# jfdev001/algebraic-multigrid

Hardware: AMD Instinct MI355X
Metric: V-cycles/sec, 2D Poisson N=4096^2 (fine-grid smoother HBM GB/s under roofline) (higher is better)
Workload: dtype f64; 1 GPU; 2D 5-point Poisson 4096x4096 (Grid::laplacian/rhs), true Jacobi smoother omega=0.6 2+2 sweeps, 16-level V-cycle, coarsest 511 dofs, fp64, 1xMI355X; smoother has no counterpart in the reference: pinned to the oracle twin; n=4096, dim=2, levels=16, smoother=jacobi, sweeps=2, graph=True, coarse_solve=band-chain (LDS-resident scalar recurrence, half-bandwidth <= 3, bit-exact), layout=dict

## Files before the change

### algebraic-multigrid_amd/amg_ctypes.py

```python
import contextlib
import ctypes as C
import os

import numpy as np

_HERE = os.path.dirname(os.path.abspath(__file__))
LIB_PATH = os.path.join(_HERE, "libamg_hip.so")

OK, EINVAL, EHIP, ENOMEM, EUNSUPPORTED, ECOMM = 0, 1, 2, 3, 4, 5
SM_SPGS, SM_REF_JACOBI, SM_SOR, SM_JACOBI, SM_MULTICOLOR_GS, SM_CHEBYSHEV, SM_LINE_JACOBI = 0, 1, 2, 3, 4, 5, 6
SM_LINE_ALT = 7
LAYOUT_AUTO, LAYOUT_CSR, LAYOUT_SELL, LAYOUT_DICT = 0, 1, 2, 3

_i32p = C.POINTER(C.c_int32)
_f64p = C.POINTER(C.c_double)
_i64p = C.POINTER(C.c_int64)


class AmgHipError(RuntimeError):
    def __init__(self, status, msg):
        super().__init__(f"amg_hip status {status}: {msg}")
        self.status = status
        self.message = msg

# ... 76 lines not shown
    "amg_hip_setup_on_device": (C.c_int, [C.c_void_p, _i32p]),
    "amg_hip_create_tensor": (C.c_int, [C.c_int64, _i32p, _i32p, _f64p, _f64p, C.c_int32, _i64p,
                                        C.c_int32, C.POINTER(Options), C.POINTER(C.c_void_p)]),
    "amg_hip_create_tensor_dev": (C.c_int, [C.c_int64, C.c_void_p, C.c_void_p, C.c_void_p, C.c_void_p,
                                            C.c_int32, _i64p, C.c_int32, C.POINTER(Options),
                                            C.POINTER(C.c_void_p)]),
    "amg_hip_get_level_dims": (C.c_int, [C.c_void_p, C.c_int32, _i64p]),
    "amg_hip_create_tensor_semi": (C.c_int, [C.c_int64, _i32p, _i32p, _f64p, _f64p, C.c_int32, _i64p,
                                             C.c_int32, _i32p, C.c_double, C.c_int64, C.POINTER(Options),
                                             C.POINTER(C.c_void_p)]),
    "amg_hip_create_tensor_semi_dev": (C.c_int, [C.c_int64, C.c_void_p, C.c_void_p, C.c_void_p, C.c_void_p,
                                                 C.c_int32, _i64p, C.c_int32, _i32p, C.c_double, C.c_int64,
                                                 C.POINTER(Options), C.POINTER(C.c_void_p)]),
    "amg_hip_get_level_axes": (C.c_int, [C.c_void_p, C.c_int32, _i32p]),
    "amg_hip_create_tensor_opdep": (C.c_int, [C.c_int64, _i32p, _i32p, _f64p, _f64p, C.c_int32, _i64p,
                                              C.c_int32, _i32p, C.c_int64, C.POINTER(Options),
                                              C.POINTER(C.c_void_p)]),
    "amg_hip_set_axis_stencil": (None, [C.c_int32]),
    "amg_hip_get_axis_weights": (C.c_int, [C.c_void_p, C.c_int32, _f64p]),
    "amg_hip_axis_restrict": (C.c_int, [C.c_int32, _i64p, C.c_int32, _f64p, _f64p, _f64p]),
    "amg_hip_axis_prolong_add": (C.c_int, [C.c_int32, _i64p, C.c_int32, _f64p, _f64p, _f64p]),
    "amg_hip_get_natural_sides": (C.c_int, [C.c_void_p, _i32p]),
    "amg_hip_create_tensor_periodic": (C.c_int, [C.c_int64, _i32p, _i32p, _f64p, _f64p, C.c_int32, _i64p,
                                                 C.c_int32, C.c_int32, _i32p, C.POINTER(Options),
                                                 C.POINTER(C.c_void_p)]),
    "amg_hip_create_tensor_periodic_dev": (C.c_int, [C.c_int64, C.c_void_p, C.c_void_p, C.c_void_p, C.c_void_p,
                                                     C.c_int32, _i64p, C.c_int32, C.c_int32, _i32p,
                                                     C.POINTER(Options), C.POINTER(C.c_void_p)]),
    "amg_hip_get_periodic_axes": (C.c_int, [C.c_void_p, _i32p]),
    "amg_hip_tensor_restrict_per": (C.c_int, [C.c_int32, _i64p, C.c_int32, C.c_int32, C.c_int32, _f64p, _f64p]),
    "amg_hip_tensor_prolong_add_per": (C.c_int, [C.c_int32, _i64p, C.c_int32, C.c_int32, C.c_int32, _f64p, _f64p]),
    "amg_hip_tensor_restrict_bc": (C.c_int, [C.c_int32, _i64p, C.c_int32, C.c_int32, _f64p, _f64p]),
    "amg_hip_tensor_prolong_add_bc": (C.c_int, [C.c_int32, _i64p, C.c_int32, C.c_int32, _f64p, _f64p]),
    "amg_hip_tensor_axis_strength": (C.c_int, [C.c_int64, _i32p, _i32p, _f64p, C.c_int32, _i64p, _f64p]),
    "amg_hip_tensor_restrict_axes": (C.c_int, [C.c_int32, _i64p, C.c_int32, _f64p, _f64p]),
    "amg_hip_tensor_prolong_add_axes": (C.c_int, [C.c_int32, _i64p, C.c_int32, _f64p, _f64p]),
    "amg_hip_level_transfer_kind": (C.c_int, [C.c_void_p, C.c_int32, _i32p]),
    "amg_hip_tensor_restrict": (C.c_int, [C.c_int32, _i64p, _f64p, _f64p]),
    "amg_hip_tensor_prolong_add": (C.c_int, [C.c_int32, _i64p, _f64p, _f64p]),
    "amg_hip_destroy": (None, [C.c_void_p]),
    "amg_hip_vcycle": (C.c_int, [C.c_void_p]),
    "amg_hip_vcycles": (C.c_int, [C.c_void_p, C.c_int32]),
    "amg_hip_sync": (C.c_int, [C.c_void_p]),
    "amg_hip_solve": (C.c_int, [C.c_void_p, C.c_double, C.c_int64, C.c_int64, _i64p, _f64p,
                                _i32p]),
    "amg_hip_rss": (C.c_int, [C.c_void_p, _f64p]),
    "amg_hip_apply": (C.c_int, [C.c_void_p, C.c_void_p, C.c_void_p]),
    "amg_hip_pcg": (C.c_int, [C.c_void_p, C.c_double, C.c_int64, _i64p, _f64p]),
    "amg_hip_set_mean_projection": (C.c_int, [C.c_void_p, C.c_int32]),
    "amg_hip_get_mean_projection": (C.c_int, [C.c_void_p, _i32p]),
    "amg_hip_center_vec": (C.c_int, [C.c_void_p, C.c_int32, C.c_int32]),
    "amg_hip_block_vcycles": (C.c_int, [C.c_void_p, C.c_int32, C.c_void_p, C.c_void_p, C.c_int32]),
    "amg_hip_block_rss": (C.c_int, [C.c_void_p, C.c_int32, C.c_void_p, C.c_void_p, _f64p]),
    "amg_hip_block_pcg": (C.c_int, [C.c_void_p, C.c_int32, C.c_void_p, C.c_void_p, C.c_double, C.c_int64,
                                    _i64p, _f64p]),
    "amg_hip_block_must_move": (C.c_int, [C.c_void_p, C.c_int32, _f64p]),
    "amg_hip_apply_f32": (C.c_int, [C.c_void_p, C.c_void_p, C.c_void_p]),
    "amg_hip_pcg_mixed": (C.c_int, [C.c_void_p, C.c_double, C.c_int64, _i64p, _f64p]),
    "amg_hip_f32_must_move": (C.c_int, [C.c_void_p, _f64p]),
    "amg_hip_f32_get_vec": (C.c_int, [C.c_void_p, C.c_int32, C.c_int32, C.POINTER(C.c_float)]),
    "amg_hip_f32_set_vec": (C.c_int, [C.c_void_p, C.c_int32, C.c_int32, C.POINTER(C.c_float)]),
    "amg_hip_f32_level_op": (C.c_int, [C.c_void_p, C.c_int32, C.c_int32]),
    "amg_hip_f32_line_subsweep": (C.c_int, [C.c_void_p, C.c_int32, C.c_int32, C.c_int32]),
    "amg_hip_f32_line_factors": (C.c_int, [C.c_void_p, C.c_int32] + [C.POINTER(C.c_float)] * 3),
    "amg_hip_set_f32_lines": (None, [C.c_int32]),
    "amg_hip_set_f32_dict": (None, [C.c_int32]),
    "amg_hip_set_block_lines": (None, [C.c_int32]),
    "amg_hip_n_levels": (C.c_int32, [C.c_void_p]),
    "amg_hip_get_n_dofs": (C.c_int64, [C.c_void_p, C.c_int32]),
    "amg_hip_get_level_nnz": (C.c_int64, [C.c_void_p, C.c_int32]),
    "amg_hip_get_level_matrix": (C.c_int, [C.c_void_p, C.c_int32, _i32p, _i32p, _f64p]),
    "amg_hip_get_transfer_nnz": (C.c_int64, [C.c_void_p, C.c_int32, C.c_int32]),
    "amg_hip_get_transfer": (C.c_int, [C.c_void_p, C.c_int32, C.c_int32, _i32p, _i32p, _f64p]),
    "amg_hip_get_vec": (C.c_int, [C.c_void_p, C.c_int32, C.c_int32, _f64p]),
    "amg_hip_set_vec": (C.c_int, [C.c_void_p, C.c_int32, C.c_int32, _f64p]),
    "amg_hip_copy_vec_dev": (C.c_int, [C.c_void_p, C.c_int32, C.c_int32, C.c_void_p, C.c_int32]),
    "amg_hip_zero_vec": (C.c_int, [C.c_void_p, C.c_int32, C.c_int32]),
    "amg_hip_coarse_halfbw": (C.c_int64, [C.c_void_p]),
    "amg_hip_coarse_solve_kind": (C.c_int32, [C.c_void_p]),
    "amg_hip_fine_sweep_info": (C.c_int, [C.c_void_p, C.c_char_p, C.c_int32, _i32p, _f64p]),
    "amg_hip_set_patch_min_rows": (None, [C.c_int64]),
    "amg_hip_set_band_chain": (None, [C.c_int32]),
    "amg_hip_set_tail_fusion": (None, [C.c_int32]),
    "amg_hip_set_periodic_device_setup": (None, [C.c_int32]),
    "amg_hip_set_patch_tile_flags": (None, [C.c_int32]),
    "amg_hip_set_patch_xf": (None, [C.c_int32]),
    "amg_hip_set_patch_tall": (None, [C.c_int32]),
    "amg_hip_set_patch_seam": (None, [C.c_int32]),
    "amg_hip_patch_leg_lines": (C.c_int32, [C.c_void_p, C.c_int32, C.c_int32]),
    "amg_hip_create_rs": (C.c_int, [C.c_int64, _i32p, _i32p, _f64p, _f64p, C.c_int32, C.c_double, C.c_int64,
                                    C.POINTER(Options), C.POINTER(C.c_void_p)]),
    "amg_hip_slab_plan": (C.c_int, [C.c_int64, C.c_int32, C.c_int32, C.c_int32, C.POINTER(SlabInfo)]),
    "amg_hip_slab_setup": (C.c_int, [C.c_void_p, C.c_int32, C.c_int32, C.c_int32, C.POINTER(SlabInfo)]),
    "amg_hip_slab_run": (C.c_int, [C.c_void_p, C.c_int32]),
    "amg_hip_create_poisson_window": (C.c_int, [C.c_int32, C.c_int64, C.c_int64, C.c_int64, C.c_int32,
                                                C.POINTER(Options), C.POINTER(C.c_void_p)]),
    "amg_hip_window_setup": (C.c_int, [C.c_void_p, _i64p, _i64p, _i64p, _i64p]),
    "amg_hip_window_run": (C.c_int, [C.c_void_p, C.c_int32]),
    "amg_hip_vec_dev_ptr": (C.c_int, [C.c_void_p, C.c_int32, C.c_int32, C.POINTER(C.c_void_p), _i64p]),
    "amg_hip_get_stream": (C.c_int, [C.c_void_p, C.POINTER(C.c_void_p)]),
    "amg_hip_comm_unique_id": (C.c_int, [C.c_char_p]),
    "amg_hip_comm_create": (C.c_int, [C.c_char_p, C.c_int32, C.c_int32, C.c_int32, C.POINTER(C.c_void_p)]),
    "amg_hip_comm_destroy": (None, [C.c_void_p]),
    "amg_hip_comm_rank": (C.c_int32, [C.c_void_p]),
    "amg_hip_comm_world": (C.c_int32, [C.c_void_p]),
    "amg_hip_comm_neighbor_exchange": (C.c_int, [C.c_void_p, C.c_void_p, C.c_int64, C.c_void_p, C.c_int64,
                                                 C.c_void_p, C.c_int64, C.c_void_p, C.c_int64, C.c_void_p]),
    "amg_hip_comm_all_gather": (C.c_int, [C.c_void_p, C.c_void_p, C.c_void_p, C.c_int64, C.c_void_p]),
    "amg_hip_slab_cycle": (C.c_int, [C.c_void_p, C.c_void_p, C.POINTER(SlabInfo)]),
    "amg_hip_window_cycle": (C.c_int, [C.c_void_p, C.c_void_p, C.c_void_p, C.POINTER(WindowPlanC)]),
    "amg_hip_level_layout": (C.c_int32, [C.c_void_p, C.c_int32, C.POINTER(C.c_int32), C.POINTER(C.c_int64)]),
    "amg_hip_get_colors": (C.c_int, [C.c_void_p, C.c_int32, _i32p, _i32p]),
    "amg_hip_level_op": (C.c_int, [C.c_void_p, C.c_int32, C.c_int32]),
    "amg_hip_cheb_bounds": (C.c_int, [C.c_void_p, C.c_int32, _f64p, _f64p]),
    "amg_hip_line_stride": (C.c_int, [C.c_void_p, C.c_int32, C.POINTER(C.c_int64)]),
    "amg_hip_smooth_line": (C.c_int, [C.c_int64, _i32p, _i32p, _f64p, C.c_int64, C.c_double, C.c_int64,
                                      _f64p, _f64p]),
    "amg_hip_line_directions": (C.c_int, [C.c_void_p, C.c_int32, C.POINTER(C.c_int32), C.POINTER(C.c_int64)]),
    "amg_hip_smooth_line_alt": (C.c_int, [C.c_int64, _i32p, _i32p, _f64p, C.c_int32, C.POINTER(C.c_int64),
                                          C.c_double, C.c_int64, C.c_int32, _f64p, _f64p]),
    "amg_hip_line_cyclic": (C.c_int, [C.c_void_p, C.c_int32, _i32p]),
    "amg_hip_smooth_line_alt_per": (C.c_int, [C.c_int64, _i32p, _i32p, _f64p, C.c_int32, C.POINTER(C.c_int64),
                                              C.c_int32, C.c_double, C.c_int64, C.c_int32, _f64p, _f64p]),
    "amg_hip_smooth_chebyshev": (C.c_int, [C.c_int64, _i32p, _i32p, _f64p, _f64p, _f64p, C.c_int32,
                                           C.c_double, C.c_double, C.c_int64]),
    "amg_hip_cycle_bytes": (C.c_int, [C.c_void_p, _f64p, _f64p]),
    "amg_hip_cycle_must_move": (C.c_int, [C.c_void_p, C.c_int32, _f64p]),
    "amg_hip_profile_fine_sweep": (C.c_int, [C.c_void_p, C.c_int32, _f64p, _f64p]),
    "amg_hip_smooth": (C.c_int, [C.c_int32, C.c_int64, _i32p, _i32p, _f64p, _f64p, _f64p,
                                 C.c_double, C.c_double, C.c_int64, C.c_int64, _i64p, _i32p]),
    "amg_hip_spgs_sweep": (C.c_int, [C.c_int32, C.c_int64, _i32p, _i32p, _f64p, _f64p, _f64p]),
    "amg_hip_residual": (C.c_int, [C.c_int64, _i32p, _i32p, _f64p, _f64p, _f64p, _f64p]),
    "amg_hip_spmv": (C.c_int, [C.c_int64, C.c_int64, _i32p, _i32p, _f64p, _f64p, _f64p]),
    "amg_hip_linear_restrict": (C.c_int, [C.c_int64, C.c_int64, _f64p, _f64p]),
    "amg_hip_linear_prolong_add": (C.c_int, [C.c_int64, C.c_int64, _f64p, _f64p]),
    "amg_hip_rss_host": (C.c_int, [C.c_int64, _i32p, _i32p, _f64p, _f64p, _f64p, _f64p]),
    "amg_hip_coarse_solve": (C.c_int, [C.c_int64, _i32p, _i32p, _f64p, _f64p, _f64p, _i64p]),
    "amg_hip_coarse_solve_fast": (C.c_int, [C.c_int64, _i32p, _i32p, _f64p, _f64p, _f64p, _i64p,
                                            _i32p]),
    "amg_hip_laplacian": (C.c_int64, [C.c_int32, C.c_int64, _i32p, _i32p, _f64p]),
    "amg_hip_rhs": (C.c_int, [C.c_int32, C.c_int64, _f64p]),
    "amg_hip_csr_shape": (C.c_int, [C.c_int64, _i32p, _i32p, _i32p]),
    "amg_hip_dev_residual": (C.c_int, [C.c_int64, C.c_int64, C.c_int32, C.c_int32, C.c_void_p,
                                       C.c_void_p, C.c_void_p, C.c_void_p, C.c_void_p,
                                       C.c_void_p, C.c_void_p]),
    "amg_hip_dev_jacobi": (C.c_int, [C.c_int64, C.c_int64, C.c_int32, C.c_int32, C.c_void_p,
                                     C.c_void_p, C.c_void_p, C.c_void_p, C.c_void_p, C.c_void_p,
                                     C.c_double, C.c_int64, C.c_void_p]),
    "amg_hip_dev_spmv": (C.c_int, [C.c_int64, C.c_int64, C.c_int32, C.c_int32, C.c_void_p,
                                   C.c_void_p, C.c_void_p, C.c_void_p, C.c_void_p, C.c_void_p]),
    "amg_hip_devmat_create": (C.c_int, [C.c_int64, C.c_int64, _i32p, _i32p, _f64p, C.c_int32,
                                        C.c_int64, C.c_int32, C.POINTER(C.c_void_p)]),
    "amg_hip_set_index16": (None, [C.c_int32]),
    "amg_hip_set_nontemporal": (None, [C.c_int32]),
    "amg_hip_set_dict_rows": (None, [C.c_int32]),
    "amg_hip_set_dict_stencil": (None, [C.c_int32]),
    "amg_hip_set_xcd_mapping": (None, [C.c_int32]),
    "amg_hip_set_row_types": (None, [C.c_int32]),
    "amg_hip_dict_probe": (C.c_int, [C.c_int64, C.c_int64, _i32p, _i32p, _f64p, C.c_int64,
                                     C.POINTER(C.c_int32), C.POINTER(C.c_int32), C.POINTER(C.c_int32)]),
    "amg_hip_devmat_destroy": (None, [C.c_void_p]),
    "amg_hip_devmat_layout": (C.c_int, [C.c_void_p, C.POINTER(C.c_int32), C.POINTER(C.c_int64)]),
    "amg_hip_devmat_apply": (C.c_int, [C.c_void_p, C.c_int32, C.c_void_p, C.c_void_p, C.c_void_p,
                                       C.c_double, C.c_int64, C.c_void_p]),
    "amg_hip_dev_jacobi_from_zero": (C.c_int, [C.c_int64, C.c_void_p, C.c_void_p, C.c_void_p,
                                               C.c_double, C.c_void_p]),
# ... 72 lines not shown


def set_nontemporal(on):
    lib().amg_hip_set_nontemporal(int(on))


def set_dict_rows(rows_per_lane):
    lib().amg_hip_set_dict_rows(int(rows_per_lane))


def set_dict_stencil(on):
    lib().amg_hip_set_dict_stencil(int(on))


def dict_probe(rowptr, col, val, ncols, diag_shift=0):
    rowptr, col, val = _a32(rowptr), _a32(col), _a64(val)
    a, b, c = C.c_int32(0), C.c_int32(0), C.c_int32(0)
    st = lib().amg_hip_dict_probe(rowptr.size - 1, ncols, _p32(rowptr), _p32(col), _p64(val),
                                  diag_shift, C.byref(a), C.byref(b), C.byref(c))
    if st == EUNSUPPORTED:
        return None
    _chk(st)
    return a.value, b.value, c.value


class Comm:

    def __init__(self, id_bytes, rank, world, device=-1):
        h = C.c_void_p()
        _chk(lib().amg_hip_comm_create(bytes(id_bytes), int(rank), int(world), int(device), C.byref(h)))
        self._h, self.rank, self.world = h, rank, world

    @staticmethod
    def unique_id():
        buf = C.create_string_buffer(128)
        _chk(lib().amg_hip_comm_unique_id(buf))
        return buf.raw

    def slab_cycle(self, mg, info):
        _chk(lib().amg_hip_slab_cycle(mg._h, self._h, C.byref(info)))

    def window_cycle(self, window_mg, tail_mg, plan_c):
        _chk(lib().amg_hip_window_cycle(window_mg._h, tail_mg._h, self._h, C.byref(plan_c)))

    def close(self):
        if getattr(self, "_h", None):
            lib().amg_hip_comm_destroy(self._h)
            self._h = None

    def __del__(self):
        self.close()


def slab_plan(lines, rank, world, levels):
    info = SlabInfo()
    _chk(lib().amg_hip_slab_plan(int(lines), int(rank), int(world), int(levels), C.byref(info)))
    return info


def set_patch_tile_flags(on):
    lib().amg_hip_set_patch_tile_flags(int(bool(on)))


def set_axis_stencil(on):
    lib().amg_hip_set_axis_stencil(int(bool(on)))


def set_patch_xf(on):
    lib().amg_hip_set_patch_xf(int(bool(on)))


def set_patch_tall(on):
    lib().amg_hip_set_patch_tall(int(bool(on)))


def set_patch_seam(on):
    lib().amg_hip_set_patch_seam(int(bool(on)))


def set_tail_fusion(on):
    lib().amg_hip_set_tail_fusion(int(bool(on)))


def set_periodic_device_setup(on):
    lib().amg_hip_set_periodic_device_setup(int(bool(on)))


def set_f32_lines(on):
    lib().amg_hip_set_f32_lines(int(bool(on)))


@contextlib.contextmanager
def f32_lines():
    set_f32_lines(1)
    try:
        yield
    finally:
        set_f32_lines(0)


def set_f32_dict(on):
    lib().amg_hip_set_f32_dict(int(bool(on)))


@contextlib.contextmanager
def f32_dict():
    set_f32_dict(1)
    try:
        yield
    finally:
        set_f32_dict(0)


def set_block_lines(on):
    lib().amg_hip_set_block_lines(int(bool(on)))


@contextlib.contextmanager
def block_lines():
    set_block_lines(1)
    try:
        yield
    finally:
        set_block_lines(0)


def set_band_chain(on):
    lib().amg_hip_set_band_chain(int(bool(on)))


PATCH_MIN_ROWS_DEFAULT = 1000000


def set_patch_min_rows(rows):
    lib().amg_hip_set_patch_min_rows(int(rows))


def set_row_types(on):
    lib().amg_hip_set_row_types(int(on))


def set_xcd_mapping(on):
    lib().amg_hip_set_xcd_mapping(int(on))


class DevMat:

    RESIDUAL, JACOBI, SPMV = 0, 1, 2

    def __init__(self, rowptr, col, val, ncols, layout=LAYOUT_AUTO, diag_shift=0, device=0):
        rowptr, col, val = _a32(rowptr), _a32(col), _a64(val)
        self.rows, self.cols = int(rowptr.size - 1), int(ncols)
        self.diag_shift, self.device = int(diag_shift), int(device)
        self._h = C.c_void_p()
        st = lib().amg_hip_devmat_create(self.rows, self.cols, _p32(rowptr), _p32(col), _p64(val), int(layout),
                                         self.diag_shift, self.device, C.byref(self._h))
        if st == EINVAL:
            raise ValueError(lib().amg_hip_last_error().decode())
        _chk(st)

    def layout(self):
        lay, nb = C.c_int32(0), C.c_int64(0)
        _chk(lib().amg_hip_devmat_layout(self._h, C.byref(lay), C.byref(nb)))
        return lay.value, int(nb.value)

    def apply(self, op, x, f=None, omega=1.0, diag_shift=None):
# ... 487 lines not shown

    @property
    def n_levels(self):
        return lib().amg_hip_n_levels(self._h)

    def get_n_dofs(self, level):
        return int(lib().amg_hip_get_n_dofs(self._h, level))

    def get_coefficient_matrix(self, level):
        n = self.get_n_dofs(level)
        nnz = lib().amg_hip_get_level_nnz(self._h, level)
        colptr = np.empty(n + 1, np.int32)
        rowind = np.empty(nnz, np.int32)
        val = np.empty(nnz, np.float64)
        _chk(lib().amg_hip_get_level_matrix(self._h, level, _p32(colptr), _p32(rowind), _p64(val)))
        return colptr, rowind, val

    def get_transfer(self, level, which):
        w = 1 if which == "R" else 0
        nnz = lib().amg_hip_get_transfer_nnz(self._h, level, w)
        if nnz < 0:
            raise ValueError("level out of range")
        n_h, n_H = self.get_n_dofs(level), self.get_n_dofs(level + 1)
        cols = n_h if w else n_H
        colptr = np.empty(cols + 1, np.int32)
        rowind = np.empty(nnz, np.int32)
        val = np.empty(nnz, np.float64)
        _chk(lib().amg_hip_get_transfer(self._h, level, w, _p32(colptr), _p32(rowind), _p64(val)))
        return colptr, rowind, val

    def _get(self, level, which):
        out = np.empty(self.get_n_dofs(level), np.float64)
        _chk(lib().amg_hip_get_vec(self._h, level, which, _p64(out)))
        return out

    def get_soln(self, level=0):
        return self._get(level, 0)

    def get_rhs(self, level=0):
        return self._get(level, 1)

    def get_residual(self, level=0):
        return self._get(level, 2)

    def set_vec(self, level, which, v):
        v = _a64(v)
        assert v.size == self.get_n_dofs(level)
        _chk(lib().amg_hip_set_vec(self._h, level, {"u": 0, "f": 1, "r": 2}[which], _p64(v)))

    def copy_vec_dev(self, level, which, dev_ptr, to_solver):
        _chk(lib().amg_hip_copy_vec_dev(self._h, level, {"u": 0, "f": 1, "r": 2}[which],
                                        C.c_void_p(dev_ptr), int(to_solver)))

    def zero_vec(self, level, which):
        _chk(lib().amg_hip_zero_vec(self._h, level, {"u": 0, "f": 1, "r": 2}[which]))

    def get_tolerance(self):
        return self.tolerance

    def level_layout(self, level):
        lay, nb = C.c_int32(0), C.c_int64(0)
        _chk(lib().amg_hip_level_layout(self._h, level, C.byref(lay), C.byref(nb)))
        return int(lay.value), int(nb.value)

    def coarse_halfbw(self):
        return int(lib().amg_hip_coarse_halfbw(self._h))

    def get_colors(self, level):
        color = np.empty(self.get_n_dofs(level), np.int32)
        nc = C.c_int32(0)
        _chk(lib().amg_hip_get_colors(self._h, level, _p32(color), C.byref(nc)))
        return color, nc.value

    def cycle_bytes(self):
        a, b = C.c_double(0), C.c_double(0)
        _chk(lib().amg_hip_cycle_bytes(self._h, C.byref(a), C.byref(b)))
        return a.value, b.value

    def cycle_must_move(self, part=0):
        b = C.c_double(0)
        _chk(lib().amg_hip_cycle_must_move(self._h, int(part), C.byref(b)))
        return b.value

    def patch_leg_lines(self, level, leg):
        return int(lib().amg_hip_patch_leg_lines(self._h, int(level), int(leg)))

    def profile_fine_sweep(self, n_launches):
        a, b = C.c_double(0), C.c_double(0)
        _chk(lib().amg_hip_profile_fine_sweep(self._h, n_launches, C.byref(a), C.byref(b)))
        name = C.create_string_buffer(256)
        k, nb = C.c_int32(0), C.c_double(0)
        _chk(lib().amg_hip_fine_sweep_info(self._h, name, 256, C.byref(k), C.byref(nb)))
        return a.value, b.value, k.value, name.value.decode(), nb.value

    def fine_sweep_info(self):
        name = C.create_string_buffer(256)
        k, nb = C.c_int32(0), C.c_double(0)
        _chk(lib().amg_hip_fine_sweep_info(self._h, name, 256, C.byref(k), C.byref(nb)))
        return name.value.decode(), k.value, nb.value

    def cheb_bounds(self, level):
        lo, hi = C.c_double(0), C.c_double(0)
        st = lib().amg_hip_cheb_bounds(self._h, int(level), C.byref(lo), C.byref(hi))
        if st == EINVAL:
            raise ValueError(lib().amg_hip_last_error().decode())
        _chk(st)
        return lo.value, hi.value

    def line_stride(self, level):
        s = C.c_int64(0)
        st = lib().amg_hip_line_stride(self._h, int(level), C.byref(s))
        if st == EINVAL:
            raise ValueError(lib().amg_hip_last_error().decode())
        _chk(st)
        return s.value

    def line_directions(self, level):
        nd = C.c_int32(0)
        st3 = (C.c_int64 * 3)()
        st = lib().amg_hip_line_directions(self._h, int(level), C.byref(nd), st3)
        if st == EINVAL:
            raise ValueError(lib().amg_hip_last_error().decode())
        _chk(st)
        return [int(st3[d]) for d in range(nd.value)]

    def line_cyclic(self, level):
        m = C.c_int32(0)
        st = lib().amg_hip_line_cyclic(self._h, int(level), C.byref(m))
        if st == EINVAL:
            raise ValueError(lib().amg_hip_last_error().decode())
        _chk(st)
        return m.value

    def coarse_solve_kind(self):
        return {0: "band (one wave, sequential, bit-exact)", 1: "spike (partitioned, parallel)",
                2: "band-wide (blocked sequential, any half-bandwidth, bit-exact)",
                3: "band-chain (LDS-resident scalar recurrence, half-bandwidth <= 3, bit-exact)"}[
                    int(lib().amg_hip_coarse_solve_kind(self._h))]

    def level_op(self, level, op):
        _chk(lib().amg_hip_level_op(self._h, level, op))

    def vcycle(self, n=1):
        _chk(lib().amg_hip_vcycles(self._h, n))

    def sync(self):
        _chk(lib().amg_hip_sync(self._h))

    def rss(self):
        out = C.c_double(0)
        _chk(lib().amg_hip_rss(self._h, C.byref(out)))
        return out.value

    def slab_setup(self, rank, world, max_levels=-1):
        info = SlabInfo()
        _chk(lib().amg_hip_slab_setup(self._h, int(rank), int(world), int(max_levels), C.byref(info)))
        return info

    def slab_run(self, part):
        _chk(lib().amg_hip_slab_run(self._h, int(part)))

    def apply_dev(self, v_dev, z_dev):
        _chk(lib().amg_hip_apply(self._h, C.c_void_p(v_dev), C.c_void_p(z_dev)))

    def pcg(self, rtol=1e-10, max_iters=100):
        it, rel = C.c_int64(0), C.c_double(0)
# ... 363 lines not shown
```

### algebraic-multigrid_amd/csrc/kernels.hip

```cpp
#include <hip/hip_runtime.h>
#include <cstdlib>
#include <stdint.h>

#include <cstdio>
#include <type_traits>
#include <utility>
#include <vector>
#include <algorithm>
#include <cmath>

#include "kernels.hpp"

namespace amg_hip {

__device__ __forceinline__ void lds_barrier() {
  asm volatile("s_waitcnt lgkmcnt(0)\n\ts_barrier" ::: "memory");
}

constexpr bool mode_cheb(int m) { return (m & ~3) == 16; }
constexpr bool mode_jac(int m) { return m == CSR_JACOBI || mode_cheb(m); }
constexpr bool cheb_first(int m) { return (m & 1) != 0; }
constexpr bool cheb_last(int m) { return (m & 2) != 0; }
template <int MODE>
__device__ __forceinline__ double cheb_update(double t, double xi, double di, double alpha, double beta,
// ... 745 lines not shown
    dict_rows<MODE, WORDS, UN, R>(s, row0, tab, x, omega, dshift, res);
  }
  if constexpr (mode_cheb(MODE)) {
    double dn[R];
#pragma unroll
    for (int r = 0; r < R; ++r) res[r] = cheb_update<MODE>(res[r], s.xi[r], s.di[r], alpha, omega, dn[r]);
    if (!cheb_last(MODE)) dict_store<WORDS, NT, R>(s, row0, dn, dvec);
  }
  dict_store<WORDS, NT, R>(s, row0, res, out);
}

template <int R>
__device__ __forceinline__ void dict_restrict_tail(int tile, int n, const double* rs, int nH,
                                                   double* __restrict__ fH,
                                                   const double* __restrict__ diagH,
                                                   double* __restrict__ uH1,
                                                   double* __restrict__ uH0, double omega) {
  for (int q = threadIdx.x; q < 128 * R - 1; q += 256) {
    const int j = tile * (128 * R - 1) + q;
    if (j >= nH) break;
    const int64_t i = 2 * (int64_t)j;
    double sum = 0.0;
    if (i < n) sum += 0.5 * rs[2 * q];
    if (i + 1 < n) sum += 1.0 * rs[2 * q + 1];
    if (i + 2 < n) sum += 0.5 * rs[2 * q + 2];
    fH[j] = sum;
    if (uH1) {
      const double xi = 0.0, acc = 0.0;
      const double d = diagH[j];
      uH1[j] = (d == 0.0) ? xi : xi + omega * ((sum - acc) / d - xi);
    } else {
      uH0[j] = 0.0;
    }
  }
}
template <int R>
__device__ __forceinline__ void dict_prolong_tail(int tile, int n, const double* rs, int n_h,
                                                  const double* uh_in, double* uh_out) {
  typedef double f64x2 __attribute__((ext_vector_type(2)));
  const int stride = 256 * R - 2;
#pragma unroll
  for (int r = 0; r < R; ++r) {
    const int q = (int)threadIdx.x * R + r;
    const int j = tile * stride + q;
    if ((q == 0 && tile != 0) || q > stride || j > n) continue;
    double t0 = 0.0, t1 = 0.0;
    const double b = (j < n) ? rs[q] : 0.0;
    if (j >= 1 && j - 1 < n) t0 += 0.5 * rs[q - 1];
    if (j < n) {
      t0 += 0.5 * b;
      t1 += 1.0 * b;
    }
    const int64_t i = 2 * (int64_t)j;
    if (i + 1 < n_h) {
      f64x2 u = *reinterpret_cast<const f64x2*>(uh_in + i);
      u.x = u.x + t0;
      u.y = u.y + t1;
      *reinterpret_cast<f64x2*>(uh_out + i) = u;
    } else if (i < n_h) {
      uh_out[i] = uh_in[i] + t0;
    }
  }
}
__device__ __forceinline__ double dict_restrict_pre(int tile, int nH, const double* __restrict__ diagH) {
  const int q = threadIdx.x, j = tile * 255 + q;
  return (q < 255 && j < nH) ? diagH[j] : 0.0;
}
__device__ __forceinline__ void dict_restrict_tail(int tile, int n, const double* rs, int nH,
                                                   double* __restrict__ fH, double dH,
                                                   double* __restrict__ uH1, double omega) {
  const int q = threadIdx.x, j = tile * 255 + q;
  if (q >= 255 || j >= nH) return;
  const int64_t i = 2 * (int64_t)j;
  double sum = 0.0;
  if (i < n) sum += 0.5 * rs[2 * q];
  if (i + 1 < n) sum += 1.0 * rs[2 * q + 1];
  if (i + 2 < n) sum += 0.5 * rs[2 * q + 2];
  fH[j] = sum;
  const double xi = 0.0, acc = 0.0;
  const double d = dH;
  uH1[j] = (d == 0.0) ? xi : xi + omega * ((sum - acc) / d - xi);
}
typedef double pair_f64x2 __attribute__((ext_vector_type(2)));
__device__ __forceinline__ void dict_prolong_pre(int tile, int n, int n_h, const double* uh_in,
                                                 pair_f64x2 (&pre)[2], double& lone) {
  bool two[2], one[2];
  int64_t i[2];
#pragma unroll
  for (int r = 0; r < 2; ++r) {
    const int q = (int)threadIdx.x * 2 + r;
    const int j = tile * 510 + q;
    const bool on = !((q == 0 && tile != 0) || q > 510 || j > n);
    i[r] = 2 * (int64_t)j;
    two[r] = on && i[r] + 1 < n_h;
    one[r] = on && i[r] + 1 == n_h;
    pre[r].x = pre[r].y = 0.0;
  }
  lone = 0.0;
#pragma unroll
  for (int r = 0; r < 2; ++r)
    if (two[r]) pre[r] = *reinterpret_cast<const pair_f64x2*>(uh_in + i[r]);
  if (one[0] || one[1]) lone = uh_in[n_h - 1];
}
__device__ __forceinline__ void dict_prolong_tail(int tile, int n, const double* rs, int n_h,
                                                  const pair_f64x2 (&pre)[2], double lone,
                                                  double* uh_out) {
#pragma unroll
  for (int r = 0; r < 2; ++r) {
    const int q = (int)threadIdx.x * 2 + r;
    const int j = tile * 510 + q;
    if ((q == 0 && tile != 0) || q > 510 || j > n) continue;
    double t0 = 0.0, t1 = 0.0;
    const double b = (j < n) ? rs[q] : 0.0;
    if (j >= 1 && j - 1 < n) t0 += 0.5 * rs[q - 1];
    if (j < n) {
      t0 += 0.5 * b;
      t1 += 1.0 * b;
    }
    const int64_t i = 2 * (int64_t)j;
    if (i + 1 < n_h) {
      pair_f64x2 u = pre[r];
      u.x = u.x + t0;
      u.y = u.y + t1;
      *reinterpret_cast<pair_f64x2*>(uh_out + i) = u;
    } else if (i < n_h) {
      uh_out[i] = lone + t0;
    }
  }
}
template <int WORDS, int UN, bool NT, int R>
__global__ __launch_bounds__(256) void dict_resid_restrict_kernel(
    int n, const uint64_t* __restrict__ codes, const uint8_t* __restrict__ rtype,
    const uint64_t* __restrict__ rwords, const int32_t* __restrict__ doff,
    const double* __restrict__ dval, int ntab, const double* x, const double* __restrict__ f,
    double* r_out, int nH, double* __restrict__ fH, const double* __restrict__ diagH,
    double* __restrict__ uH1, double* __restrict__ uH0, double omega, int xcd_map,
    const double* __restrict__ utd, const int32_t* __restrict__ uti) {
  __shared__ DictEntry tab[256];
  __shared__ uint64_t wtab[256 * WORDS];
  __shared__ double rs[256 * R];
  const int tile = xcd_tile(blockIdx.x, gridDim.x, xcd_map);
  const int row0 = tile * (256 * R - 2) + (int)threadIdx.x * R;
  DictStream<WORDS, R> s;
  dict_fetch<CSR_RESID, WORDS, NT, R>(s, row0, n, codes, rtype, f, x, 0);
  dict_stage_table<CSR_RESID>(tab, doff, dval, ntab);
  if (rtype) dict_stage_words<WORDS>(wtab, rwords);
  __syncthreads();
  double res[R];
  bool fast = false;
  if constexpr (R == 2 && (UN == 7 || UN == 16)) {
    if (utd) fast = dict_stencil_can<UN>(s.ty, s.live, uti);
    if (fast) dict_rows_stencil<CSR_RESID, UN>(s.ty, s.fi, s.xi, row0, utd, uti, x, omega, res);
  }
  if (!fast) {
    if (rtype) dict_expand<WORDS, R>(s, wtab);
    dict_rows<CSR_RESID, WORDS, UN, R>(s, row0, tab, x, omega, 0, res);
  }
  if (r_out) dict_store<WORDS, NT, R>(s, row0, res, r_out);
#pragma unroll
  for (int r = 0; r < R; ++r) rs[threadIdx.x * R + r] = s.live[r] ? res[r] : 0.0;
  __syncthreads();
  dict_restrict_tail<R>(tile, n, rs, nH, fH, diagH, uH1, uH0, omega);
}
template <int WORDS, int UN, bool NT, int R>
__global__ __launch_bounds__(256) void dict_jacobi_prolong_kernel(
    int n, const uint64_t* __restrict__ codes, const uint8_t* __restrict__ rtype,
    const uint64_t* __restrict__ rwords, const int32_t* __restrict__ doff,
    const double* __restrict__ dval, int ntab, const double* x, const double* __restrict__ f,
    double* out, double omega, int n_h, const double* uh_in, double* uh_out, int xcd_map,
    const double* __restrict__ utd, const int32_t* __restrict__ uti) {
  __shared__ DictEntry tab[256];
  __shared__ uint64_t wtab[256 * WORDS];
  __shared__ double rs[256 * R];
  const int tile = xcd_tile(blockIdx.x, gridDim.x, xcd_map);
  const int stride = 256 * R - 2;
  const int row0 = tile * stride + (int)threadIdx.x * R;
  DictStream<WORDS, R> s;
  dict_fetch<CSR_JACOBI, WORDS, NT, R>(s, row0, n, codes, rtype, f, x, 0);
  dict_stage_table<CSR_JACOBI>(tab, doff, dval, ntab);
  if (rtype) dict_stage_words<WORDS>(wtab, rwords);
  __syncthreads();
  double res[R];
  bool fast = false;
  if constexpr (R == 2 && (UN == 7 || UN == 16)) {
    if (utd) fast = dict_stencil_can<UN>(s.ty, s.live, uti);
    if (fast) dict_rows_stencil<CSR_JACOBI, UN>(s.ty, s.fi, s.xi, row0, utd, uti, x, omega, res);
  }
  if (!fast) {
    if (rtype) dict_expand<WORDS, R>(s, wtab);
    dict_rows<CSR_JACOBI, WORDS, UN, R>(s, row0, tab, x, omega, 0, res);
  }
  dict_store<WORDS, NT, R>(s, row0, res, out);
#pragma unroll
  for (int r = 0; r < R; ++r) rs[threadIdx.x * R + r] = s.live[r] ? res[r] : 0.0;
// ... 170 lines not shown
    const uint64_t* __restrict__ rwords, const int32_t* __restrict__ doff,
    const double* __restrict__ dval, int ntab, const double* a, const double* __restrict__ f,
    double* u_out, double* r_out, int nH, double* __restrict__ fH,
    const double* __restrict__ diagH, double* __restrict__ uH1, double omega, int hbw,
    int xcd_map) {
  __shared__ DictEntry tabJ[256];
  __shared__ DictEntry tabR[256];
  __shared__ __attribute__((aligned(16))) uint64_t wc[PAIR_W * WORDS];
  __shared__ uint16_t tw[PAIR_W / 2];
  __shared__ __attribute__((aligned(16))) double aw[PAIR_AW];
  __shared__ __attribute__((aligned(16))) double fw[PAIR_W];
  __shared__ double uw[PAIR_W];
  __shared__ double rs[512];
  const int tile = xcd_tile(blockIdx.x, gridDim.x, xcd_map);
  const int t0 = tile * 510, w0 = t0 - hbw, W = 512 + 2 * hbw;
  const bool types = rtype != nullptr;
  PairLoads<WORDS> g;
  if (types) dict_pair_issue<WORDS, true>(g, n, w0, hbw, codes, rtype, rwords, doff, dval, ntab, a, f);
  else dict_pair_issue<WORDS, false>(g, n, w0, hbw, codes, rtype, rwords, doff, dval, ntab, a, f);
  const double dH = dict_restrict_pre(tile, nH, diagH);
  dict_put_table<CSR_JACOBI>(tabJ, g.tv, g.to, ntab);
  dict_put_table<CSR_RESID>(tabR, g.tv, g.to, ntab);
  if (types) dict_pair_commit<WORDS, true>(g, n, w0, hbw, wc, tw, aw, fw);
  else dict_pair_commit<WORDS, false>(g, n, w0, hbw, wc, tw, aw, fw);
  __syncthreads();
  dict_pair_stage1<WORDS, UN>(n, w0, hbw, types, tabJ, wc, tw, aw, fw, omega, uw, u_out);
  __syncthreads();
  const int row0 = t0 + (int)threadIdx.x * 2;
  DictStream<WORDS, 2> s;
  dict_pair_stream<WORDS>(s, row0 - w0, W, row0, n, types, wc, tw, fw);
  if (types) dict_expand<WORDS, 2>(s, wc);
  double res[2];
  dict_rows<CSR_RESID, WORDS, UN, 2>(s, row0 - w0, tabR, uw, omega, 0, res);
  if (r_out) dict_store<WORDS, false, 2>(s, row0, res, r_out);
  rs[threadIdx.x * 2] = s.live[0] ? res[0] : 0.0;
  rs[threadIdx.x * 2 + 1] = s.live[1] ? res[1] : 0.0;
  __syncthreads();
  dict_restrict_tail(tile, n, rs, nH, fH, dH, uH1, omega);
}
template <int WORDS, int UN>
__global__ __launch_bounds__(256) void dict_pair_up_kernel(
    int n, const uint64_t* __restrict__ codes, const uint8_t* __restrict__ rtype,
    const uint64_t* __restrict__ rwords, const int32_t* __restrict__ doff,
    const double* __restrict__ dval, int ntab, const double* a, const double* __restrict__ f,
    double* u_out, double omega, int hbw, int n_h, const double* uh_in, double* uh_out,
    int xcd_map) {
  __shared__ DictEntry tabJ[256];
  __shared__ __attribute__((aligned(16))) uint64_t wc[PAIR_W * WORDS];
  __shared__ uint16_t tw[PAIR_W / 2];
  __shared__ __attribute__((aligned(16))) double aw[PAIR_AW];
  __shared__ __attribute__((aligned(16))) double fw[PAIR_W];
  __shared__ double uw[PAIR_W];
  __shared__ double rs[512];
  const int tile = xcd_tile(blockIdx.x, gridDim.x, xcd_map);
  const int t0 = tile * 510, w0 = t0 - hbw, W = 512 + 2 * hbw;
  const bool types = rtype != nullptr;
  PairLoads<WORDS> g;
  if (types) dict_pair_issue<WORDS, true>(g, n, w0, hbw, codes, rtype, rwords, doff, dval, ntab, a, f);
  else dict_pair_issue<WORDS, false>(g, n, w0, hbw, codes, rtype, rwords, doff, dval, ntab, a, f);
  pair_f64x2 pre[2];
  double pre1;
  dict_prolong_pre(tile, n, n_h, uh_in, pre, pre1);
  dict_put_table<CSR_JACOBI>(tabJ, g.tv, g.to, ntab);
  if (types) dict_pair_commit<WORDS, true>(g, n, w0, hbw, wc, tw, aw, fw);
  else dict_pair_commit<WORDS, false>(g, n, w0, hbw, wc, tw, aw, fw);
  __syncthreads();
  dict_pair_stage1<WORDS, UN>(n, w0, hbw, types, tabJ, wc, tw, aw, fw, omega, uw, nullptr);
  __syncthreads();
  const int row0 = t0 + (int)threadIdx.x * 2;
  DictStream<WORDS, 2> s;
  dict_pair_stream<WORDS>(s, row0 - w0, W, row0, n, types, wc, tw, fw);
  s.xi[0] = uw[row0 - w0];
  s.xi[1] = uw[row0 - w0 + 1];
  if (types) dict_expand<WORDS, 2>(s, wc);
  double res[2];
  dict_rows<CSR_JACOBI, WORDS, UN, 2>(s, row0 - w0, tabJ, uw, omega, 0, res);
  dict_store<WORDS, false, 2>(s, row0, res, u_out);
  rs[threadIdx.x * 2] = s.live[0] ? res[0] : 0.0;
  rs[threadIdx.x * 2 + 1] = s.live[1] ? res[1] : 0.0;
  __syncthreads();
  dict_prolong_tail(tile, n, rs, n_h, pre, pre1, uh_out);
}

constexpr int PATCH_TW = 64;
constexpr int PATCH_EH = 48;
constexpr int patch_th(int rings) { return PATCH_EH - 2 * rings; }
static bool patch_rings_ok(int rings) { return rings == 2 || rings == 3; }
constexpr int PATCH_EC = PATCH_TW + 8;
constexpr int PATCH_NT = 432;
constexpr int PATCH_K = PATCH_EH * PATCH_EC / PATCH_NT;
constexpr int PATCH_BUF = (PATCH_EH + 2) * PATCH_EC;
constexpr int PATCH_MAXTAB = 192;
static_assert(PATCH_EH * PATCH_EC == PATCH_K * PATCH_NT && PATCH_NT % PATCH_EC == 0, "patch geometry");
template <int EH_, int EC_>
struct PatchFrameT {
  static constexpr int EH = EH_, EC = EC_, CL = (EC_ - PATCH_TW) / 2;
  static constexpr int NT = EH_ / PATCH_K * EC_, BUF = (EH_ + 2) * EC_;
  static constexpr int th(int rings) { return EH_ - 2 * rings; }
  static_assert(EH_ % PATCH_K == 0 && (EC_ - PATCH_TW) % 2 == 0 && NT >= PATCH_MAXTAB && NT <= 1024, "patch frame");
};
using PatchFrame = PatchFrameT<PATCH_EH, PATCH_EC>;
static_assert(PatchFrame::NT == PATCH_NT && PatchFrame::BUF == PATCH_BUF && PatchFrame::CL == 4, "patch geometry");

struct PatchJ { double a, d; };
struct PatchR { double a; int32_t loff, ok; };

struct PatchCells {
  int cell0, row0, lj0, li;
  double f[PATCH_K];
  uint32_t ty[PATCH_K / 4];
  bool live[PATCH_K];
  bool uniform;
  uint32_t tu;
  bool flagged;
  __device__ __forceinline__ uint32_t type(int k) const {
    return flagged ? tu : (ty[k >> 2] >> (8 * (k & 3))) & 255u;
  }
};

struct PatchU {
  double wj[9], wr[9], diag;
#ifdef AMG_PATCH_FASTDIV
  double rdiag;
#endif
  uint32_t rmask, corners;
};
__device__ __forceinline__ void patch_load_u(PatchU& U, uint32_t tu, const double* __restrict__ utabd,
                                             const int32_t* __restrict__ utabi) {
  const double* d = utabd + (size_t)tu * 19;
  const int32_t* i = utabi + (size_t)tu * 2;
#pragma unroll
  for (int e = 0; e < 9; ++e) {
    U.wj[e] = d[e];
    U.wr[e] = d[9 + e];
  }
  U.diag = d[18];
#ifdef AMG_PATCH_FASTDIV
  U.rdiag = 1.0 / (U.diag == 0.0 ? 1.0 : U.diag);
#endif
  U.rmask = (uint32_t)i[0];
  U.corners = (uint32_t)i[1];
}
template <bool RESID, bool CORNERS, bool GS = false, int MASK = -1, class FR = PatchFrame>
__device__ __forceinline__ void patch_eval_u(const double* buf, int cell0, const PatchU& U,
                                             const double (&f)[PATCH_K], double omega,
                                             double (&res)[PATCH_K]) {
  const double* p = buf + cell0 - FR::EC;
  if (!CORNERS && !RESID && U.diag == 0.0) {
#pragma unroll
    for (int k = 0; k < PATCH_K; ++k) res[k] = p[(k + 1) * FR::EC];
    return;
  }
  double w[3][3];
#pragma unroll
  for (int r = 0; r < 2; ++r)
#pragma unroll
    for (int c = 0; c < 3; ++c) w[r][c] = (CORNERS || c == 1 || r == 1) ? p[r * FR::EC + c - 1] : 0.0;
#pragma unroll
  for (int k = 0; k < PATCH_K; ++k) {
#pragma unroll
    for (int c = 0; c < 3; ++c)
      w[2][c] = (CORNERS || c == 1) ? p[(k + 2) * FR::EC + c - 1] : 0.0;
    if (!CORNERS) {
      w[2][0] = p[(k + 2) * FR::EC - 1];
      w[2][2] = p[(k + 2) * FR::EC + 1];
    }
// ... 914 lines not shown
      if (nt) go(W, U, integral_constant<bool, true>{}, integral_constant<int, 1>{});
      else go(W, U, integral_constant<bool, false>{}, integral_constant<int, 1>{});
    }
    return hipGetLastError();
  };
  if (words == 1) {
    if (wmax <= 3) return with_nr(integral_constant<int, 1>{}, integral_constant<int, 3>{});
    if (wmax <= 5) return with_nr(integral_constant<int, 1>{}, integral_constant<int, 5>{});
    if (wmax <= 7) return with_nr(integral_constant<int, 1>{}, integral_constant<int, 7>{});
    return with_nr(integral_constant<int, 1>{}, integral_constant<int, 8>{});
  }
  if (wmax <= 9) return with_nr(integral_constant<int, 2>{}, integral_constant<int, 9>{});
  if (wmax <= 12) return with_nr(integral_constant<int, 2>{}, integral_constant<int, 12>{});
  return with_nr(integral_constant<int, 2>{}, integral_constant<int, 16>{});
}
static bool dict_args_ok(int64_t n, int words, int wmax, int ntab) {
  return n < ((int64_t)1 << 31) - 1024 && ntab <= 255 && (words == 1 || words == 2) &&
         wmax <= 8 * words;
}
static bool aligned16(const void* a, const void* b, const void* c) {
  return ((reinterpret_cast<uintptr_t>(a) | reinterpret_cast<uintptr_t>(b) |
           reinterpret_cast<uintptr_t>(c)) & 15) == 0;
}
static int g_xcd_slab = 1;
static int g_dict_stencil = [] {
  const char* e = std::getenv("AMG_HIP_DICT_STENCIL");
  return (e && *e == '0') ? 0 : 1;
}();
static const double* dict_stencil_tab(const DictRef& D, const double* x) {
  return (g_dict_stencil && D.utd && D.uti && D.rtype && (reinterpret_cast<uintptr_t>(x) & 15) == 0) ? D.utd : nullptr;
}
static int dict_xcd_map(const DictRef& D, int64_t tile_rows = 512) {
  if (!g_xcd_map) return 0;
  const int64_t tp = D.hb / tile_rows / 8 * 8;
  if (g_xcd_slab && tp >= 16 && tp <= (1 << 20)) return (int)tp;
  return D.nt ? 0 : 1;
}
static bool dict_two_rows(int64_t n, const DictRef& D, const void* f, const void* out) {
  return g_dict_rows_per_lane == 2 && n >= 4096 && aligned16(f, out, D.rtype ? nullptr : D.codes) &&
         (!D.rtype || (reinterpret_cast<uintptr_t>(D.rtype) & 1) == 0);
}
hipError_t launch_dict_resid_restrict(int64_t n, const DictRef& D, const double* x,
                                      const double* f, double* r_out, int64_t nH, double* fH,
                                      const double* diagH, double* uH1, double* uH0,
                                      double omega, hipStream_t st) {
  if (n <= 0) return hipSuccess;
  if (!dict_args_ok(n, D.words, D.wmax, D.ntab) || nH > n || !fH || (uH1 ? !diagH : !uH0))
    return hipErrorInvalidValue;
  const bool two = dict_two_rows(n, D, f, r_out);
  const int64_t stride = 256 * (two ? 2 : 1) - 2;
  const unsigned tiles = (unsigned)((n + stride - 1) / stride);
  return dict_dispatch(D.words, D.wmax, D.nt != 0, two, [&](auto W, auto U, auto NTF, auto RR) {
    hipLaunchKernelGGL((dict_resid_restrict_kernel<decltype(W)::value, decltype(U)::value,
                                                   decltype(NTF)::value, decltype(RR)::value>),
                       dim3(tiles), dim3(256), 0, st, (int)n, D.codes, D.rtype, D.rwords, D.doff,
                       D.dval, D.ntab, x, f, r_out, (int)nH, fH, diagH, uH1, uH0, omega, dict_xcd_map(D, stride),
                       dict_stencil_tab(D, x), D.uti);
  });
}
hipError_t launch_dict_jacobi_prolong(int64_t n, const DictRef& D, const double* x,
                                      const double* f, double* out, double omega, int64_t n_h,
                                      const double* uh_in, double* uh_out, hipStream_t st) {
  if (n <= 0) return hipSuccess;
  if (!dict_args_ok(n_h, D.words, D.wmax, D.ntab) || n > n_h || !uh_in || !uh_out ||
      ((reinterpret_cast<uintptr_t>(uh_in) | reinterpret_cast<uintptr_t>(uh_out)) & 15) != 0)
    return hipErrorInvalidValue;
  const bool two = dict_two_rows(n, D, f, out);
  const int64_t stride = 256 * (two ? 2 : 1) - 2;
  const unsigned tiles = (unsigned)((n + stride - 1) / stride);
  return dict_dispatch(D.words, D.wmax, D.nt != 0, two, [&](auto W, auto U, auto NTF, auto RR) {
    hipLaunchKernelGGL((dict_jacobi_prolong_kernel<decltype(W)::value, decltype(U)::value,
                                                   decltype(NTF)::value, decltype(RR)::value>),
                       dim3(tiles), dim3(256), 0, st, (int)n, D.codes, D.rtype, D.rwords, D.doff,
                       D.dval, D.ntab, x, f, out, omega, (int)n_h, uh_in, uh_out, dict_xcd_map(D, stride),
                       dict_stencil_tab(D, x), D.uti);
  });
}
bool dict_pair_ok(int64_t n, const DictRef& D, int hb, const void* a, const void* b, const void* c) {
  return hb >= 0 && hb <= PAIR_HB - 1 && n >= 256 && n <= 400000 && !D.nt &&
         dict_args_ok(n, D.words, D.wmax, D.ntab) && g_dict_rows_per_lane == 2 &&
         aligned16(a, b, c) && aligned16(D.rtype ? nullptr : D.codes, nullptr, nullptr) &&
         (!D.rtype || (reinterpret_cast<uintptr_t>(D.rtype) & 1) == 0);
}
template <class F>
static hipError_t dict_dispatch_wu(int words, int wmax, F&& go) {
  using std::integral_constant;
  if (words == 1) {
    if (wmax <= 3) go(integral_constant<int, 1>{}, integral_constant<int, 3>{});
    else if (wmax <= 5) go(integral_constant<int, 1>{}, integral_constant<int, 5>{});
    else if (wmax <= 7) go(integral_constant<int, 1>{}, integral_constant<int, 7>{});
    else go(integral_constant<int, 1>{}, integral_constant<int, 8>{});
  } else {
    if (wmax <= 9) go(integral_constant<int, 2>{}, integral_constant<int, 9>{});
    else if (wmax <= 12) go(integral_constant<int, 2>{}, integral_constant<int, 12>{});
    else go(integral_constant<int, 2>{}, integral_constant<int, 16>{});
  }
  return hipGetLastError();
}
hipError_t launch_dict_pair_down(int64_t n, const DictRef& D, int hb, const double* a,
                                 const double* f, double* u_out, double* r_out, int64_t nH,
                                 double* fH, const double* diagH, double* uH1, double omega,
                                 hipStream_t st) {
  if (!dict_pair_ok(n, D, hb, a, f, u_out) || !fH || !diagH || !uH1 || nH > n ||
      (r_out && (reinterpret_cast<uintptr_t>(r_out) & 15)))
    return hipErrorInvalidValue;
  const int hbw = (hb + 1) & ~1;
  const unsigned tiles = (unsigned)((n + 509) / 510);
  return dict_dispatch_wu(D.words, D.wmax, [&](auto W, auto U) {
    hipLaunchKernelGGL((dict_pair_down_kernel<decltype(W)::value, decltype(U)::value>), dim3(tiles),
                       dim3(256), 0, st, (int)n, D.codes, D.rtype, D.rwords, D.doff, D.dval, D.ntab,
                       a, f, u_out, r_out, (int)nH, fH, diagH, uH1, omega, hbw, dict_xcd_map(D));
  });
}
hipError_t launch_dict_pair_up(int64_t n, const DictRef& D, int hb, const double* a,
                               const double* f, double* u_out, double omega, int64_t n_h,
                               const double* uh_in, double* uh_out, hipStream_t st) {
  if (!dict_pair_ok(n, D, hb, a, f, u_out) || n > n_h || !uh_in || !uh_out ||
      ((reinterpret_cast<uintptr_t>(uh_in) | reinterpret_cast<uintptr_t>(uh_out)) & 15) != 0)
    return hipErrorInvalidValue;
  const int hbw = (hb + 1) & ~1;
  const unsigned tiles = (unsigned)((n + 509) / 510);
  return dict_dispatch_wu(D.words, D.wmax, [&](auto W, auto U) {
    hipLaunchKernelGGL((dict_pair_up_kernel<decltype(W)::value, decltype(U)::value>), dim3(tiles),
                       dim3(256), 0, st, (int)n, D.codes, D.rtype, D.rwords, D.doff, D.dval, D.ntab,
                       a, f, u_out, omega, hbw, (int)n_h, uh_in, uh_out, dict_xcd_map(D));
  });
}
constexpr int MARCH_TL = 16, MARCH_TC = 64, MARCH_NT = 512;
constexpr int MARCH_XL = MARCH_TL + 4, MARCH_XC = MARCH_TC + 4;
constexpr int MARCH_SL = MARCH_TL + 2, MARCH_SC = MARCH_TC + 2;
constexpr int MARCH_XN = MARCH_XL * MARCH_XC, MARCH_SN = MARCH_SL * MARCH_SC;
constexpr int MARCH_XS = (MARCH_XN + MARCH_NT - 1) / MARCH_NT;
constexpr int MARCH_SS = (MARCH_SN + MARCH_NT - 1) / MARCH_NT;
constexpr int MARCH_OS = MARCH_TL * MARCH_TC / MARCH_NT;
constexpr int MARCH_TYPES = 64;
typedef MarchRef MarchArgs;
__device__ __forceinline__ double march_update(const double (&w)[6], double diag, const double (&nb)[6],
                                               double xi, double fi, double omega) {
  double acc = 0.0;
#pragma unroll
  for (int u = 0; u < 6; ++u) acc += w[u] * nb[u];
  const bool nod = diag == 0.0;
  const double q = (fi - acc) / (nod ? 1.0 : diag);
  return nod ? xi : xi + omega * (q - xi);
}
__global__ __launch_bounds__(MARCH_NT) void march_kernel(MarchArgs A) {
  __shared__ double X[3][MARCH_XN];
  __shared__ double S[3][MARCH_SN];
  __shared__ double wt[MARCH_TYPES * 8];
  const int tid = (int)threadIdx.x;
  const int tiles_c = A.m / MARCH_TC, tiles_l = A.lines / MARCH_TL;
  const int tile = (int)blockIdx.x % (tiles_c * tiles_l), chunk = (int)blockIdx.x / (tiles_c * tiles_l);
  const int l0 = (tile / tiles_c) * MARCH_TL, c0 = (tile % tiles_c) * MARCH_TC;
  const int pa = chunk * A.chunk_planes, pb = min(pa + A.chunk_planes, A.planes);
  for (int q = tid; q < A.ntypes * 8; q += MARCH_NT) wt[q] = A.wtab[q];
  int xoff[MARCH_XS];
#pragma unroll
  for (int k = 0; k < MARCH_XS; ++k) {
    const int q = k * MARCH_NT + tid;
    const int line = l0 - 2 + q / MARCH_XC, col = c0 - 2 + q % MARCH_XC;
    xoff[k] = (q < MARCH_XN && line >= 0 && line < A.lines && col >= 0 && col < A.m) ? line * A.m + col : -1;
  }
  static_assert(MARCH_SS == MARCH_OS + 1 && 2 * MARCH_SC + 2 * MARCH_TL <= MARCH_NT, "first-sweep cell map");
  int soff[MARCH_SS], si[MARCH_SS], sx[MARCH_SS];
  int ooff[MARCH_OS];
#pragma unroll
  for (int k = 0; k < MARCH_OS; ++k) {
    const int q = k * MARCH_NT + tid;
    const int ol = q / MARCH_TC, oc = q % MARCH_TC;
    ooff[k] = (l0 + ol) * A.m + c0 + oc;
    soff[k] = ooff[k];
    si[k] = (ol + 1) * MARCH_SC + oc + 1;
    sx[k] = (ol + 2) * MARCH_XC + oc + 2;
  }
  {
    const int r = tid;
    int sl, sc;
    if (r < MARCH_SC) { sl = 0; sc = r; }
    else if (r < 2 * MARCH_SC) { sl = MARCH_SL - 1; sc = r - MARCH_SC; }
    else if (r < 2 * MARCH_SC + MARCH_TL) { sl = r - 2 * MARCH_SC + 1; sc = 0; }
    else { sl = r - 2 * MARCH_SC - MARCH_TL + 1; sc = MARCH_SC - 1; }
    const bool ring = r < 2 * MARCH_SC + 2 * MARCH_TL;
    if (!ring) { sl = 1; sc = 1; }
    const int line = l0 - 1 + sl, col = c0 - 1 + sc;
    soff[MARCH_OS] = (ring && line >= 0 && line < A.lines && col >= 0 && col < A.m) ? line * A.m + col : -1;
    si[MARCH_OS] = ring ? sl * MARCH_SC + sc : -1;
    sx[MARCH_OS] = (sl + 1) * MARCH_XC + sc + 1;
  }
  const int64_t M = (int64_t)A.m * A.lines;
  double xr[MARCH_XS];
  auto fetch_x = [&](int plane) {
#pragma unroll
    for (int k = 0; k < MARCH_XS; ++k)
      xr[k] = (plane >= 0 && plane < A.planes && xoff[k] >= 0) ? A.x[(int64_t)plane * M + xoff[k]] : 0.0;
  };
  double wi[6];
#pragma unroll
  for (int u = 0; u < 6; ++u) wi[u] = A.wint[u];
  const double di = A.dint;
  const uint32_t ti = (uint32_t)A.tint;
  double nf1[MARCH_SS];
  uint32_t nt1[MARCH_SS];
  auto fetch_ops = [&](int q) {
    const int p1 = q - 1;
    const bool live1 = p1 >= pa - 1 && p1 <= pb && p1 >= 0 && p1 < A.planes;
#pragma unroll
    for (int k = 0; k < MARCH_SS; ++k) {
      const bool live = live1 && soff[k] >= 0;
      const int64_t r = live ? (int64_t)p1 * M + soff[k] : 0;
// ... 5130 lines not shown
```

### algebraic-multigrid_amd/csrc/kernels.hpp

```cpp
#pragma once
#include <hip/hip_runtime_api.h>
#include <stddef.h>
#include <stdint.h>

namespace amg_hip {

enum CsrMode {
  CSR_RESID = 0,
  CSR_JACOBI = 1,
  CSR_SPMV = 2,
  CSR_RSSQ = 3,
  CSR_GS = 4,
  CSR_JACOBI_P = 5,
  CSR_SPMV_ADD = 6,
  CSR_CHEB = 7
};
constexpr int cheb_kernel_mode(bool first, bool last) { return 16 + (first ? 1 : 0) + (last ? 2 : 0); }
struct ChebStep {
  double* d = nullptr;
  double alpha = 0.0, beta = 0.0;
  bool first = true, last = true;
};

hipError_t launch_dict_gs_sweep(int nc, const int32_t* starts_dev, int64_t n_storage, int words, int wmax,
// ... 26 lines not shown
hipError_t launch_line_setup(const LineRef& L, const int32_t* rowptr, const int32_t* col, const double* val,
                             uint64_t* bad, hipStream_t st);
int64_t line_setup_host(int64_t n, int64_t s, const int32_t* rowptr, const int32_t* col, const double* val,
                        int64_t m = 0, int cyc = 0);
hipError_t launch_line_solve(const LineRef& L, const double* r, double* y, double* u, double omega,
                             hipStream_t st);
bool line_few_chains(int64_t s);
hipError_t launch_line_solve_f32(const LineRefT<float>& L, const float* r, float* y, float* u, float omega,
                                 hipStream_t st);
constexpr int LINEX_COLS = 64, LINEX_RUNS = 8;
template <typename T>
struct LineXRefT {
  int64_t n = 0, nx = 1;
  T *dl = nullptr, *ip = nullptr, *cp = nullptr;
  int32_t cyc = 0;
};
using LineXRef = LineXRefT<double>;
int64_t linex_run(int64_t nx);
hipError_t launch_linex_setup(const LineXRef& L, const int32_t* rowptr, const int32_t* col, const double* val,
                              uint64_t* bad, hipStream_t st);
int64_t linex_setup_host(int64_t n, int64_t nx, const int32_t* rowptr, const int32_t* col, const double* val,
                         int cyc = 0);
hipError_t launch_linex_solve(const LineXRef& L, double* r, double* u, double omega, hipStream_t st);
hipError_t launch_linex_solve_f32(const LineXRefT<float>& L, float* r, float* u, float omega, hipStream_t st);
template <typename T>
struct SeamRefT {
  int64_t n = 0, s = 1, m = 0;
  const T* p = nullptr;
  const T* coef = nullptr;
};
using SeamRef = SeamRefT<double>;
hipError_t launch_seam_rhs(int64_t n, int64_t s, int64_t m, const int32_t* rowptr, const int32_t* col,
                           const double* val, double* u, double* v, hipStream_t st);
hipError_t launch_seam_coef(int64_t n, int64_t s, int64_t m, const int32_t* rowptr, const int32_t* col,
                            const double* val, const double* q, double* coef, uint64_t* bad, hipStream_t st);
int64_t seam_setup_host(int64_t n, int64_t s, int64_t m, const int32_t* rowptr, const int32_t* col,
                        const double* val);
hipError_t launch_line_seam(const SeamRef& S, double* r, hipStream_t st);
hipError_t launch_line_seam_f32(const SeamRefT<float>& S, float* r, hipStream_t st);
hipError_t launch_sell(int mode, int64_t n, int idx16, const int64_t* soff,
                       const void* scol, const double* sval, const double* x,
                       const double* f, double* out, double omega, int64_t diag_shift,
                       hipStream_t st);
struct DictRef {
  int words = 1, wmax = 0, nt = 0, ntab = 0;
  const uint64_t* codes = nullptr;
  const uint8_t* rtype = nullptr;
  const uint64_t* rwords = nullptr;
  const int32_t* doff = nullptr;
  const double* dval = nullptr;
  int scan_new = 99;
  int hb = 0;
  const double* utd = nullptr;
  const int32_t* uti = nullptr;
};
void set_xcd_mapping(int on);
void set_dict_rows_per_lane(int r);
void set_dict_stencil(int on);
hipError_t launch_dict(int mode, int64_t n, const DictRef& D, const double* x, const double* f,
                       double* out, double omega, int64_t diag_shift, hipStream_t st);
hipError_t launch_dict_cheb(int64_t n, const DictRef& D, const double* x, const double* f, double* out,
                            const ChebStep& c, hipStream_t st);
void dict_kernel_name(int mode, int64_t n, const DictRef& D, const void* f, const void* out,
                      char* buf, size_t cap);
hipError_t launch_dict_gs_color(int64_t p0, int64_t count, int words, int wmax,
                                const uint64_t* codes, const int32_t* rowid, const int32_t* doff,
                                const double* dval, int ntab, const double* f, double* u,
                                hipStream_t st);
hipError_t launch_dict_resid_restrict(int64_t n, const DictRef& D, const double* x,
                                      const double* f, double* r_out, int64_t nH, double* fH,
                                      const double* diagH, double* uH1, double* uH0,
                                      double omega, hipStream_t st);
hipError_t launch_dict_jacobi_prolong(int64_t n, const DictRef& D, const double* x,
                                      const double* f, double* out, double omega, int64_t n_h,
                                      const double* uh_in, double* uh_out, hipStream_t st);
bool dict_pair_ok(int64_t n, const DictRef& D, int hb, const void* a, const void* b, const void* c);
hipError_t launch_dict_pair_down(int64_t n, const DictRef& D, int hb, const double* a,
                                 const double* f, double* u_out, double* r_out, int64_t nH,
                                 double* fH, const double* diagH, double* uH1, double omega,
                                 hipStream_t st);
hipError_t launch_dict_pair_up(int64_t n, const DictRef& D, int hb, const double* a,
                               const double* f, double* u_out, double omega, int64_t n_h,
                               const double* uh_in, double* uh_out, hipStream_t st);
constexpr int TAIL_LEVELS_MAX = 6;
struct TailLevelRef {
  int n, hbw, words, ntab;
  const uint8_t* rtype;
  const uint64_t* rwords;
  const int32_t* doff;
  const double* dval;
  const double* f;
  double* u;
  double* tmp;
  const double* diag;
};
struct TailRef {
  int nlev;
  TailLevelRef L[TAIL_LEVELS_MAX];
  int nc, wc;
  const double *cf, *cb, *dg;
  double *fc, *uc, *tmpc;
  const double* diagc;
  int n_fine;
  const double* uf_in;
  double* uf_out;
  double omega;
};
bool tail_level_ok(int64_t n, const DictRef& D, int hb);
int tail_max_coarse();
size_t tail_lds_bytes(const TailRef& A);
size_t tail_lds_capacity();
hipError_t launch_tail(const TailRef& A, hipStream_t st);

struct PatchRef {
  const uint8_t* rtype = nullptr;
  const double* ptab = nullptr;
  const double* utabd = nullptr;
  const int32_t* utabi = nullptr;
  int rings = 3;
  const uint8_t* tflag = nullptr;
  int nent = 0, ntypes = 0, un = 0, nt = 0;
  int umask = 0;
  const uint8_t* cflag = nullptr;
  double dHu = 0.0;
};
hipError_t launch_patch_coarse_flags(int64_t n, int64_t m, int rings, int64_t nH, const double* diagH,
                                     double dref, uint8_t* cflag, hipStream_t st);
hipError_t launch_patch_tile_flags(int64_t n, int64_t m, int rings, const uint8_t* rtype, int ntypes,
                                   uint8_t* flag, int64_t* n_tiles, hipStream_t st);
bool patch_geometry_ok(int64_t n, int64_t m);
int patch_un(int longest_row);
int patch_default_umask(int un);
int patch_kind_umask(int un, int umask);
int patch_lds_pitch();
int patch_max_entries();
hipError_t launch_patch_down(bool first, int64_t n, int64_t m, const PatchRef& P, const double* x,
                             const double* f, double* u_out, double* r_out, int64_t nH, double* fH,
                             const double* diagH, double* uH1, double omega, hipStream_t st,
                             int64_t line_lo = 0, int64_t line_hi = -1, bool xf = false);
int patch_tile_lines(int rings);
int patch_leg_rings(bool first);
hipError_t launch_patch_up(int64_t n, int64_t m, const PatchRef& P, const double* x, const double* f,
                           const double* uH, int64_t nH, double* u_out, double omega,
                           hipStream_t st, int64_t line_lo = 0, int64_t line_hi = -1);
int patch_seam_lines();
hipError_t launch_patch_seam_flags(int64_t n, int64_t m, const uint8_t* rtype, int ntypes, uint8_t* flag,
                                   int64_t* n_tiles, hipStream_t st);
hipError_t launch_patch_seam(int64_t n, int64_t m, const PatchRef& P, const double* x, const double* f,
                             const double* uH, int64_t nH, double* u_out, double* fH, double omega,
                             hipStream_t st);
int patch_rb_max_stages(bool tail);
uint32_t patch_rb_stages(const int* colors, int count);
hipError_t launch_patch_rb(bool prolong, bool tail, int64_t n, int64_t m, const PatchRef& P, const double* x,
                           const double* f, const double* uH, int64_t nH, double* u_out, double* r_out,
                           double* fH, double* uH_zero, uint32_t stages, uint32_t ctab, hipStream_t st,
                           int64_t line_lo = 0, int64_t line_hi = -1);
struct MarchRef {
  int m = 0, lines = 0, planes = 0, ntypes = 0, tint = -1, chunk_planes = 0;
  double omega = 1.0, dint = 0.0;
  double wint[6] = {0, 0, 0, 0, 0, 0};
  const double* wtab = nullptr;
  const uint8_t* rtype = nullptr;
  const double* x = nullptr;
  const double* f = nullptr;
  double* out = nullptr;
};
// ... 230 lines not shown
```

### algebraic-multigrid_amd/csrc/solver.cpp

```cpp
#include <cstddef>
#include <hip/hip_runtime.h>

#include <algorithm>
#include <cmath>
#include <chrono>
#include <cstdio>
#include <cstdlib>
#include <cstring>
#include <functional>
#include <map>
#include <memory>
#include <string>
#include <thread>
#include <vector>

#include <dlfcn.h>

#include "../../include/amg_hip.h"
#include "capture_once.hpp"
#include "host_setup.hpp"
#include "kernels.hpp"

using namespace amg_hip;
#ifdef AMG_PATCH_STAMPS
// ... 1340 lines not shown
  DevMem val;
};
struct F32Line {
  DevMem dl, ip, cp, v, w, y;
  LineRefT<float> ref(const LineOnDev& D) const {
    LineRefT<float> R;
    R.n = D.n;
    R.s = D.s;
    R.dl = dl.as<float>();
    R.ip = ip.as<float>();
    R.cp = cp.as<float>();
    R.v = v.as<float>();
    R.w = w.as<float>();
    return R;
  }
};
struct F32Level {
  F32Mat rows, cols_own;
  const F32Mat* cols = nullptr;
  DevMem u, f, r, tmp, d;
  DevMem pval, rval;
  F32Line line;
  DevMem xdl, xip, xcp;
  F32Line yz[2];
  DevMem seam_p[3], seam_coef[3];
  LineXRefT<float> xref(const AltOnDev& D) const {
    LineXRefT<float> R;
    R.n = D.n;
    R.nx = D.len[0];
    R.dl = xdl.as<float>();
    R.ip = xip.as<float>();
    R.cp = xcp.as<float>();
    return R;
  }
  SeamRefT<float> seam(const AltOnDev& D, int d) const {
    SeamRefT<float> S;
    S.n = D.n;
    S.s = D.stride[d];
    S.m = D.len[d];
    S.p = seam_p[d].as<float>();
    S.coef = seam_coef[d].as<float>();
    return S;
  }
};
struct F32 {
  bool ready = false;
  std::vector<F32Level> lv;
  DevMem cf, cy, cx;
  DevMem pr, pz;
  hipGraph_t graph = nullptr;
  hipGraphExec_t exec = nullptr;
  void reset_graph() {
    if (exec) (void)hipGraphExecDestroy(exec);
    if (graph) (void)hipGraphDestroy(graph);
    exec = nullptr;
    graph = nullptr;
  }
};

int g_march = [] {
  const char* e = std::getenv("AMG_HIP_MARCH");
  return (e && *e == '0') ? 0 : 1;
}();
int g_tail_fusion = [] {
  const char* e = std::getenv("AMG_HIP_TAIL_FUSION");
  return (e && *e == '1') ? 1 : 0;
}();
int g_periodic_device_setup = [] {
  const char* e = std::getenv("AMG_HIP_PERIODIC_DEVICE_SETUP");
  return (e && *e == '1') ? 1 : 0;
}();
int g_f32_lines = [] {
  const char* e = std::getenv("AMG_HIP_F32_LINES");
  return (e && *e == '1') ? 1 : 0;
}();
int g_f32_dict = [] {
  const char* e = std::getenv("AMG_HIP_F32_DICT");
  return (e && *e == '1') ? 1 : 0;
}();
int g_block_lines = [] {
  const char* e = std::getenv("AMG_HIP_BLOCK_LINES");
  return (e && *e == '1') ? 1 : 0;
}();
int64_t g_patch_min_rows = 1000000;

struct amg_hip_solver {
  amg_hip_options opt;
  int64_t patch_min_rows = g_patch_min_rows;
  int patch_xf = g_patch_xf;
  int patch_tall = g_patch_tall;
  int patch_seam = g_patch_seam;
  int device = 0;
  hipStream_t stream = nullptr;
  bool own_stream = true;
  std::vector<Level> lv;
  bool device_setup = false;
  CoarseOnDev coarse;
  DevMem scratch;
  DevMem pcg_x, pcg_p, pcg_q, pcg_b;
  bool project_mean = false;
  hipGraph_t graph = nullptr;
  hipGraphExec_t graph_exec = nullptr;
  bool graph_ready = false;
  double cycle_bytes = 0, fine_sweep_bytes = 0;
  double must_move[6] = {0, 0, 0, 0, 0, 0};
  int acct_part = -1;
  void acct(double bytes) { if (acct_part >= 0) must_move[acct_part] += bytes; }
  int seam_piece = 0, seam_src = 0;
  hipGraph_t seam_graph[5] = {nullptr, nullptr, nullptr, nullptr, nullptr};
  hipGraphExec_t seam_exec[5] = {nullptr, nullptr, nullptr, nullptr, nullptr};
  void reset_seam_graphs() {
    for (int i = 0; i < 5; ++i) {
      if (seam_exec[i]) (void)hipGraphExecDestroy(seam_exec[i]);
      if (seam_graph[i]) (void)hipGraphDestroy(seam_graph[i]);
      seam_exec[i] = nullptr;
      seam_graph[i] = nullptr;
    }
  }
  Slab slab;
  Block blk;
  bool block_acct = false;
  double block_mm[2] = {0, 0};
  void bacct(double mat, double per_col) {
    if (!block_acct) return;
    block_mm[0] += mat;
    block_mm[1] += per_col;
  }
  F32 f32;
  bool f32_acct = false;
  double f32_mm = 0;
  void facct(double bytes) { if (f32_acct) f32_mm += bytes; }

  ~amg_hip_solver() {
    f32.reset_graph();
    blk.reset_graphs();
    slab.reset_graphs();
    reset_seam_graphs();
    if (graph_exec) (void)hipGraphExecDestroy(graph_exec);
    if (graph) (void)hipGraphDestroy(graph);
    if (stream && own_stream) (void)hipStreamDestroy(stream);
  }
};

namespace {

void layout_of(const DevMat& A, int32_t* layout, int64_t* matrix_stream_bytes);
double mat_bytes(const DevMat& A) {
  int64_t b = 0;
  layout_of(A, nullptr, &b);
  return (double)b;
}

amg_hip_status enqueue_multicolor(amg_hip_solver* s, Level& L, hipStream_t st, bool again);

std::string tensor_level_error(int l, const int64_t d[3]) {
  return "level " + std::to_string(l + 1) + " is not possible: level " + std::to_string(l) + " is a " +
         std::to_string(d[0]) + " x " + std::to_string(d[1]) + " x " + std::to_string(d[2]) +
         " grid and an axis of fewer than 2 points cannot be coarsened; reduce `n_levels`";
}

bool jacobi_fuses_zero(const amg_hip_solver* s) {
  return s->opt.smoother == AMG_HIP_SM_JACOBI && !s->opt.no_fusion && s->opt.smoother_iters >= 1;
}
bool jacobi_fuses_prolong(const amg_hip_solver* s, int l) {
  const Level& L = s->lv[l];
  return s->opt.fuse_prolong && jacobi_fuses_zero(s) && L.linear && s->opt.stencil_transfers &&
         L.A_cols().sell;
}

bool fuses_resid_restrict(const amg_hip_solver* s, int l) {
  if (l + 1 >= (int)s->lv.size()) return false;
  const Level& L = s->lv[l];
  if (s->opt.no_fusion || !L.linear || !s->opt.stencil_transfers || !L.A_rows.dict ||
      L.A_rows.dict_shift != 0)
// ... 58 lines not shown
  Level& L = s->lv[l];
  const std::vector<int> q = mc_sequence(L.n_colors, s->opt.smoother_iters);
  const int n = (int)q.size();
  std::vector<McLaunch> P;
  auto chunks = [&](int from, int count, int cap, bool prolong_first) {
    if (count <= 0) return;
    const int k = (count + cap - 1) / cap;
    int at = from;
    for (int c = 0; c < k; ++c) {
      const int len = count / k + (c < count % k ? 1 : 0);
      McLaunch M;
      M.stages = patch_rb_stages(q.data() + at, len);
      M.prolong = prolong_first && c == 0;
      P.push_back(M);
      at += len;
    }
  };
  const int tail_cnt = std::min(n, patch_rb_max_stages(true));
  chunks(0, n - tail_cnt, patch_rb_max_stages(false), false);
  {
    McLaunch M;
    M.stages = patch_rb_stages(q.data() + (n - tail_cnt), tail_cnt);
    M.tail = true;
    P.push_back(M);
  }
  *n_down = (int)P.size();
  chunks(0, n, patch_rb_max_stages(false), true);
  double* third = s->opt.keep_residual ? L.mc_aux.as<double>() : L.r.as<double>();
  double* cur = L.u.as<double>();
  for (size_t i = 0; i < P.size(); ++i) {
    P[i].in = cur;
    P[i].out = i + 1 == P.size() ? L.u.as<double>() : ((i & 1) ? third : L.tmp.as<double>());
    cur = P[i].out;
  }
  return P;
}

bool fuses_jacobi_prolong(const amg_hip_solver* s, int l) {
  if (l + 2 >= (int)s->lv.size()) return false;
  if (patch_level_ok(s, l)) return false;
  const Level& L = s->lv[l];
  const DevMat& AC = s->lv[l + 1].A_cols();
  return jacobi_fuses_zero(s) && !jacobi_fuses_prolong(s, l) && L.linear &&
         s->opt.stencil_transfers && AC.dict && AC.dict_shift == 0;
}

bool pair_level_ok(const amg_hip_solver* s, int l) {
  if (l < 1 || l + 1 >= (int)s->lv.size()) return false;
  const Level& L = s->lv[l];
  const DevMat& A = L.A_rows;
  return jacobi_fuses_zero(s) && s->opt.smoother_iters == 2 && L.symmetric && A.dict &&
         A.dict_shift == 0 && fuses_resid_restrict(s, l) &&
         dict_pair_ok(L.n, A.dict_ref(), A.dict_hb, L.u.p, L.f.p, L.tmp.p);
}
bool pair_up_ok(const amg_hip_solver* s, int l) {
  return pair_level_ok(s, l) && fuses_jacobi_prolong(s, l - 1);
}

int tail_from(const amg_hip_solver* s) {
  const int nl = (int)s->lv.size();
  if (!g_tail_fusion || s->opt.keep_residual || s->opt.window || nl < 3 || s->coarse.kind != COARSE_CHAIN || s->coarse.pin ||
      s->coarse.n > tail_max_coarse())
    return -1;
  int lt = nl - 1;
  while (lt - 1 >= 1 && nl - 1 - (lt - 1) <= TAIL_LEVELS_MAX) {
    const int l = lt - 1;
    const Level& L = s->lv[l];
    if (!(pair_level_ok(s, l) && pair_up_ok(s, l) && tail_level_ok(L.n, L.A_rows.dict_ref(), L.A_rows.dict_hb) &&
          L.diag.p && s->lv[l + 1].diag.p))
      break;
    lt = l;
  }
  for (; lt <= nl - 2; ++lt) {
    TailRef T;
    std::memset(&T, 0, sizeof(T));
    T.nlev = nl - 1 - lt;
    for (int q = 0; q < T.nlev; ++q) T.L[q].n = (int)s->lv[lt + q].n;
    T.nc = (int)s->coarse.n;
    T.wc = (int)s->coarse.w;
    if (tail_lds_bytes(T) <= tail_lds_capacity()) return lt;
  }
  return -1;
}

static bool march_fill(const amg_hip_solver* s, int l, MarchRef* R) {
  const Level& L = s->lv[l];
  const DevMat& A = L.A_cols();
  if (!(s->opt.smoother == AMG_HIP_SM_JACOBI && s->opt.smoother_iters == 2 && !s->opt.no_fusion && !s->opt.window &&
        s->slab.levels == 0 && A.dict && A.dict_typed && A.march_ntypes > 0 && A.dmarch.p && A.march_m > 0 &&
        L.n % A.march_M == 0 && A.march_M % A.march_m == 0 && g_march))
    return false;
  R->m = A.march_m;
  R->lines = A.march_M / A.march_m;
  R->planes = (int)(L.n / A.march_M);
  R->ntypes = A.march_ntypes;
  R->tint = A.march_tint;
  R->omega = s->opt.omega;
  R->dint = A.march_dint;
  for (int u = 0; u < 6; ++u) R->wint[u] = A.march_wint[u];
  R->wtab = A.dmarch.as<double>();
  R->rtype = A.drtype.as<uint8_t>();
  R->f = L.f.as<double>();
  R->x = L.u.as<double>();
  R->out = L.tmp.as<double>();
  R->chunk_planes = 1;
  return march_ok(*R);
}
amg_hip_status enqueue_smooth(amg_hip_solver* s, int l, int phase = 0, int prolong_into = -1,
                              double* prolong_out = nullptr, bool reverse = false) {
  Level& L = s->lv[l];
  hipStream_t st = s->stream;
  const int iters = s->opt.smoother_iters;
  switch (s->opt.smoother) {
    case AMG_HIP_SM_SPGS:
      s->acct(iters * 2.0 * (mat_bytes(L.A_rows) + 24.0 * L.n + (L.scan_C > 0 ? 16.0 * L.n : 0.0)));
      for (int it = 0; it < iters; ++it) {
        if (L.scan_C > 0) {
          const DictRef D = L.A_rows.dict_ref();
          HIP_TRY(launch_gs_scan(L.n, D, L.f.as<double>(), L.u.as<double>(), L.tmp.as<double>(), false, 0,
                                 1.0, L.scan_C, L.scan_ring, st));
          HIP_TRY(launch_gs_scan(L.n, D, L.f.as<double>(), L.u.as<double>(), L.tmp.as<double>(), true, 0,
                                 1.0, L.scan_C, L.scan_ring, st));
          continue;
        }
        HIP_TRY(launch_gs_lex(L.lex_fwd->d, L.f.as<double>(), L.u.as<double>(), 0, 1.0, st));
        HIP_TRY(launch_gs_lex(L.lex_bwd->d, L.f.as<double>(), L.u.as<double>(), 0, 1.0, st));
      }
      return AMG_HIP_OK;
    case AMG_HIP_SM_REF_JACOBI:
    case AMG_HIP_SM_SOR: {
      const int mode = s->opt.smoother == AMG_HIP_SM_SOR ? 2 : 1;
      s->acct(iters * (mat_bytes(L.A_rows) + 24.0 * L.n + (L.scan_C > 0 ? 16.0 * L.n : 0.0)));
      for (int it = 0; it < iters; ++it) {
        if (L.scan_C > 0) {
          HIP_TRY(launch_gs_scan(L.n, L.A_rows.dict_ref(), L.f.as<double>(), L.u.as<double>(),
                                 L.tmp.as<double>(), false, mode, s->opt.omega, L.scan_C, L.scan_ring, st));
          continue;
        }
        HIP_TRY(launch_gs_lex(L.lex_fwd->d, L.f.as<double>(), L.u.as<double>(), mode,
                              s->opt.omega, st));
      }
      return AMG_HIP_OK;
    }
    case AMG_HIP_SM_JACOBI: {
      const DevMat& A = L.A_cols();
      double* a = L.u.as<double>();
      double* b = L.tmp.as<double>();
      int it = 0;
      if (phase == 3) {
        std::swap(a, b);
        it = 1;
      } else if (phase == 1 && jacobi_fuses_zero(s)) {
        HIP_TRY(launch_jacobi_from_zero(L.n, L.diag.as<double>(), L.f.as<double>(), b,
                                        s->opt.omega, st));
        s->acct(24.0 * L.n);
        std::swap(a, b);
        it = 1;
      } else if (phase == 2 && jacobi_fuses_prolong(s, l)) {
        Level& C = s->lv[l + 1];
        HIP_TRY(launch_sell_jacobi_prolong(A.n_rows, A.idx16, A.soff.as<int64_t>(),
                                           A.scol.p, A.sval.as<double>(), a,
                                           C.u.as<double>(), C.n, L.f.as<double>(), b,
                                           s->opt.omega, st));
        s->acct(mat_bytes(A) + 24.0 * L.n + 8.0 * C.n);
        std::swap(a, b);
        it = 1;
// ... 133 lines not shown
                                  L.mc_wmax, L.mc_codes.as<uint64_t>(), L.mc_rowid.as<int32_t>(),
                                  L.mc_doff.as<int32_t>(), L.mc_dval.as<double>(), L.mc_ntab,
                                  L.f.as<double>(), L.u.as<double>(), st);
    return launch_sell_gs_color(A.n_rows, A.max_width, A.soff.as<int64_t>(), A.scol.as<int32_t>(),
                                A.sval.as<double>(), L.mc_rowid.as<int32_t>(), L.mc_start[c],
                                L.mc_start[c + 1] - L.mc_start[c], L.f.as<double>(),
                                L.u.as<double>(), st);
  };
  const bool dedupe = !s->opt.no_fusion;
  for (int c = (again && dedupe) ? 1 : 0; c < L.n_colors; ++c) HIP_TRY(one(c));
  for (int c = L.n_colors - (dedupe ? 2 : 1); c >= 0; --c) HIP_TRY(one(c));
  return AMG_HIP_OK;
}

amg_hip_status enqueue_residual(amg_hip_solver* s, int l) {
  Level& L = s->lv[l];
  HIP_TRY(launch_mat(CSR_RESID, L.A_rows, L.u.as<double>(), L.f.as<double>(), L.r.as<double>(),
                     1.0, s->stream));
  s->acct(mat_bytes(L.A_rows) + 24.0 * L.n);
  return AMG_HIP_OK;
}

enum { CYCLE_ALL = 0, CYCLE_SLAB_DOWN = 1, CYCLE_SLAB_TAIL = 2, CYCLE_SLAB_UP = 3 };
struct Roctx {
  int (*push)(const char*) = nullptr;
  int (*pop)() = nullptr;
  Roctx() {
    if (!std::getenv("AMG_HIP_ROCTX")) return;
    void* h = dlopen("librocprofiler-sdk-roctx.so", RTLD_NOW | RTLD_LOCAL);
    if (!h) h = dlopen("libroctx64.so", RTLD_NOW | RTLD_LOCAL);
    if (!h) return;
    push = (int (*)(const char*))dlsym(h, "roctxRangePushA");
    pop = (int (*)())dlsym(h, "roctxRangePop");
    if (!push || !pop) push = nullptr;
  }
};
struct RoctxRange {
  static Roctx& api() {
    static Roctx r;
    return r;
  }
  bool on = false;
  RoctxRange(const char* what, int level) {
    if (!api().push) return;
    char name[48];
    if (level >= 0) std::snprintf(name, sizeof(name), "L%d %s", level, what);
    else std::snprintf(name, sizeof(name), "%s", what);
    api().push(name);
    on = true;
  }
  ~RoctxRange() {
    if (on) api().pop();
  }
};

amg_hip_status enqueue_vcycle_body(amg_hip_solver* s, int part);
amg_hip_status enqueue_vcycle(amg_hip_solver* s, int part = CYCLE_ALL) {
  const int slot = s->seam_piece == SEAM_CYCLE ? 4 : (s->seam_piece != SEAM_OFF ? 5 : part);
  s->must_move[slot] = 0;
  s->acct_part = slot;
  amg_hip_status r = enqueue_vcycle_body(s, part);
  for (Level& L : s->lv) {
    if (!L.march_odd) continue;
    L.march_odd = false;
    const hipError_t e =
        hipMemcpyAsync(L.tmp.p, L.u.p, sizeof(double) * L.n, hipMemcpyDeviceToDevice, s->stream);
    if (e != hipSuccess && r == AMG_HIP_OK) r = fail(AMG_HIP_EHIP, std::string("K-March copy: ") + hipGetErrorString(e));
    s->acct(16.0 * L.n);
    std::swap(L.u, L.tmp);
  }
  s->acct_part = -1;
  return r;
}
amg_hip_status enqueue_vcycle_body(amg_hip_solver* s, int part) {
  const int nl = (int)s->lv.size();
  hipStream_t st = s->stream;
  const Slab& sb = s->slab;
  const int k = sb.levels;
  const bool ranged = part == CYCLE_SLAB_DOWN || part == CYCLE_SLAB_UP;
  const bool zero_known = jacobi_fuses_zero(s);
  bool first_sweep_done = false;
  const int tail_lt = (part == CYCLE_ALL || part == CYCLE_SLAB_TAIL) ? tail_from(s) : -1;
  bool tail_done = false;
  if (part == CYCLE_SLAB_TAIL) {
    Level& L = s->lv[k];
    if (!patch_xf_pair(s, k - 1)) {
      HIP_TRY(launch_jacobi_from_zero(L.n, L.diag.as<double>(), L.f.as<double>(), L.tmp.as<double>(),
                                      s->opt.omega, st));
      s->acct(24.0 * L.n);
    }
    first_sweep_done = true;
  }
  const int piece = s->seam_piece;
  const int down_from = part == CYCLE_SLAB_TAIL ? k : 0;
  const int down_to = part == CYCLE_SLAB_DOWN ? k : ((part == CYCLE_SLAB_UP || piece == SEAM_FINISH) ? 0 : nl);
  for (int l = down_from; l < down_to; ++l) {
    RoctxRange range("down", l);
    if (l == nl - 1 && nl > 1 && !s->opt.keep_residual) break;
    if (mc_patch_ok(s, l)) {
      Level& L = s->lv[l];
      Level& C = s->lv[l + 1];
      const DevMat& A = L.A_rows;
      int nd = 0;
      const std::vector<McLaunch> plan = mc_plan(s, l, &nd);
      for (int q = 0; q < nd; ++q) {
        const McLaunch& M = plan[(size_t)q];
        HIP_TRY(launch_patch_rb(false, M.tail, L.n, A.patch_m, A.patch_ref(), M.in, L.f.as<double>(), nullptr, C.n,
                                M.out, (M.tail && s->opt.keep_residual) ? L.r.as<double>() : nullptr,
                                M.tail ? C.f.as<double>() : nullptr, M.tail ? C.u.as<double>() : nullptr, M.stages,
                                (uint32_t)L.mc_ctab, st));
      }
      s->acct(nd * 25.0 * L.n + 16.0 * C.n + (s->opt.keep_residual ? 8.0 * L.n : 0.0));
      first_sweep_done = false;
      continue;
    }
    if (mc_strip_ok(s, l)) {
      Level& L = s->lv[l];
      Level& C = s->lv[l + 1];
      StripRef R = mc_strip_ref(s, l);
      R.x = L.u.as<double>();
      R.u_out = L.tmp.as<double>();
      R.r_out = s->opt.keep_residual ? L.r.as<double>() : nullptr;
      R.fH = C.f.as<double>();
      R.uH_zero = C.u.as<double>();
      HIP_TRY(launch_mc_strip(false, true, R, L.A_rows.dict_ref(), st));
      s->acct(26.0 * L.n + 16.0 * C.n + (s->opt.keep_residual ? 8.0 * L.n : 0.0));
      first_sweep_done = false;
      continue;
    }
    if (patch_level_ok(s, l)) {
      Level& L = s->lv[l];
      Level& C = s->lv[l + 1];
      const DevMat& A = L.A_rows;
      if (l == 0 && piece == SEAM_CYCLE) {
        HIP_TRY(launch_patch_seam(L.n, A.patch_m, A.patch_ref(5), seam_buf(s, s->seam_src), L.f.as<double>(),
                                  C.tmp.as<double>(), C.n, seam_buf(s, 1 - s->seam_src), C.f.as<double>(),
                                  s->opt.omega, st));
        s->acct(25.0 * L.n + 16.0 * C.n);
        first_sweep_done = true;
        continue;
      }
      const bool first = l == 0;
      const bool xf_in = l >= 1 && patch_xf_pair(s, l - 1);
      const bool xf_out = patch_xf_pair(s, l);
      HIP_TRY(launch_patch_down(first, L.n, A.patch_m, A.patch_ref(patch_rings(s, first)),
                                first ? L.u.as<double>() : (xf_in ? nullptr : L.tmp.as<double>()),
                                L.f.as<double>(),
                                first ? (piece == SEAM_HEAD ? seam_buf(s, s->seam_src) : L.tmp.as<double>())
                                      : L.u.as<double>(),
                                s->opt.keep_residual ? L.r.as<double>() : nullptr, C.n,
                                C.f.as<double>(), C.diag.as<double>(), xf_out ? nullptr : C.tmp.as<double>(),
                                s->opt.omega, st, ranged ? sb.down_lo[l] : 0,
                                ranged ? sb.down_hi[l] : -1, xf_in));
      {
        double frac = 1.0;
        if (ranged && sb.down_hi[l] >= 0) {
          const double lines = (double)((L.n + A.patch_m - 1) / A.patch_m);
          frac = std::min(1.0, (double)(sb.down_hi[l] - sb.down_lo[l]) / lines);
        }
        s->acct(frac * ((xf_in ? 17.0 : 25.0) * L.n + (xf_out ? 8.0 : 24.0 - 8.0 * A.patch_cfrac) * C.n +
                        (s->opt.keep_residual ? 8.0 * L.n : 0.0)));
      }
      first_sweep_done = true;
      continue;
    }
    if (first_sweep_done && l == tail_lt) {
      TailRef T;
      std::memset(&T, 0, sizeof(T));
      T.nlev = nl - 1 - l;
      for (int q = 0; q < T.nlev; ++q) {
        Level& Q = s->lv[l + q];
        const DictRef D = Q.A_rows.dict_ref();
        TailLevelRef& R = T.L[q];
        R.n = (int)Q.n;
        R.hbw = (Q.A_rows.dict_hb + 1) & ~1;
        R.words = D.words;
        R.ntab = D.ntab;
        R.rtype = D.rtype;
        R.rwords = D.rwords;
        R.doff = D.doff;
        R.dval = D.dval;
        R.f = Q.f.as<double>();
        R.u = Q.u.as<double>();
        R.tmp = Q.tmp.as<double>();
        R.diag = Q.diag.as<double>();
      }
      Level& C = s->lv[nl - 1];
      T.nc = (int)C.n;
      T.wc = (int)s->coarse.w;
      T.cf = s->coarse.sf.as<double>();
      T.cb = s->coarse.sb.as<double>();
      T.dg = s->coarse.d.as<double>();
      T.fc = C.f.as<double>();
      T.uc = C.u.as<double>();
      T.tmpc = C.tmp.as<double>();
      T.diagc = C.diag.as<double>();
      Level& F = s->lv[l - 1];
      T.n_fine = (int)F.n;
      T.uf_in = F.u.as<double>();
      T.uf_out = pair_up_ok(s, l - 1) ? F.tmp.as<double>() : F.u.as<double>();
      T.omega = s->opt.omega;
      HIP_TRY(launch_tail(T, st));
      for (int q = 0; q < T.nlev; ++q) {
        const Level& Q = s->lv[l + q];
        const double nH = (double)s->lv[l + q + 1].n, nF = (double)s->lv[l + q - 1].n;
        s->acct(2.0 * (mat_bytes(Q.A_rows) + 24.0 * Q.n) + 24.0 * nH + 16.0 * nF);
      }
      s->acct(16.0 * (double)C.n * (double)std::max<int64_t>(s->coarse.w, 1) + 24.0 * C.n);
      tail_done = true;
      break;
    }
    if (first_sweep_done && pair_level_ok(s, l)) {
      Level& L = s->lv[l];
      Level& C = s->lv[l + 1];
      const DevMat& A = L.A_rows;
      HIP_TRY(launch_dict_pair_down(A.n_rows, A.dict_ref(), A.dict_hb, L.tmp.as<double>(),
                                    L.f.as<double>(), L.u.as<double>(),
                                    s->opt.keep_residual ? L.r.as<double>() : nullptr, C.n,
                                    C.f.as<double>(), C.diag.as<double>(), C.tmp.as<double>(),
                                    s->opt.omega, st));
      s->acct(mat_bytes(A) + 24.0 * L.n + 24.0 * C.n + (s->opt.keep_residual ? 8.0 * L.n : 0.0));
      continue;
    }
    amg_hip_status r =
        enqueue_smooth(s, l, first_sweep_done ? 3 : (l >= 1 && zero_known) ? 1 : 0);
    if (r != AMG_HIP_OK) return r;
    first_sweep_done = false;
    if (fuses_resid_restrict(s, l)) {
      Level& L = s->lv[l];
      Level& C = s->lv[l + 1];
      const DevMat& A = L.A_rows;
      HIP_TRY(launch_dict_resid_restrict(A.n_rows, A.dict_ref(), L.u.as<double>(),
                                         L.f.as<double>(),
                                         s->opt.keep_residual ? L.r.as<double>() : nullptr, C.n,
                                         C.f.as<double>(),
                                         zero_known ? C.diag.as<double>() : nullptr,
                                         zero_known ? C.tmp.as<double>() : nullptr,
                                         C.u.as<double>(), s->opt.omega, st));
      s->acct(mat_bytes(A) + 16.0 * L.n + (s->opt.keep_residual ? 8.0 * L.n : 0.0) +
              (zero_known ? 24.0 : 16.0) * C.n);
      first_sweep_done = zero_known;
      continue;
    }
    if ((r = enqueue_residual(s, l)) != AMG_HIP_OK) return r;
    if (l + 1 != nl) {
      Level& L = s->lv[l];
      Level& C = s->lv[l + 1];
      if (L.linear && s->opt.stencil_transfers) {
        HIP_TRY(launch_linear_restrict(L.n, C.n, L.r.as<double>(), C.f.as<double>(),
                                       zero_known ? nullptr : C.u.as<double>(), st));
        s->acct(8.0 * L.n + (zero_known ? 8.0 : 16.0) * C.n);
      } else if (L.tensor_stencil) {
        HIP_TRY(launch_tensor_restrict(L.tdim, L.dims, L.tmask, L.tsides, L.tper, L.r.as<double>(), C.f.as<double>(),
                                       zero_known ? nullptr : C.u.as<double>(), st));
        s->acct(8.0 * L.n + (zero_known ? 8.0 : 16.0) * C.n);
      } else if (L.axis_stencil) {
        HIP_TRY(launch_axis_restrict(L.tdim, L.dims, L.axis, L.axis_W_dev.as<double>(), L.r.as<double>(),
                                     C.f.as<double>(), zero_known ? nullptr : C.u.as<double>(), st));
        s->acct(8.0 * L.n + 16.0 * (L.n - C.n) + (zero_known ? 8.0 : 16.0) * C.n);
      } else {
        if (!zero_known) HIP_TRY(hipMemsetAsync(C.u.p, 0, sizeof(double) * C.n, st));
        const DevCsr& R = L.R_rows;
        HIP_TRY(launch_csr(CSR_SPMV, R.n_rows, R.nnz, R.max_block_nnz, R.max_row_nnz,
                           R.rowptr(), R.col(), R.v(), L.r.as<double>(), nullptr,
                           C.f.as<double>(), 1.0, 0, st));
        s->acct(12.0 * R.nnz + 4.0 * C.n + 8.0 * L.n + (zero_known ? 8.0 : 16.0) * C.n);
      }
    }
  }
  auto up_target = [&](int l) -> double* {
    return pair_up_ok(s, l) ? s->lv[l].tmp.as<double>() : s->lv[l].u.as<double>();
  };
  int prolonged_by_solve = -1;
  if (!ranged && !tail_done && piece != SEAM_FINISH) {
    RoctxRange range("coarse solve", -1);
    if (s->opt.window)
      return fail(AMG_HIP_EINVAL, "a window solver (opt.window) runs by parts: amg_hip_window_run");
    Level& C = s->lv[nl - 1];
    const int lp = nl - 2;
    const bool fuse_p = lp >= 0 && s->coarse.kind == COARSE_CHAIN && !s->opt.no_fusion && s->lv[lp].linear &&
                        s->opt.stencil_transfers && !mc_patch_ok(s, lp) && !mc_strip_ok(s, lp) &&
                        !patch_level_ok(s, lp) && !jacobi_fuses_prolong(s, lp) && !fuses_jacobi_prolong(s, lp) &&
                        (part == CYCLE_ALL || (part == CYCLE_SLAB_TAIL && lp >= k));
    if (fuse_p) {
      Level& Lp = s->lv[lp];
      HIP_TRY(launch_coarse(s->coarse, C.f.as<double>(), C.tmp.as<double>(), C.u.as<double>(), st, Lp.n,
                            Lp.u.as<double>(), up_target(lp)));
      s->acct(16.0 * Lp.n);
      prolonged_by_solve = lp;
    } else {
      HIP_TRY(launch_coarse(s->coarse, C.f.as<double>(), C.tmp.as<double>(), C.u.as<double>(), st));
    }
    s->acct(16.0 * (double)C.n * (double)std::max<int64_t>(s->coarse.w, 1) + 24.0 * C.n);
  }
  const int up_from = piece == SEAM_FINISH ? 0 : (part == CYCLE_SLAB_UP ? k - 1 : (part == CYCLE_SLAB_DOWN ? -1 : (tail_done ? tail_lt - 1 : nl - 2)));
  const int up_to = part == CYCLE_SLAB_TAIL ? k : ((piece == SEAM_HEAD || piece == SEAM_CYCLE) ? 1 : 0);
  for (int l = up_from; l >= up_to; --l) {
    RoctxRange range("up", l);
    Level& L = s->lv[l];
    Level& C = s->lv[l + 1];
    if (mc_patch_ok(s, l)) {
      const DevMat& A = L.A_rows;
      int nd = 0;
      const std::vector<McLaunch> plan = mc_plan(s, l, &nd);
      for (size_t q = (size_t)nd; q < plan.size(); ++q) {
        const McLaunch& M = plan[q];
        HIP_TRY(launch_patch_rb(M.prolong, false, L.n, A.patch_m, A.patch_ref(), M.in, L.f.as<double>(),
                                M.prolong ? C.u.as<double>() : nullptr, C.n, M.out, nullptr, nullptr, nullptr,
                                M.stages, (uint32_t)L.mc_ctab, st));
      }
      s->acct((double)(plan.size() - (size_t)nd) * 25.0 * L.n + 8.0 * C.n);
      continue;
    }
    if (mc_strip_ok(s, l)) {
      StripRef R = mc_strip_ref(s, l);
      R.x = L.tmp.as<double>();
      R.u_out = L.u.as<double>();
      R.uH = C.u.as<double>();
      HIP_TRY(launch_mc_strip(true, false, R, L.A_rows.dict_ref(), st));
      s->acct(26.0 * L.n + 8.0 * C.n);
      continue;
    }
    if (patch_level_ok(s, l)) {
      const DevMat& A = L.A_rows;
      const bool top = l == 0;
      const double* uH = patch_level_ok(s, l + 1) ? C.tmp.as<double>() : C.u.as<double>();
      HIP_TRY(launch_patch_up(L.n, A.patch_m, A.patch_ref(patch_rings(s, false)),
                              top ? L.tmp.as<double>() : L.u.as<double>(), L.f.as<double>(), uH, C.n,
                              top ? L.u.as<double>() : L.tmp.as<double>(), s->opt.omega, st,
                              ranged ? sb.up_lo[l] : 0, ranged ? sb.up_hi[l] : -1));
      {
        double frac = 1.0;
        if (ranged && sb.up_hi[l] >= 0) {
          const double lines = (double)((L.n + A.patch_m - 1) / A.patch_m);
          frac = std::min(1.0, (double)(sb.up_hi[l] - sb.up_lo[l]) / lines);
        }
        s->acct(frac * (25.0 * L.n + 8.0 * C.n));
      }
      continue;
    }
    const int into = (l >= 1 && fuses_jacobi_prolong(s, l - 1)) ? l - 1 : -1;
    if (jacobi_fuses_prolong(s, l)) {
      amg_hip_status r = enqueue_smooth(s, l, 2, into, into >= 0 ? up_target(into) : nullptr);
      if (r != AMG_HIP_OK) return r;
      continue;
    }
    if (fuses_jacobi_prolong(s, l)) {
    } else if (l == prolonged_by_solve) {
    } else if (L.linear && s->opt.stencil_transfers) {
      if (up_target(l) != L.u.as<double>())
        HIP_TRY(launch_linear_prolong_to(L.n, C.n, C.u.as<double>(), L.u.as<double>(), up_target(l), st));
      else
        HIP_TRY(launch_linear_prolong_add(L.n, C.n, C.u.as<double>(), L.u.as<double>(), st));
      s->acct(8.0 * C.n + 16.0 * L.n);
    } else if (L.tensor_stencil) {
      HIP_TRY(launch_tensor_prolong_add(L.tdim, L.dims, L.tmask, L.tsides, L.tper, C.u.as<double>(), L.u.as<double>(), st));
      s->acct(8.0 * C.n + 16.0 * L.n);
    } else if (L.axis_stencil) {
      HIP_TRY(launch_axis_prolong_add(L.tdim, L.dims, L.axis, L.axis_W_dev.as<double>(), C.u.as<double>(),
                                      L.u.as<double>(), st));
      s->acct(16.0 * L.n + 16.0 * (L.n - C.n) + 8.0 * C.n);
    } else {
      const DevCsr& P = L.P_rows;
      HIP_TRY(launch_csr(CSR_SPMV_ADD, P.n_rows, P.nnz, P.max_block_nnz, P.max_row_nnz,
                         P.rowptr(), P.col(), P.v(), C.u.as<double>(), L.u.as<double>(),
                         L.u.as<double>(), 1.0, 0, st));
      s->acct(12.0 * P.nnz + 4.0 * L.n + 8.0 * C.n + 16.0 * L.n);
    }
    if (pair_up_ok(s, l)) {
      Level& F = s->lv[l - 1];
      const DevMat& A = L.A_cols();
      HIP_TRY(launch_dict_pair_up(A.n_rows, A.dict_ref(), A.dict_hb, L.tmp.as<double>(),
                                  L.f.as<double>(), L.u.as<double>(), s->opt.omega, F.n,
                                  F.u.as<double>(), up_target(l - 1), st));
      s->acct(mat_bytes(A) + 24.0 * L.n + 16.0 * F.n);
      continue;
    }
    amg_hip_status r = enqueue_smooth(s, l, 0, into, into >= 0 ? up_target(into) : nullptr, true);
    if (r != AMG_HIP_OK) return r;
  }
  return AMG_HIP_OK;
}

amg_hip_status ensure_graph(amg_hip_solver* s) {
  if (s->graph_ready) return AMG_HIP_OK;
  AMG_TRY(capture_once(s->stream, [s] { return enqueue_vcycle(s); }, &s->graph, &s->graph_exec));
  s->graph_ready = true;
  return AMG_HIP_OK;
}

amg_hip_status run_seam_piece(amg_hip_solver* s, int piece, int src) {
  auto enqueue = [s, piece, src] {
    s->seam_piece = piece;
    s->seam_src = src;
    const amg_hip_status r = enqueue_vcycle(s);
    s->seam_piece = SEAM_OFF;
    s->seam_src = 0;
    return r;
  };
  if (!s->opt.use_graph) return enqueue();
  const int gi = piece == SEAM_FINISH ? 4 : (piece == SEAM_HEAD ? 0 : 2) + src;
  if (!s->seam_exec[gi]) AMG_TRY(capture_once(s->stream, enqueue, &s->seam_graph[gi], &s->seam_exec[gi]));
  HIP_TRY(hipGraphLaunch(s->seam_exec[gi], s->stream));
  return AMG_HIP_OK;
}

amg_hip_status set_device(const amg_hip_solver* s) {
  if (s->opt.host_only)
    return fail(AMG_HIP_EINVAL, "solver was created with host_only = 1: no device state");
  HIP_TRY(hipSetDevice(s->device));
  return AMG_HIP_OK;
}

amg_hip_status set_patch_coarse_flags(amg_hip_solver* s) {
  for (size_t l = 0; l + 1 < s->lv.size(); ++l) {
    Level& L = s->lv[l];
    Level& C = s->lv[l + 1];
    DevMat& A = L.A_rows;
    if (!A.patch || !C.diag.p || C.n < 1) continue;
    const int rings = s->opt.smoother == AMG_HIP_SM_MULTICOLOR_GS ? 3 : patch_rings(s, l == 0);
    const int64_t lines = (L.n + A.patch_m - 1) / A.patch_m;
    const int64_t cref = std::min<int64_t>(C.n - 1, ((lines / 2) * A.patch_m + A.patch_m / 2) >> 1);
    double dref = 0.0;
    HIP_TRY(hipMemcpy(&dref, C.diag.as<double>() + cref, sizeof(double), hipMemcpyDeviceToHost));
    for (int rg = 3; rg >= rings; --rg) {
      int64_t tiles = 0;
      HIP_TRY(launch_patch_tile_flags(L.n, A.patch_m, rg, nullptr, A.patch_ntypes, nullptr, &tiles, nullptr));
      HIP_TRY(A.patch_cflags.alloc(((size_t)tiles + 3) & ~(size_t)3));
      HIP_TRY(hipMemset(A.patch_cflags.p, 0, A.patch_cflags.bytes));
      HIP_TRY(launch_patch_coarse_flags(L.n, A.patch_m, rg, C.n, C.diag.as<double>(), dref,
                                        A.patch_cflags.as<uint8_t>(), nullptr));
      if (rg != 3) continue;
      std::vector<uint8_t> fl((size_t)tiles);
      HIP_TRY(hipMemcpy(fl.data(), A.patch_cflags.p, fl.size(), hipMemcpyDeviceToHost));
      int64_t on = 0;
      for (uint8_t f : fl) on += f != 0;
      A.patch_cfrac = g_patch_tile_flags && tiles > 0 ? (double)on / (double)tiles : 0.0;
    }
    A.patch_crings = rings;
    A.patch_dH = dref;
  }
  HIP_TRY(hipDeviceSynchronize());
  return AMG_HIP_OK;
}

void compute_bytes(amg_hip_solver* s) {
  const int nl = (int)s->lv.size();
  double total = 0;
  const int iters = s->opt.smoother_iters;
  int sweeps_per_smooth = iters;
// ... 1726 lines not shown
}

amg_hip_status enqueue_f32_vcycle(amg_hip_solver* s, bool dry) {
  const int nl = (int)s->lv.size();
  amg_hip_status r;
  F32_DO(launch_zero_f32(s->lv[0].n, s->f32.lv[0].u.as<float>(), s->stream));
  s->facct(4.0 * (double)s->lv[0].n);
  for (int l = 0; l + 1 < nl; ++l) {
    if ((r = enqueue_f32_smooth(s, l, dry)) != AMG_HIP_OK) return r;
    if ((r = enqueue_f32_residual(s, l, dry)) != AMG_HIP_OK) return r;
    if ((r = enqueue_f32_restrict(s, l, dry)) != AMG_HIP_OK) return r;
  }
  if ((r = enqueue_f32_coarse(s, dry)) != AMG_HIP_OK) return r;
  for (int l = nl - 2; l >= 0; --l) {
    if ((r = enqueue_f32_prolong(s, l, dry)) != AMG_HIP_OK) return r;
    if ((r = enqueue_f32_smooth(s, l, dry, true)) != AMG_HIP_OK) return r;
  }
  return AMG_HIP_OK;
}
#undef F32_DO

amg_hip_status f32_apply(amg_hip_solver* s, const double* v, double* z) {
  F32& F = s->f32;
  const int64_t n = s->lv[0].n;
  HIP_TRY(launch_to_f32(n, v, F.lv[0].f.as<float>(), s->stream));
  if (!s->opt.use_graph) {
    amg_hip_status r = enqueue_f32_vcycle(s, false);
    if (r != AMG_HIP_OK) return r;
  } else {
    if (!F.exec) AMG_TRY(capture_once(s->stream, [s] { return enqueue_f32_vcycle(s, false); }, &F.graph, &F.exec));
    HIP_TRY(hipGraphLaunch(F.exec, s->stream));
  }
  HIP_TRY(launch_to_f64(n, F.lv[0].u.as<float>(), z, s->stream));
  return AMG_HIP_OK;
}

}

namespace amg_hip {
amg_hip_status fail_status(amg_hip_status st, const std::string& msg) { return fail(st, msg); }
}

extern "C" {

const char* amg_hip_last_error(void) { return g_err.c_str(); }

static_assert(offsetof(amg_hip_options, cyclic_lines) == 68 && offsetof(amg_hip_options, stream) == 72 &&
                  offsetof(amg_hip_options, singular) == 108 && sizeof(amg_hip_options) == 112,
              "amg_hip_options: the layout of the earlier releases must not move");
void amg_hip_default_options(amg_hip_options* o) {
  if (!o) return;
  std::memset(o, 0, sizeof(*o));
  o->smoother = AMG_HIP_SM_SPGS;
  o->smoother_iters = 1;
  o->omega = 1.0;
  o->device = -1;
  o->use_graph = 1;
  o->stencil_transfers = 1;
  o->layout = g_default_layout;
  o->keep_structural_zeros = 0;
  o->no_fusion = 0;
  o->fuse_prolong = 0;
  o->fast_coarse_solve = 0;
  o->stream = nullptr;
  o->window = 0;
  o->cheb_degree = 2;
  o->cheb_lower = 0.3;
  o->cheb_upper = 1.0;
}

void amg_hip_set_index16(int32_t on) { g_index16 = on ? 1 : 0; }
void amg_hip_set_nontemporal(int32_t on) { g_nontemporal = on ? 1 : 0; }
void amg_hip_set_xcd_mapping(int32_t on) { set_xcd_mapping(on); }
void amg_hip_set_row_types(int32_t on) { g_row_types = on ? 1 : 0; }
void amg_hip_set_dict_rows(int32_t rows_per_lane) { set_dict_rows_per_lane(rows_per_lane); }
void amg_hip_set_dict_stencil(int32_t on) { set_dict_stencil(on); }
void amg_hip_set_patch_tile_flags(int32_t on) { g_patch_tile_flags = on ? 1 : 0; }
void amg_hip_set_axis_stencil(int32_t on) { g_axis_stencil = on ? 1 : 0; }
void amg_hip_set_patch_xf(int32_t on) { g_patch_xf = on ? 1 : 0; }
void amg_hip_set_patch_tall(int32_t on) { g_patch_tall = on ? 1 : 0; }
void amg_hip_set_patch_seam(int32_t on) { g_patch_seam = on ? 1 : 0; }
void amg_hip_set_band_chain(int32_t on) { g_no_band_chain = on ? 0 : 1; }
void amg_hip_set_tail_fusion(int32_t on) { g_tail_fusion = on ? 1 : 0; }
void amg_hip_set_periodic_device_setup(int32_t on) { g_periodic_device_setup = on ? 1 : 0; }
void amg_hip_set_f32_lines(int32_t on) { g_f32_lines = on ? 1 : 0; }
void amg_hip_set_f32_dict(int32_t on) { g_f32_dict = on ? 1 : 0; }
void amg_hip_set_block_lines(int32_t on) { g_block_lines = on ? 1 : 0; }
void amg_hip_set_patch_min_rows(int64_t rows) { g_patch_min_rows = rows < 0 ? INT64_MAX : rows; }

void amg_hip_set_default_layout(int32_t layout) {
  if (layout >= AMG_HIP_LAYOUT_AUTO && layout <= AMG_HIP_LAYOUT_DICT) g_default_layout = layout;
}

int amg_hip_device_count(void) {
  int n = 0;
  if (hipGetDeviceCount(&n) != hipSuccess) return 0;
  return n;
}

amg_hip_status amg_hip_create(int64_t n, const int32_t* colptr, const int32_t* rowind,
                              const double* val, const double* b, int32_t n_levels,
                              const amg_hip_options* opts, amg_hip_solver** out) {
  return build_solver(n, colptr, rowind, val, b, n_levels, opts, out);
}

amg_hip_status amg_hip_create_custom(int64_t n, const int32_t* colptr, const int32_t* rowind,
                                     const double* val, const double* b, int32_t n_levels,
                                     const int32_t* const* P_colptr,
                                     const int32_t* const* P_rowind, const double* const* P_val,
                                     const int32_t* const* R_colptr,
                                     const int32_t* const* R_rowind, const double* const* R_val,
                                     const amg_hip_options* opts, amg_hip_solver** out) {
  if (n_levels > 1 && (!P_colptr || !P_rowind || !P_val || !R_colptr || !R_rowind || !R_val))
    return fail(AMG_HIP_EINVAL, "custom transfer operator arrays are null");
  HierarchySpec h;
  h.Pc = P_colptr, h.Pr = P_rowind, h.Pv = P_val;
  h.Rc = R_colptr, h.Rr = R_rowind, h.Rv = R_val;
  return build_solver(n, colptr, rowind, val, b, n_levels, opts, out, h);
}

amg_hip_status amg_hip_create_rs(int64_t n, const int32_t* colptr, const int32_t* rowind,
                                 const double* val, const double* b, int32_t max_levels,
                                 double theta, int64_t min_coarse, const amg_hip_options* opts,
                                 amg_hip_solver** out) {
  if (!(theta >= 0.0 && theta <= 1.0)) return fail(AMG_HIP_EINVAL, "`theta` must be in [0, 1]");
  if (min_coarse < 1) return fail(AMG_HIP_EINVAL, "`min_coarse` must be at least 1");
  HierarchySpec h;
  h.rs_theta = theta;
  h.rs_min_coarse = min_coarse;
  return build_solver(n, colptr, rowind, val, b, max_levels, opts, out, h);
}

static std::string tensor_dims_error(int32_t dim, const int64_t* dims) {
  if (dim != 2 && dim != 3) return "`dim` must be 2 or 3";
  if (!dims) return "`dims` is null";
  if (dims[0] < 1 || dims[1] < 1 || dims[2] < 1) return "every entry of `dims` must be at least 1";
  if (dim == 2 && dims[2] != 1) return "`dims[2]` must be 1 when `dim` is 2";
  if (dims[0] >= ((int64_t)1 << 31) / dims[1] / dims[2]) return "the grid has 2^31 points or more";
  return "";
}

static std::string window_error(const std::string& who, const char* kind) {
  return who + "window solvers (opt.window) coarsen the flat index; a " + kind + "-coarsening hierarchy is not sharded";
}
static std::string grid_size_error(int64_t n, const int64_t* dims, bool figures) {
  if (n == dims[0] * dims[1] * dims[2]) return "";
  const std::string grid = std::to_string(dims[0]) + " x " + std::to_string(dims[1]) + " x " +
                           std::to_string(dims[2]) + " grid";
  return "`n`" + (figures ? " = " + std::to_string(n) : "") + " is not the " + (figures ? grid : "number of points") +
         " of `dims`";
}
static amg_hip_status tensor_grid_args(const std::string& who, int64_t n, int32_t dim, const int64_t* dims,
                                       int32_t window, const char* kind) {
  std::string e = tensor_dims_error(dim, dims);
  if (e.empty()) e = grid_size_error(n, dims, kind != nullptr);
  if (!e.empty()) return fail(AMG_HIP_EINVAL, who + e);
  if (kind && window) return fail(AMG_HIP_EUNSUPPORTED, window_error(who, kind));
  return AMG_HIP_OK;
}
static HierarchySpec tensor_spec(int32_t dim, const int64_t* dims, const SemiRule* semi = nullptr,
                                 int32_t periodic_axes = 0, bool periodic_ctor = false) {
  HierarchySpec h;
  h.dim = dim;
  h.dims = dims;
  h.semi = semi;
  h.periodic = (uint32_t)periodic_axes;
// ... 503 lines not shown
    s->graph = nullptr;
    s->graph_ready = false;
  }
  *info = pl;
  info->pitch0 = m0;
  info->gather_pitch = mk;
  info->gather_rows = G.n;
  info->u0 = s->lv[0].u.as<double>();
  info->f_gather = G.f.as<double>();
  return AMG_HIP_OK;
}

amg_hip_status amg_hip_slab_run(amg_hip_solver* s, int32_t part) {
  if (!s || part < CYCLE_SLAB_DOWN || part > CYCLE_SLAB_UP)
    return fail(AMG_HIP_EINVAL, "amg_hip_slab_run: part is 1 (down-legs), 2 (replicated rest) or 3 (up-legs)");
  Slab& sb = s->slab;
  if (sb.levels < 1) return fail(AMG_HIP_EINVAL, "amg_hip_slab_run: amg_hip_slab_setup has not succeeded");
  amg_hip_status r = set_device(s);
  if (r != AMG_HIP_OK) return r;
  if (!s->opt.use_graph) return enqueue_vcycle(s, part);
  const int gi = part - 1;
  if (!sb.exec[gi])
    AMG_TRY(capture_once(s->stream, [s, part] { return enqueue_vcycle(s, part); }, &sb.graph[gi], &sb.exec[gi]));
  HIP_TRY(hipGraphLaunch(sb.exec[gi], s->stream));
  return AMG_HIP_OK;
}

amg_hip_status amg_hip_window_setup(amg_hip_solver* s, const int64_t* down_lo, const int64_t* down_hi,
                                    const int64_t* up_lo, const int64_t* up_hi) {
  if (!s) return fail(AMG_HIP_EINVAL, "null solver");
  if (!s->opt.window) return fail(AMG_HIP_EINVAL, "amg_hip_window_setup: not a window solver (opt.window)");
  if ((down_lo || down_hi || up_lo || up_hi) && !(down_lo && down_hi && up_lo && up_hi))
    return fail(AMG_HIP_EINVAL, "amg_hip_window_setup: give all four range arrays or none");
  amg_hip_status r = set_device(s);
  if (r != AMG_HIP_OK) return r;
  HIP_TRY(hipStreamSynchronize(s->stream));
  const int k = (int)s->lv.size() - 1;
  Slab& sb = s->slab;
  sb.reset_graphs();
  sb.levels = k;
  sb.rank = 0;
  sb.world = 1;
  sb.down_lo.assign(k, 0);
  sb.down_hi.assign(k, -1);
  sb.up_lo.assign(k, 0);
  sb.up_hi.assign(k, -1);
  if (down_lo)
    for (int l = 0; l < k; ++l) {
      if (down_lo[l] < 0 || up_lo[l] < 0 || down_hi[l] < down_lo[l] || up_hi[l] < up_lo[l])
        return fail(AMG_HIP_EINVAL, "amg_hip_window_setup: bad line range");
      sb.down_lo[l] = down_lo[l];
      sb.down_hi[l] = down_hi[l];
      sb.up_lo[l] = up_lo[l];
      sb.up_hi[l] = up_hi[l];
    }
  return AMG_HIP_OK;
}

amg_hip_status amg_hip_window_run(amg_hip_solver* s, int32_t part) {
  if (!s || (part != CYCLE_SLAB_DOWN && part != CYCLE_SLAB_UP))
    return fail(AMG_HIP_EINVAL, "amg_hip_window_run: part is 1 (down-legs) or 3 (up-legs)");
  if (!s->opt.window) return fail(AMG_HIP_EINVAL, "amg_hip_window_run: not a window solver (opt.window)");
  if (s->slab.levels < 1) {
    amg_hip_status r = amg_hip_window_setup(s, nullptr, nullptr, nullptr, nullptr);
    if (r != AMG_HIP_OK) return r;
  }
  return amg_hip_slab_run(s, part);
}

#ifdef AMG_PATCH_STAMPS
amg_hip_status amg_hip_debug_patch_stamps(void* dev_ptr) {
  HIP_TRY(debug_set_patch_stamps((unsigned long long*)dev_ptr));
  return AMG_HIP_OK;
}
#endif

amg_hip_status amg_hip_get_stream(amg_hip_solver* s, void** stream) {
  if (!s || !stream) return fail(AMG_HIP_EINVAL, "bad argument");
  if (s->opt.host_only) return fail(AMG_HIP_EINVAL, "solver was created with host_only = 1: no device state");
  *stream = (void*)s->stream;
  return AMG_HIP_OK;
}

amg_hip_status amg_hip_vec_dev_ptr(amg_hip_solver* s, int32_t level, int32_t which, void** ptr, int64_t* n) {
  if (!s || !ptr || level < 0 || level >= (int32_t)s->lv.size() || which < 0 || which > 2)
    return fail(AMG_HIP_EINVAL, "bad argument");
  if (s->opt.host_only) return fail(AMG_HIP_EINVAL, "solver was created with host_only = 1: no device state");
  Level& L = s->lv[level];
  *ptr = which == 0 ? L.u.p : (which == 1 ? L.f.p : L.r.p);
  if (n) *n = L.n;
  return AMG_HIP_OK;
}

amg_hip_status amg_hip_sync(amg_hip_solver* s) {
  if (!s) return fail(AMG_HIP_EINVAL, "null solver");
  amg_hip_status r = set_device(s);
  if (r != AMG_HIP_OK) return r;
  HIP_TRY(hipStreamSynchronize(s->stream));
  return AMG_HIP_OK;
}

amg_hip_status amg_hip_copy_vec_dev(amg_hip_solver* s, int32_t level, int32_t which,
                                    void* dev_ptr, int32_t to_solver) {
  if (!s || !dev_ptr || level < 0 || level >= (int32_t)s->lv.size() || which < 0 || which > 2)
    return fail(AMG_HIP_EINVAL, "bad argument");
  amg_hip_status r = set_device(s);
  if (r != AMG_HIP_OK) return r;
  Level& L = s->lv[level];
  void* v = which == 0 ? L.u.p : (which == 1 ? L.f.p : L.r.p);
  if (to_solver)
    HIP_TRY(hipMemcpyAsync(v, dev_ptr, sizeof(double) * L.n, hipMemcpyDeviceToDevice, s->stream));
  else
    HIP_TRY(hipMemcpyAsync(dev_ptr, v, sizeof(double) * L.n, hipMemcpyDeviceToDevice, s->stream));
  return AMG_HIP_OK;
}

amg_hip_status amg_hip_zero_vec(amg_hip_solver* s, int32_t level, int32_t which) {
  if (!s || level < 0 || level >= (int32_t)s->lv.size() || which < 0 || which > 2)
    return fail(AMG_HIP_EINVAL, "bad argument");
  amg_hip_status r = set_device(s);
  if (r != AMG_HIP_OK) return r;
  Level& L = s->lv[level];
  void* v = which == 0 ? L.u.p : (which == 1 ? L.f.p : L.r.p);
  HIP_TRY(hipMemsetAsync(v, 0, sizeof(double) * L.n, s->stream));
  return AMG_HIP_OK;
}

amg_hip_status amg_hip_level_op(amg_hip_solver* s, int32_t level, int32_t op) {
  if (!s) return fail(AMG_HIP_EINVAL, "null solver");
  const int nl = (int)s->lv.size();
  if (level < 0 || level >= nl) return fail(AMG_HIP_EINVAL, "level out of range");
  amg_hip_status r = set_device(s);
  if (r != AMG_HIP_OK) return r;
  hipStream_t st = s->stream;
  Level& L = s->lv[level];
  switch (op) {
    case 0: return enqueue_smooth(s, level, 0);
    case 1: return enqueue_residual(s, level);
    case 2: {
      if (level + 1 >= nl) return fail(AMG_HIP_EINVAL, "no coarser level");
      Level& C = s->lv[level + 1];
      if (L.linear && s->opt.stencil_transfers) {
        HIP_TRY(launch_linear_restrict(L.n, C.n, L.r.as<double>(), C.f.as<double>(), C.u.as<double>(), st));
      } else if (L.tensor_stencil) {
        HIP_TRY(launch_tensor_restrict(L.tdim, L.dims, L.tmask, L.tsides, L.tper, L.r.as<double>(), C.f.as<double>(), C.u.as<double>(), st));
      } else if (L.axis_stencil) {
        HIP_TRY(launch_axis_restrict(L.tdim, L.dims, L.axis, L.axis_W_dev.as<double>(), L.r.as<double>(),
                                     C.f.as<double>(), C.u.as<double>(), st));
      } else {
        HIP_TRY(hipMemsetAsync(C.u.p, 0, sizeof(double) * C.n, st));
        const DevCsr& R = L.R_rows;
        HIP_TRY(launch_csr(CSR_SPMV, R.n_rows, R.nnz, R.max_block_nnz, R.max_row_nnz, R.rowptr(),
                           R.col(), R.v(), L.r.as<double>(), nullptr, C.f.as<double>(), 1.0, 0, st));
      }
      return AMG_HIP_OK;
    }
    case 3: {
      if (level + 1 >= nl) return fail(AMG_HIP_EINVAL, "no coarser level");
      Level& C = s->lv[level + 1];
      if (L.linear && s->opt.stencil_transfers) {
        HIP_TRY(launch_linear_prolong_add(L.n, C.n, C.u.as<double>(), L.u.as<double>(), st));
      } else if (L.tensor_stencil) {
        HIP_TRY(launch_tensor_prolong_add(L.tdim, L.dims, L.tmask, L.tsides, L.tper, C.u.as<double>(), L.u.as<double>(), st));
      } else if (L.axis_stencil) {
        HIP_TRY(launch_axis_prolong_add(L.tdim, L.dims, L.axis, L.axis_W_dev.as<double>(), C.u.as<double>(),
                                        L.u.as<double>(), st));
      } else {
        const DevCsr& P = L.P_rows;
        HIP_TRY(launch_csr(CSR_SPMV_ADD, P.n_rows, P.nnz, P.max_block_nnz, P.max_row_nnz, P.rowptr(),
                           P.col(), P.v(), C.u.as<double>(), L.u.as<double>(), L.u.as<double>(), 1.0, 0, st));
      }
      return AMG_HIP_OK;
    }
    case 4:
      if (level != nl - 1) return fail(AMG_HIP_EINVAL, "the direct solve belongs to the coarsest level");
      HIP_TRY(launch_coarse(s->coarse, L.f.as<double>(), L.tmp.as<double>(), L.u.as<double>(), st));
      return AMG_HIP_OK;
  }
  return fail(AMG_HIP_EINVAL, "unknown level operation");
}

amg_hip_status amg_hip_cheb_bounds(const amg_hip_solver* s, int32_t level, double* lo, double* hi) {
  if (!s || !lo || !hi) return fail(AMG_HIP_EINVAL, "null argument");
  if (s->opt.smoother != AMG_HIP_SM_CHEBYSHEV)
    return fail(AMG_HIP_EINVAL, "amg_hip_cheb_bounds: the solver's smoother is not AMG_HIP_SM_CHEBYSHEV");
  if (level < 0 || level >= (int)s->lv.size()) return fail(AMG_HIP_EINVAL, "level out of range");
  *lo = s->lv[level].cheb_lo;
  *hi = s->lv[level].cheb_hi;
  return AMG_HIP_OK;
}

amg_hip_status amg_hip_line_stride(const amg_hip_solver* s, int32_t level, int64_t* stride) {
  if (!s || !stride) return fail(AMG_HIP_EINVAL, "null argument");
  if (s->opt.smoother != AMG_HIP_SM_LINE_JACOBI)
    return fail(AMG_HIP_EINVAL, "amg_hip_line_stride: the solver's smoother is not AMG_HIP_SM_LINE_JACOBI");
  if (level < 0 || level >= (int)s->lv.size()) return fail(AMG_HIP_EINVAL, "level out of range");
  *stride = s->lv[level].line.s;
  return AMG_HIP_OK;
}

amg_hip_status amg_hip_line_directions(const amg_hip_solver* s, int32_t level, int32_t* n_dir, int64_t strides[3]) {
  if (!s || !n_dir || !strides) return fail(AMG_HIP_EINVAL, "null argument");
  if (s->opt.smoother != AMG_HIP_SM_LINE_ALT)
    return fail(AMG_HIP_EINVAL, "amg_hip_line_directions: the solver's smoother is not AMG_HIP_SM_LINE_ALT");
  if (level < 0 || level >= (int)s->lv.size()) return fail(AMG_HIP_EINVAL, "level out of range");
  const AltOnDev& D = s->lv[level].alt;
  *n_dir = D.n_dir;
  for (int d = 0; d < 3; ++d) strides[d] = d < D.n_dir ? D.stride[d] : 0;
  return AMG_HIP_OK;
}

amg_hip_status amg_hip_line_cyclic(const amg_hip_solver* s, int32_t level, int32_t* axis_mask) {
  if (!s || !axis_mask) return fail(AMG_HIP_EINVAL, "null argument");
  if (s->opt.smoother != AMG_HIP_SM_LINE_ALT)
    return fail(AMG_HIP_EINVAL, "amg_hip_line_cyclic: the solver's smoother is not AMG_HIP_SM_LINE_ALT");
  if (level < 0 || level >= (int)s->lv.size()) return fail(AMG_HIP_EINVAL, "level out of range");
  *axis_mask = s->lv[level].alt.cyclic_mask();
  return AMG_HIP_OK;
// ... 291 lines not shown
  return enqueue_f32_line_subsweep(s, level, d, false);
}

amg_hip_status amg_hip_f32_line_factors(amg_hip_solver* s, int32_t level, float* dl, float* ip, float* cp) {
  amg_hip_status r = f32_line_hook_ready(s, level, !dl || !ip || !cp ? "null argument" : nullptr);
  if (r != AMG_HIP_OK) return r;
  const AltOnDev& D = s->lv[level].alt;
  if (s->opt.smoother != AMG_HIP_SM_LINE_ALT || D.n_dir == 0 || D.axis[0] != 0)
    return fail(AMG_HIP_EINVAL, "level " + std::to_string(level) + " has no x direction (K-LineX factors)");
  F32Level& Q = s->f32.lv[(size_t)level];
  const size_t bytes = sizeof(float) * (size_t)D.n;
  HIP_TRY(hipStreamSynchronize(s->stream));
  HIP_TRY(hipMemcpy(dl, Q.xdl.p, bytes, hipMemcpyDeviceToHost));
  HIP_TRY(hipMemcpy(ip, Q.xip.p, bytes, hipMemcpyDeviceToHost));
  HIP_TRY(hipMemcpy(cp, Q.xcp.p, bytes, hipMemcpyDeviceToHost));
  return AMG_HIP_OK;
}

amg_hip_status amg_hip_solve(amg_hip_solver* s, double tol, int64_t every, int64_t n_iters,
                             int64_t* iters, double* last_rss, int32_t* converged) {
  if (!s) return fail(AMG_HIP_EINVAL, "null solver");
  if (every > n_iters)
    return fail(AMG_HIP_EINVAL, "`compute_error_every_n_iters` must be leq to `n_iters`, got " +
                                    std::to_string(every) + " and " + std::to_string(n_iters));
  if (every <= 0) return fail(AMG_HIP_EINVAL, "`compute_error_every_n_iters` must be positive");
  int64_t iter = 0;
  double error = 100;
  while (iter < n_iters && error > tol) {
    const int64_t k = std::min<int64_t>(std::min(every - iter % every, n_iters - iter), 1 << 20);
    amg_hip_status r = amg_hip_vcycles(s, (int32_t)k);
    if (r != AMG_HIP_OK) return r;
    iter += k;
    if ((iter % every) == 0) {
      if ((r = amg_hip_rss(s, &error)) != AMG_HIP_OK) return r;
    }
  }
  HIP_TRY(hipStreamSynchronize(s->stream));
  if (iters) *iters = iter;
  if (last_rss) *last_rss = error;
  if (converged) *converged = error <= tol;
  return AMG_HIP_OK;
}

int32_t amg_hip_n_levels(const amg_hip_solver* s) { return s ? (int32_t)s->lv.size() : 0; }
int64_t amg_hip_get_n_dofs(const amg_hip_solver* s, int32_t level) {
  if (!s || level < 0 || level >= (int32_t)s->lv.size()) return -1;
  return s->lv[level].n;
}
int64_t amg_hip_get_level_nnz(const amg_hip_solver* s, int32_t level) {
  if (!s || level < 0 || level >= (int32_t)s->lv.size()) return -1;
  return s->lv[level].nnz_struct;
}
amg_hip_status amg_hip_get_level_matrix(const amg_hip_solver* s, int32_t level,
                                        int32_t* colptr, int32_t* rowind, double* val) {
  if (!s || level < 0 || level >= (int32_t)s->lv.size())
    return fail(AMG_HIP_EINVAL, "level out of range");
  if (!s->opt.host_only) HIP_TRY(hipSetDevice(s->device));
  HIP_TRY(s->lv[level].ensure_host_matrix());
  const Sparse& A = s->lv[level].A_csc;
  if (colptr) std::memcpy(colptr, A.ptr.data(), sizeof(int32_t) * A.ptr.size());
  if (rowind) std::memcpy(rowind, A.idx.data(), sizeof(int32_t) * A.idx.size());
  if (val) std::memcpy(val, A.val.data(), sizeof(double) * A.val.size());
  return AMG_HIP_OK;
}
int64_t amg_hip_get_transfer_nnz(const amg_hip_solver* s, int32_t level, int32_t which) {
  if (!s || level < 0 || level + 1 >= (int32_t)s->lv.size()) return -1;
  return (which ? s->lv[level].R() : s->lv[level].P()).nnz();
}
amg_hip_status amg_hip_get_transfer(const amg_hip_solver* s, int32_t level, int32_t which,
                                    int32_t* colptr, int32_t* rowind, double* val) {
  if (!s || level < 0 || level + 1 >= (int32_t)s->lv.size())
    return fail(AMG_HIP_EINVAL, "level out of range");
  const Sparse& M = which ? s->lv[level].R() : s->lv[level].P();
  if (colptr) std::memcpy(colptr, M.ptr.data(), sizeof(int32_t) * M.ptr.size());
  if (rowind) std::memcpy(rowind, M.idx.data(), sizeof(int32_t) * M.idx.size());
  if (val) std::memcpy(val, M.val.data(), sizeof(double) * M.val.size());
  return AMG_HIP_OK;
}

static DevMem* pick_vec(amg_hip_solver* s, int32_t level, int32_t which) {
  if (!s || level < 0 || level >= (int32_t)s->lv.size()) return nullptr;
  Level& L = s->lv[level];
  if (which == 0 && level >= 1 && !s->opt.host_only && patch_level_ok(s, level)) return &L.tmp;
  return which == 0 ? &L.u : (which == 1 ? &L.f : (which == 2 ? &L.r : nullptr));
}
amg_hip_status amg_hip_get_vec(amg_hip_solver* s, int32_t level, int32_t which, double* out) {
  DevMem* m = pick_vec(s, level, which);
  if (!m || !out) return fail(AMG_HIP_EINVAL, "bad level / vector selector");
  if (s->opt.host_only) return fail(AMG_HIP_EINVAL, "host_only solver has no vectors");
  if (which == 2 && !s->opt.keep_residual &&
      (fuses_resid_restrict(s, level) || patch_level_ok(s, level) || mc_patch_ok(s, level) || mc_strip_ok(s, level) ||
       (level == (int32_t)s->lv.size() - 1 && level > 0)))
    return fail(AMG_HIP_EINVAL, "the residual of this level is not kept (create the solver with "
                                "opt.keep_residual = 1)");
  HIP_TRY(hipSetDevice(s->device));
  HIP_TRY(hipStreamSynchronize(s->stream));
  HIP_TRY(hipMemcpy(out, m->p, sizeof(double) * s->lv[level].n, hipMemcpyDeviceToHost));
  return AMG_HIP_OK;
}
amg_hip_status amg_hip_set_vec(amg_hip_solver* s, int32_t level, int32_t which,
                               const double* in) {
  DevMem* m = pick_vec(s, level, which);
  if (!m || !in) return fail(AMG_HIP_EINVAL, "bad level / vector selector");
  if (s->opt.host_only) return fail(AMG_HIP_EINVAL, "host_only solver has no vectors");
  HIP_TRY(hipSetDevice(s->device));
  HIP_TRY(hipStreamSynchronize(s->stream));
  HIP_TRY(hipMemcpy(m->p, in, sizeof(double) * s->lv[level].n, hipMemcpyHostToDevice));
  return AMG_HIP_OK;
}
int64_t amg_hip_coarse_halfbw(const amg_hip_solver* s) { return s ? s->coarse.w : -1; }
int32_t amg_hip_coarse_solve_kind(const amg_hip_solver* s) { return s ? s->coarse.kind : -1; }

namespace {
void layout_of(const DevMat& A, int32_t* layout, int64_t* matrix_stream_bytes) {
  int32_t lay;
  int64_t bytes;
  if (A.dict) {
    lay = AMG_HIP_LAYOUT_DICT;
    bytes = (A.dict_typed ? A.n_rows + 256 * 8 * A.dict_words : A.n_rows * 8 * A.dict_words) +
            (int64_t)A.dict_ntab * 12;
  } else if (A.sell) {
    lay = AMG_HIP_LAYOUT_SELL;
    bytes = A.slots * ((A.idx16 & 1) ? 10 : 12) + (A.n_rows + 63) / 64 * 8;
  } else {
    lay = AMG_HIP_LAYOUT_CSR;
    bytes = A.csr.nnz * 12 + (A.csr.n_rows + 1) * 4;
  }
  if (layout) *layout = lay;
  if (matrix_stream_bytes) *matrix_stream_bytes = bytes;
}
}
amg_hip_status amg_hip_level_layout(const amg_hip_solver* s, int32_t level, int32_t* layout,
                                    int64_t* matrix_stream_bytes) {
  if (!s || level < 0 || level >= (int32_t)s->lv.size())
    return fail(AMG_HIP_EINVAL, "level out of range");
  if (s->opt.host_only) return fail(AMG_HIP_EINVAL, "host_only solver has no device matrices");
  layout_of(s->lv[level].A_rows, layout, matrix_stream_bytes);
  return AMG_HIP_OK;
}

amg_hip_status amg_hip_get_colors(const amg_hip_solver* s, int32_t level, int32_t* color,
                                  int32_t* n_colors) {
  if (!s || level < 0 || level >= (int32_t)s->lv.size())
    return fail(AMG_HIP_EINVAL, "level out of range");
  const Level& L = s->lv[level];
  if (L.color.empty()) return fail(AMG_HIP_EINVAL, "solver was not built with the multicolour smoother");
  if (color) std::memcpy(color, L.color.data(), sizeof(int32_t) * L.color.size());
  if (n_colors) *n_colors = L.n_colors;
  return AMG_HIP_OK;
}

amg_hip_status amg_hip_cycle_bytes(const amg_hip_solver* s, double* cycle_bytes,
                                   double* fine_sweep_bytes) {
  if (!s) return fail(AMG_HIP_EINVAL, "null solver");
  if (cycle_bytes) *cycle_bytes = s->cycle_bytes;
  if (fine_sweep_bytes) *fine_sweep_bytes = s->fine_sweep_bytes;
  return AMG_HIP_OK;
}

namespace {
void cheb_profiled_step(const amg_hip_solver* s, ChebStep* out) {
  const Level& L = s->lv[0];
  const int k = s->opt.cheb_degree;
  std::vector<double> alpha, beta;
  cheb_coefs(L.cheb_lo, L.cheb_hi, k, &alpha, &beta);
  const int j = k >= 3 ? 1 : 0;
// ... 1255 lines not shown
```

### include/amg_hip.h

```cpp
#ifndef AMG_HIP_H
#define AMG_HIP_H

#include <stddef.h>
#include <stdint.h>

#ifdef __cplusplus
extern "C" {
#endif

typedef enum {
  AMG_HIP_OK = 0,
  AMG_HIP_EINVAL = 1,
  AMG_HIP_EHIP = 2,
  AMG_HIP_ENOMEM = 3,
  AMG_HIP_EUNSUPPORTED = 4,
  AMG_HIP_ECOMM = 5
} amg_hip_status;

typedef enum {
  AMG_HIP_SM_SPGS = 0,
  AMG_HIP_SM_REF_JACOBI = 1,
  AMG_HIP_SM_SOR = 2,
  AMG_HIP_SM_JACOBI = 3,
  AMG_HIP_SM_MULTICOLOR_GS = 4,
  AMG_HIP_SM_CHEBYSHEV = 5,
  AMG_HIP_SM_LINE_JACOBI = 6,
  AMG_HIP_SM_LINE_ALT = 7
} amg_hip_smoother;

typedef enum {
  AMG_HIP_LAYOUT_AUTO = 0,
  AMG_HIP_LAYOUT_CSR = 1,
  AMG_HIP_LAYOUT_SELL = 2,
  AMG_HIP_LAYOUT_DICT = 3
} amg_hip_layout;

typedef struct {
  int32_t smoother;
  int32_t smoother_iters;
  double omega;
  int32_t device;
  int32_t use_graph;
  int32_t stencil_transfers;
  int32_t layout;
  int32_t host_only;
  int32_t keep_structural_zeros;
  int32_t no_fusion;
  int32_t fuse_prolong;
  int32_t fast_coarse_solve;
  int32_t host_galerkin;
  int32_t keep_residual;
  int32_t exact_coarse_solve;
  int32_t exact_gs;
  int32_t cyclic_lines;
  void* stream;
  int32_t window;
  int32_t cheb_degree;
  double cheb_lower;
  double cheb_upper;
  int32_t natural_sides;
  int32_t singular;
} amg_hip_options;

typedef struct amg_hip_solver amg_hip_solver;

const char* amg_hip_last_error(void);
void amg_hip_default_options(amg_hip_options* o);

void amg_hip_set_default_layout(int32_t layout);

void amg_hip_set_index16(int32_t on);
void amg_hip_set_nontemporal(int32_t on);
void amg_hip_set_xcd_mapping(int32_t on);
void amg_hip_set_row_types(int32_t on);
void amg_hip_set_dict_rows(int32_t rows_per_lane);
void amg_hip_set_dict_stencil(int32_t on);
void amg_hip_set_patch_min_rows(int64_t rows);

void amg_hip_set_patch_tile_flags(int32_t on);
void amg_hip_set_patch_xf(int32_t on);
void amg_hip_set_patch_tall(int32_t on);
void amg_hip_set_patch_seam(int32_t on);
void amg_hip_set_band_chain(int32_t on);

void amg_hip_set_tail_fusion(int32_t on);

void amg_hip_set_periodic_device_setup(int32_t on);

void amg_hip_set_f32_lines(int32_t on);

void amg_hip_set_f32_dict(int32_t on);

void amg_hip_set_block_lines(int32_t on);

int amg_hip_device_count(void);

amg_hip_status amg_hip_create(int64_t n, const int32_t* colptr,
                              const int32_t* rowind, const double* val,
                              const double* b, int32_t n_levels,
                              const amg_hip_options* opts,
                              amg_hip_solver** out);

amg_hip_status amg_hip_create_custom(int64_t n, const int32_t* colptr,
                                     const int32_t* rowind, const double* val,
                                     const double* b, int32_t n_levels,
                                     const int32_t* const* P_colptr,
                                     const int32_t* const* P_rowind,
                                     const double* const* P_val,
                                     const int32_t* const* R_colptr,
                                     const int32_t* const* R_rowind,
                                     const double* const* R_val,
                                     const amg_hip_options* opts,
                                     amg_hip_solver** out);

amg_hip_status amg_hip_create_rs(int64_t n, const int32_t* colptr, const int32_t* rowind,
                                 const double* val, const double* b, int32_t max_levels,
                                 double theta, int64_t min_coarse, const amg_hip_options* opts,
                                 amg_hip_solver** out);

amg_hip_status amg_hip_create_tensor(int64_t n, const int32_t* colptr, const int32_t* rowind,
                                     const double* val, const double* b, int32_t dim,
                                     const int64_t* dims , int32_t n_levels,
                                     const amg_hip_options* opts, amg_hip_solver** out);
amg_hip_status amg_hip_create_tensor_semi(int64_t n, const int32_t* colptr, const int32_t* rowind,
                                          const double* val, const double* b, int32_t dim,
                                          const int64_t* dims , int32_t n_levels,
                                          const int32_t* axis_masks ,
                                          double theta, int64_t min_coarse,
                                          const amg_hip_options* opts, amg_hip_solver** out);
amg_hip_status amg_hip_create_tensor_opdep(int64_t n, const int32_t* colptr, const int32_t* rowind,
                                           const double* val, const double* b, int32_t dim,
                                           const int64_t* dims , int32_t n_levels,
                                           const int32_t* axis_masks ,
                                           int64_t min_coarse, const amg_hip_options* opts, amg_hip_solver** out);
void amg_hip_set_axis_stencil(int32_t on);
amg_hip_status amg_hip_get_axis_weights(const amg_hip_solver* s, int32_t level, double* W);
amg_hip_status amg_hip_get_natural_sides(const amg_hip_solver* s, int32_t* mask);
amg_hip_status amg_hip_create_tensor_periodic(int64_t n, const int32_t* colptr, const int32_t* rowind,
                                              const double* val, const double* b, int32_t dim,
                                              const int64_t* dims , int32_t periodic_axes,
                                              int32_t n_levels,
                                              const int32_t* axis_masks ,
                                              const amg_hip_options* opts, amg_hip_solver** out);
amg_hip_status amg_hip_get_periodic_axes(const amg_hip_solver* s, int32_t* mask);
amg_hip_status amg_hip_get_level_axes(const amg_hip_solver* s, int32_t level, int32_t* axis_mask);
amg_hip_status amg_hip_tensor_axis_strength(int64_t n, const int32_t* colptr, const int32_t* rowind,
                                            const double* val, int32_t dim, const int64_t* dims ,
                                            double* w );
amg_hip_status amg_hip_get_level_dims(const amg_hip_solver* s, int32_t level, int64_t* dims );
amg_hip_status amg_hip_level_transfer_kind(const amg_hip_solver* s, int32_t level, int32_t* kind);

amg_hip_status amg_hip_create_poisson(int32_t dim, int64_t n, int32_t n_levels,
                                      const amg_hip_options* opts, amg_hip_solver** out);

amg_hip_status amg_hip_create_poisson_tensor(int32_t dim, int64_t n, int32_t n_levels,
                                             const amg_hip_options* opts, amg_hip_solver** out);
amg_hip_status amg_hip_create_tensor_dev(int64_t n, const int32_t* rowptr_dev, const int32_t* col_dev,
                                         const double* val_dev, const double* b_dev, int32_t dim,
                                         const int64_t* dims , int32_t n_levels,
                                         const amg_hip_options* opts, amg_hip_solver** out);
amg_hip_status amg_hip_create_tensor_semi_dev(int64_t n, const int32_t* rowptr_dev, const int32_t* col_dev,
                                              const double* val_dev, const double* b_dev, int32_t dim,
                                              const int64_t* dims , int32_t n_levels,
                                              const int32_t* axis_masks ,
                                              double theta, int64_t min_coarse,
                                              const amg_hip_options* opts, amg_hip_solver** out);
amg_hip_status amg_hip_create_tensor_periodic_dev(int64_t n, const int32_t* rowptr_dev, const int32_t* col_dev,
                                                  const double* val_dev, const double* b_dev, int32_t dim,
// ... 317 lines not shown
```

Before: 1541 V-cycles/s.

## Fuse two consecutive coarse levels' smooth/residual/restrict into single duo kernels

Adds dict_duo_down and dict_duo_up kernels. Each one processes two adjacent intermediate levels (smooth, residual, restrict, and the next level's smooth and restrict) within one LDS-resident tile, using halo windows sized from the two half-bandwidths. The goal is to halve kernel launches and the global round trips of intermediate vectors on the mid-hierarchy levels. In exchange it recomputes overlapping halo rows and uses more LDS per block, which may lower occupancy. A tmp/u swap view keeps the external vector API consistent.

```diff
diff --git a/algebraic-multigrid_amd/amg_ctypes.py b/algebraic-multigrid_amd/amg_ctypes.py
--- a/algebraic-multigrid_amd/amg_ctypes.py
+++ b/algebraic-multigrid_amd/amg_ctypes.py
@@ -182,6 +182,11 @@
     "amg_hip_set_patch_min_rows": (None, [C.c_int64]),
     "amg_hip_set_band_chain": (None, [C.c_int32]),
     "amg_hip_set_tail_fusion": (None, [C.c_int32]),
+    "amg_hip_set_pair_duo": (None, [C.c_int32]),
+    "amg_hip_pair_duo_partner": (C.c_int32, [C.c_void_p, C.c_int32]),
+    "amg_hip_duo_windows": (C.c_int32, [C.c_int32, C.c_int32, C.c_int32, _i32p]),
+    "amg_hip_duo_owned": (C.c_int32, [C.c_int32, C.c_int32, _i32p]),
+    "amg_hip_duo_tile_rows": (C.c_int32, [C.c_int32]),
     "amg_hip_set_periodic_device_setup": (None, [C.c_int32]),
     "amg_hip_set_patch_tile_flags": (None, [C.c_int32]),
     "amg_hip_set_patch_xf": (None, [C.c_int32]),
@@ -420,6 +425,30 @@
     lib().amg_hip_set_tail_fusion(int(bool(on)))
 
 
+def set_pair_duo(on):
+    lib().amg_hip_set_pair_duo(int(bool(on)))
+
+
+DUO_WINDOWS_LEN = 31
+
+
+def duo_windows(hb_l, hb_l1, tile_rows=510):
+    out = np.zeros(DUO_WINDOWS_LEN, np.int32)
+    rc = lib().amg_hip_duo_windows(int(hb_l), int(hb_l1), int(tile_rows), out.ctypes.data_as(_i32p))
+    return rc == 0, out
+
+
+def duo_owned(tile, tile_rows=510):
+    out = np.zeros(6, np.int32)
+    if lib().amg_hip_duo_owned(int(tile), int(tile_rows), out.ctypes.data_as(_i32p)) != 0:
+        raise ValueError("amg_hip_duo_owned: bad argument")
+    return [(int(out[0]), int(out[1])), (int(out[2]), int(out[3])), (int(out[4]), int(out[5]))]
+
+
+def duo_tile_rows(hb_l):
+    return int(lib().amg_hip_duo_tile_rows(int(hb_l)))
+
+
 def set_periodic_device_setup(on):
     lib().amg_hip_set_periodic_device_setup(int(bool(on)))
 
@@ -1073,6 +1102,9 @@
         _chk(lib().amg_hip_cycle_must_move(self._h, int(part), C.byref(b)))
         return b.value
 
+    def pair_duo_partner(self, level):
+        return int(lib().amg_hip_pair_duo_partner(self._h, int(level)))
+
     def patch_leg_lines(self, level, leg):
         return int(lib().amg_hip_patch_leg_lines(self._h, int(level), int(leg)))
 
diff --git a/algebraic-multigrid_amd/csrc/kernels.hip b/algebraic-multigrid_amd/csrc/kernels.hip
--- a/algebraic-multigrid_amd/csrc/kernels.hip
+++ b/algebraic-multigrid_amd/csrc/kernels.hip
@@ -851,6 +851,7 @@
   uH1[j] = (d == 0.0) ? xi : xi + omega * ((sum - acc) / d - xi);
 }
 typedef double pair_f64x2 __attribute__((ext_vector_type(2)));
+template <int STRIDE = 510>
 __device__ __forceinline__ void dict_prolong_pre(int tile, int n, int n_h, const double* uh_in,
                                                  pair_f64x2 (&pre)[2], double& lone) {
   bool two[2], one[2];
@@ -858,8 +859,8 @@
 #pragma unroll
   for (int r = 0; r < 2; ++r) {
     const int q = (int)threadIdx.x * 2 + r;
-    const int j = tile * 510 + q;
-    const bool on = !((q == 0 && tile != 0) || q > 510 || j > n);
+    const int j = tile * STRIDE + q;
+    const bool on = !((q == 0 && tile != 0) || q > STRIDE || j > n);
     i[r] = 2 * (int64_t)j;
     two[r] = on && i[r] + 1 < n_h;
     one[r] = on && i[r] + 1 == n_h;
@@ -871,14 +872,15 @@
     if (two[r]) pre[r] = *reinterpret_cast<const pair_f64x2*>(uh_in + i[r]);
   if (one[0] || one[1]) lone = uh_in[n_h - 1];
 }
+template <int STRIDE = 510>
 __device__ __forceinline__ void dict_prolong_tail(int tile, int n, const double* rs, int n_h,
                                                   const pair_f64x2 (&pre)[2], double lone,
                                                   double* uh_out) {
 #pragma unroll
   for (int r = 0; r < 2; ++r) {
     const int q = (int)threadIdx.x * 2 + r;
-    const int j = tile * 510 + q;
-    if ((q == 0 && tile != 0) || q > 510 || j > n) continue;
+    const int j = tile * STRIDE + q;
+    if ((q == 0 && tile != 0) || q > STRIDE || j > n) continue;
     double t0 = 0.0, t1 = 0.0;
     const double b = (j < n) ? rs[q] : 0.0;
     if (j >= 1 && j - 1 < n) t0 += 0.5 * rs[q - 1];
@@ -1215,6 +1217,392 @@
   dict_prolong_tail(tile, n, rs, n_h, pre, pre1, uh_out);
 }
 
+enum {
+  DW_D_R1_LO, DW_D_R1,
+  DW_D_U1_LO, DW_D_U1,
+  DW_D_M1_LO, DW_D_M1,
+  DW_D_R0_LO, DW_D_R0,
+  DW_D_M0_LO, DW_D_M0,
+  DW_D_A0_LO, DW_D_A0,
+  DW_U_S1_LO, DW_U_S1,
+  DW_U_M1_LO, DW_U_M1,
+  DW_U_A1_LO, DW_U_A1,
+  DW_U_S0_LO, DW_U_S0,
+  DW_U_M0_LO, DW_U_M0,
+  DW_U_A0_LO, DW_U_A0,
+  DW_CAP_D_M1, DW_CAP_D_M0, DW_CAP_D_A0, DW_CAP_U_M1, DW_CAP_U_A1, DW_CAP_U_M0, DW_CAP_U_A0,
+  DW_COUNT
+};
+constexpr int DUO_T = 510;
+constexpr int DUO_T_SMALL = 254;
+constexpr int DUO_T_SMALL_HBW = 34;
+constexpr int DUO_D_M1 = 448;
+constexpr int DUO_D_M0 = 1024;
+constexpr int DUO_D_A0 = DUO_D_M0 + 2 * PAIR_HB;
+constexpr int DUO_U_M1 = 512;
+constexpr int DUO_U_A1 = DUO_U_M1 + 2 * PAIR_HB;
+constexpr int DUO_U_M0 = 512 + 2 * PAIR_HB;
+constexpr int DUO_U_A0 = DUO_U_M0 + 2 * PAIR_HB;
+static_assert(DW_COUNT == AMG_DUO_WINDOWS_LEN, "kernels.hpp");
+__host__ __device__ inline void duo_windows(int hbw0, int hbw1, int T, int* w) {
+  const int r1 = (T / 2 + 4) & ~1;
+  w[DW_D_R1_LO] = 0;                    w[DW_D_R1] = r1;
+  w[DW_D_U1_LO] = hbw1;                 w[DW_D_U1] = r1 + 2 * hbw1;
+  w[DW_D_M1_LO] = 2 * hbw1;             w[DW_D_M1] = r1 + 4 * hbw1;
+  w[DW_D_R0_LO] = 4 * hbw1;             w[DW_D_R0] = 2 * w[DW_D_M1] + 2;
+  w[DW_D_M0_LO] = 4 * hbw1 + hbw0;      w[DW_D_M0] = w[DW_D_R0] + 2 * hbw0;
+  w[DW_D_A0_LO] = 4 * hbw1 + 2 * hbw0;  w[DW_D_A0] = w[DW_D_R0] + 4 * hbw0;
+  const int s0 = T + 2;
+  w[DW_U_S0_LO] = 0;         w[DW_U_S0] = s0;
+  w[DW_U_M0_LO] = hbw0;      w[DW_U_M0] = s0 + 2 * hbw0;
+  w[DW_U_A0_LO] = 2 * hbw0;  w[DW_U_A0] = s0 + 4 * hbw0;
+  const int s1 = (s0 / 2 + 2 * hbw0 + 4) & ~1;
+  w[DW_U_S1_LO] = hbw0 + 2;             w[DW_U_S1] = s1;
+  w[DW_U_M1_LO] = hbw0 + 2 + hbw1;      w[DW_U_M1] = s1 + 2 * hbw1;
+  w[DW_U_A1_LO] = hbw0 + 2 + 2 * hbw1;  w[DW_U_A1] = s1 + 4 * hbw1;
+  w[DW_CAP_D_M1] = DUO_D_M1; w[DW_CAP_D_M0] = DUO_D_M0; w[DW_CAP_D_A0] = DUO_D_A0;
+  w[DW_CAP_U_M1] = DUO_U_M1; w[DW_CAP_U_A1] = DUO_U_A1; w[DW_CAP_U_M0] = DUO_U_M0; w[DW_CAP_U_A0] = DUO_U_A0;
+}
+
+__host__ __device__ inline void duo_owned(int t0, int T, int* o) {
+  o[0] = t0;             o[1] = t0 + T;
+  o[2] = t0 / 2;         o[3] = (t0 + T) / 2;
+  o[4] = (t0 + 3) >> 2;  o[5] = (t0 + T + 3) >> 2;
+}
+template <int WORDS, int AP, int FP>
+struct DuoLoads {
+  double tv;
+  int32_t to;
+  uint64_t rw[WORDS];
+  pair_f64x2 a[AP > 0 ? AP : 1];
+  pair_f64x2 f[FP];
+  double fl[FP];
+  uint32_t ty[FP], tl[FP];
+  pair_u64x2 c[FP][WORDS], cl[FP];
+};
+template <int WORDS, bool TYPES, int AP, int FP>
+__device__ __forceinline__ void duo_issue(DuoLoads<WORDS, AP, FP>& g, int n, int a_lo, int AW, int m_lo,
+                                          int W, const uint64_t* __restrict__ codes,
+                                          const uint8_t* __restrict__ rtype,
+                                          const uint64_t* __restrict__ rwords,
+                                          const int32_t* __restrict__ doff,
+                                          const double* __restrict__ dval, int ntab, const double* a,
+                                          const double* __restrict__ f) {
+  const int t = threadIdx.x;
+  g.tv = t < ntab ? dval[t] : 0.0;
+  g.to = t < ntab ? doff[t] : 0;
+#pragma unroll
+  for (int k = 0; k < WORDS; ++k) g.rw[k] = TYPES ? rwords[t * WORDS + k] : 0;
+#pragma unroll
+  for (int k = 0; k < AP; ++k) {
+    const int idx = (k * 256 + t) * 2;
+    const int row = a_lo + idx;
+    g.a[k].x = g.a[k].y = 0.0;
+    if (idx < AW && row >= 0) {
+      if (row + 1 < n) g.a[k] = *reinterpret_cast<const pair_f64x2*>(a + row);
+      else if (row < n) g.a[k].x = a[row];
+    }
+  }
+  bool both[FP], lone[FP];
+#pragma unroll
+  for (int k = 0; k < FP; ++k) {
+    const int lw = (k * 256 + t) * 2, row0 = m_lo + lw;
+    const bool inside = row0 >= 0 && lw < W;
+    both[k] = inside && row0 + 1 < n;
+    lone[k] = inside && row0 + 1 == n;
+    g.f[k].x = g.f[k].y = g.fl[k] = 0.0;
+    if (f) {
+      if (both[k]) g.f[k] = *reinterpret_cast<const pair_f64x2*>(f + row0);
+      if (lone[k]) g.fl[k] = f[row0];
+    }
+  }
+#pragma unroll
+  for (int k = 0; k < FP; ++k) {
+    const int row0 = m_lo + (k * 256 + t) * 2;
+    if (TYPES) {
+      g.ty[k] = 0xFFFFu;
+      g.tl[k] = 0xFFu;
+      if (both[k]) g.ty[k] = *reinterpret_cast<const uint16_t*>(rtype + row0);
+      if (lone[k]) g.tl[k] = rtype[row0];
+    } else {
+      g.cl[k].x = g.cl[k].y = ~(uint64_t)0;
+#pragma unroll
+      for (int j = 0; j < WORDS; ++j) g.c[k][j].x = g.c[k][j].y = ~(uint64_t)0;
+      const uint64_t* cp = codes + (int64_t)row0 * WORDS;
+      if (both[k]) {
+#pragma unroll
+        for (int j = 0; j < WORDS; ++j) g.c[k][j] = reinterpret_cast<const pair_u64x2*>(cp)[j];
+      }
+      if (lone[k]) {
+        if (WORDS == 2) g.cl[k] = *reinterpret_cast<const pair_u64x2*>(cp);
+        else g.cl[k].x = cp[0];
+      }
+    }
+  }
+}
+template <int WORDS, bool TYPES, int AP, int FP>
+__device__ __forceinline__ void duo_commit(const DuoLoads<WORDS, AP, FP>& g, int n, int AW, int m_lo, int W,
+                                           uint64_t* wc, uint16_t* tw, double* aw, double* fw) {
+  const int t = threadIdx.x;
+  if (TYPES) {
+#pragma unroll
+    for (int k = 0; k < WORDS; ++k) wc[t * WORDS + k] = g.rw[k];
+  }
+#pragma unroll
+  for (int k = 0; k < AP; ++k) {
+    const int idx = (k * 256 + t) * 2;
+    if (idx < AW) *reinterpret_cast<pair_f64x2*>(aw + idx) = g.a[k];
+  }
+#pragma unroll
+  for (int k = 0; k < FP; ++k) {
+    const int lw = (k * 256 + t) * 2;
+    if (lw >= W) continue;
+    const bool both = m_lo + lw >= 0 && m_lo + lw + 1 < n;
+    if (fw) {
+      pair_f64x2 fv = g.f[k];
+      fv.x = both ? fv.x : g.fl[k];
+      *reinterpret_cast<pair_f64x2*>(fw + lw) = fv;
+    }
+    if (TYPES) {
+      uint32_t tl = g.tl[k];
+      asm volatile("" : "+v"(tl));
+      tw[lw >> 1] = (uint16_t)(both ? g.ty[k] : (tl | 0xFF00u));
+    } else {
+      pair_u64x2* wp = reinterpret_cast<pair_u64x2*>(wc + lw * WORDS);
+      wp[0] = both ? g.c[k][0] : g.cl[k];
+      if (WORDS == 2) wp[1] = g.c[k][WORDS - 1];
+    }
+  }
+}
+template <int MODE, int WORDS, int UN>
+__device__ __forceinline__ void duo_stage(int n, int m_lo, int W, int lo, int cnt, bool types,
+                                          const DictEntry* tab, const uint64_t* wc, const uint16_t* tw,
+                                          const double* fw, const double* x, int xs, double omega,
+                                          double* out, double* gout, int own_lo, int own_hi) {
+  for (int base = 0; base < cnt; base += 512) {
+    const int k = base + (int)threadIdx.x * 2;
+    const bool in = k < cnt;
+    const int lw = in ? lo + k : W;
+    const int row0 = m_lo + lw;
+    DictStream<WORDS, 2> s;
+    dict_pair_stream<WORDS>(s, lw, W, row0, n, types, wc, tw, fw);
+    if (in && mode_jac(MODE)) {
+      s.xi[0] = x[xs + lw];
+      s.xi[1] = x[xs + lw + 1];
+    }
+    if (types) dict_expand<WORDS, 2>(s, wc);
+    double res[2];
+    dict_rows<MODE, WORDS, UN, 2>(s, in ? xs + lw : 0, tab, x, omega, 0, res);
+    if (in) {
+      out[k] = s.live[0] ? res[0] : 0.0;
+      out[k + 1] = s.live[1] ? res[1] : 0.0;
+      if (gout) {
+#pragma unroll
+        for (int r = 0; r < 2; ++r)
+          if (s.live[r] && row0 + r >= own_lo && row0 + r < own_hi) gout[row0 + r] = res[r];
+      }
+    }
+  }
+}
+__device__ __forceinline__ void duo_restrict_row(int c, int n, int nH, const double* rs, int q, double d,
+                                                 double omega, double& sum_out, double& v_out) {
+  double sum = 0.0, v = 0.0;
+  if (c >= 0 && c < nH) {
+    const int64_t i = 2 * (int64_t)c;
+    if (i < n) sum += 0.5 * rs[2 * q];
+    if (i + 1 < n) sum += 1.0 * rs[2 * q + 1];
+    if (i + 2 < n) sum += 0.5 * rs[2 * q + 2];
+    const double xi = 0.0, acc = 0.0;
+    v = (d == 0.0) ? xi : xi + omega * ((sum - acc) / d - xi);
+  }
+  sum_out = sum;
+  v_out = v;
+}
+
+template <int W0, int U0, int W1, int U1>
+__global__ __launch_bounds__(256) void dict_duo_down_kernel(
+    int n0, const uint64_t* __restrict__ codes0, const uint8_t* __restrict__ rtype0,
+    const uint64_t* __restrict__ rwords0, const int32_t* __restrict__ doff0,
+    const double* __restrict__ dval0, int ntab0, int hbw0,
+    int n1, const uint64_t* __restrict__ codes1, const uint8_t* __restrict__ rtype1,
+    const uint64_t* __restrict__ rwords1, const int32_t* __restrict__ doff1,
+    const double* __restrict__ dval1, int ntab1, int hbw1,
+    const double* a0, const double* __restrict__ f0, double* u0_out, double* r0_out,
+    double* __restrict__ f1_out, const double* __restrict__ diag1, double* u1_out, double* r1_out,
+    int n2, double* __restrict__ f2_out, const double* __restrict__ diag2, double* __restrict__ v2_out,
+    double omega, int T, int xcd_map) {
+  constexpr int WC0 = DUO_D_M0 * W0, WC1 = (DUO_D_M1 > 256 ? DUO_D_M1 : 256) * W1;
+  __shared__ DictEntry tab[256];
+  __shared__ __attribute__((aligned(16))) uint64_t wc0[WC0];
+  __shared__ __attribute__((aligned(16))) uint64_t wc1[WC1];
+  __shared__ uint16_t tw0[DUO_D_M0 / 2];
+  __shared__ uint16_t tw1[DUO_D_M1 / 2];
+  __shared__ __attribute__((aligned(16))) double aw0[DUO_D_A0];
+  __shared__ __attribute__((aligned(16))) double fw0[DUO_D_M0];
+  __shared__ __attribute__((aligned(16))) double uw0[DUO_D_M0];
+  static_assert(2 * DUO_D_M1 <= DUO_D_M0 && DUO_D_M1 + DUO_T / 2 + 8 <= DUO_D_M0, "the aliases fit");
+  double* rs0 = aw0;
+  double* fw1 = fw0;
+  double* vw1 = fw0 + DUO_D_M1;
+  double* uw1 = uw0;
+  double* rs1 = uw0 + DUO_D_M1;
+  int w[DW_COUNT];
+  duo_windows(hbw0, hbw1, T, w);
+  const int tile = xcd_tile(blockIdx.x, gridDim.x, xcd_map);
+  const int t0 = tile * T, ce = (t0 / 2) & ~1, b0 = 2 * ce;
+  const int m0 = b0 - w[DW_D_M0_LO], M0 = w[DW_D_M0], A0 = w[DW_D_A0];
+  const int m1 = ce - w[DW_D_M1_LO], M1 = w[DW_D_M1];
+  const bool types0 = rtype0 != nullptr, types1 = rtype1 != nullptr;
+  const int t = threadIdx.x;
+  DuoLoads<W0, (DUO_D_A0 / 2 + 255) / 256, DUO_D_M0 / 512> g0;
+  DuoLoads<W1, 0, 1> g1;
+  if (types0) duo_issue<W0, true>(g0, n0, m0 - hbw0, A0, m0, M0, codes0, rtype0, rwords0, doff0, dval0, ntab0, a0, f0);
+  else duo_issue<W0, false>(g0, n0, m0 - hbw0, A0, m0, M0, codes0, rtype0, rwords0, doff0, dval0, ntab0, a0, f0);
+  if (types1) duo_issue<W1, true>(g1, n1, 0, 0, m1, M1, codes1, rtype1, rwords1, doff1, dval1, ntab1, nullptr, nullptr);
+  else duo_issue<W1, false>(g1, n1, 0, 0, m1, M1, codes1, rtype1, rwords1, doff1, dval1, ntab1, nullptr, nullptr);
+  pair_f64x2 d1;
+  d1.x = d1.y = 0.0;
+  {
+    const int c = m1 + 2 * t;
+    if (2 * t < M1 && c >= 0) {
+      if (c + 1 < n1) d1 = *reinterpret_cast<const pair_f64x2*>(diag1 + c);
+      else if (c < n1) d1.x = diag1[c];
+    }
+  }
+  int own[6];
+  duo_owned(t0, T, own);
+  const int cc_lo = own[4], cc_hi = min(own[5], n2);
+  const double d2 = cc_lo + t < cc_hi ? diag2[cc_lo + t] : 0.0;
+  dict_put_table<CSR_JACOBI>(tab, g0.tv, g0.to, ntab0);
+  if (types0) duo_commit<W0, true>(g0, n0, A0, m0, M0, wc0, tw0, aw0, fw0);
+  else duo_commit<W0, false>(g0, n0, A0, m0, M0, wc0, tw0, aw0, fw0);
+  if (types1) duo_commit<W1, true>(g1, n1, 0, m1, M1, wc1, tw1, nullptr, nullptr);
+  else duo_commit<W1, false>(g1, n1, 0, m1, M1, wc1, tw1, nullptr, nullptr);
+  __syncthreads();
+  duo_stage<CSR_JACOBI, W0, U0>(n0, m0, M0, 0, M0, types0, tab, wc0, tw0, fw0, aw0, hbw0, omega, uw0, u0_out,
+                                own[0], own[1]);
+  __syncthreads();
+  dict_put_table<CSR_RESID>(tab, g0.tv, g0.to, ntab0);
+  __syncthreads();
+  duo_stage<CSR_RESID, W0, U0>(n0, m0, M0, hbw0, w[DW_D_R0], types0, tab, wc0, tw0, fw0, uw0, 0, omega, rs0,
+                               r0_out, own[0], own[1]);
+  __syncthreads();
+  const int c_own = own[2], c_end = own[3];
+  if (2 * t < M1) {
+    double fv[2], vv[2];
+    duo_restrict_row(m1 + 2 * t, n0, n1, rs0, 2 * t, d1.x, omega, fv[0], vv[0]);
+    duo_restrict_row(m1 + 2 * t + 1, n0, n1, rs0, 2 * t + 1, d1.y, omega, fv[1], vv[1]);
+#pragma unroll
+    for (int r = 0; r < 2; ++r) {
+      const int c = m1 + 2 * t + r;
+      fw1[2 * t + r] = fv[r];
+      vw1[2 * t + r] = vv[r];
+      if (c >= c_own && c < c_end && c < n1) f1_out[c] = fv[r];
+    }
+  }
+  dict_put_table<CSR_JACOBI>(tab, g1.tv, g1.to, ntab1);
+  __syncthreads();
+  duo_stage<CSR_JACOBI, W1, U1>(n1, m1, M1, hbw1, w[DW_D_U1], types1, tab, wc1, tw1, fw1, vw1, 0, omega, uw1,
+                                u1_out, c_own, c_end);
+  __syncthreads();
+  dict_put_table<CSR_RESID>(tab, g1.tv, g1.to, ntab1);
+  __syncthreads();
+  duo_stage<CSR_RESID, W1, U1>(n1, m1, M1, 2 * hbw1, w[DW_D_R1], types1, tab, wc1, tw1, fw1, uw1, -hbw1, omega,
+                               rs1, r1_out, c_own, c_end);
+  __syncthreads();
+  if (cc_lo + t < cc_hi) {
+    const int cc = cc_lo + t;
+    double fv, vv;
+    duo_restrict_row(cc, n1, n2, rs1 + (2 * cc - ce) - 2 * t, t, d2, omega, fv, vv);
+    f2_out[cc] = fv;
+    v2_out[cc] = vv;
+  }
+}
+template <int W0, int U0, int W1, int U1>
+__global__ __launch_bounds__(256) void dict_duo_up_kernel(
+    int n0, const uint64_t* __restrict__ codes0, const uint8_t* __restrict__ rtype0,
+    const uint64_t* __restrict__ rwords0, const int32_t* __restrict__ doff0,
+    const double* __restrict__ dval0, int ntab0, int hbw0,
+    int n1, const uint64_t* __restrict__ codes1, const uint8_t* __restrict__ rtype1,
+    const uint64_t* __restrict__ rwords1, const int32_t* __restrict__ doff1,
+    const double* __restrict__ dval1, int ntab1, int hbw1,
+    const double* a1, const double* __restrict__ f1, double* u1_out,
+    const double* u0_in, const double* __restrict__ f0, double* u0_out,
+    double omega, int n_h, const double* uh_in, double* uh_out, int T, int xcd_map) {
+  constexpr int WC0 = DUO_U_M0 * W0, WC1 = DUO_U_M1 * W1;
+  __shared__ DictEntry tab[256];
+  __shared__ __attribute__((aligned(16))) uint64_t wc0[WC0];
+  __shared__ __attribute__((aligned(16))) uint64_t wc1[WC1];
+  __shared__ uint16_t tw0[DUO_U_M0 / 2];
+  __shared__ uint16_t tw1[DUO_U_M1 / 2];
+  __shared__ __attribute__((aligned(16))) double aw1[DUO_U_A1];
+  __shared__ __attribute__((aligned(16))) double fw1[DUO_U_M1];
+  __shared__ __attribute__((aligned(16))) double uw1[DUO_U_M1];
+  __shared__ __attribute__((aligned(16))) double aw0[DUO_U_A0];
+  __shared__ __attribute__((aligned(16))) double fw0[DUO_U_M0];
+  __shared__ __attribute__((aligned(16))) double uw0[DUO_U_M0];
+  double* vw1 = aw1;
+  double* rs = aw0;
+  int w[DW_COUNT];
+  duo_windows(hbw0, hbw1, T, w);
+  const int tile = xcd_tile(blockIdx.x, gridDim.x, xcd_map);
+  const int t0 = tile * T, ce = (t0 / 2) & ~1;
+  const int m0 = t0 - hbw0, M0 = w[DW_U_M0], A0 = w[DW_U_A0];
+  const int m1 = ce - w[DW_U_M1_LO], M1 = w[DW_U_M1], A1 = w[DW_U_A1];
+  const bool types0 = rtype0 != nullptr, types1 = rtype1 != nullptr;
+  const int t = threadIdx.x;
+  DuoLoads<W1, (DUO_U_A1 / 2 + 255) / 256, 1> g1;
+  DuoLoads<W0, (DUO_U_A0 / 2 + 255) / 256, (DUO_U_M0 + 511) / 512> g0;
+  if (types1) duo_issue<W1, true>(g1, n1, m1 - hbw1, A1, m1, M1, codes1, rtype1, rwords1, doff1, dval1, ntab1, a1, f1);
+  else duo_issue<W1, false>(g1, n1, m1 - hbw1, A1, m1, M1, codes1, rtype1, rwords1, doff1, dval1, ntab1, a1, f1);
+  if (types0) duo_issue<W0, true>(g0, n0, m0 - hbw0, A0, m0, M0, codes0, rtype0, rwords0, doff0, dval0, ntab0, u0_in, f0);
+  else duo_issue<W0, false>(g0, n0, m0 - hbw0, A0, m0, M0, codes0, rtype0, rwords0, doff0, dval0, ntab0, u0_in, f0);
+  pair_f64x2 pre[2];
+  double pre1;
+  if (T == DUO_T) dict_prolong_pre<DUO_T>(tile, n0, n_h, uh_in, pre, pre1);
+  else dict_prolong_pre<DUO_T_SMALL>(tile, n0, n_h, uh_in, pre, pre1);
+  dict_put_table<CSR_JACOBI>(tab, g1.tv, g1.to, ntab1);
+  if (types1) duo_commit<W1, true>(g1, n1, A1, m1, M1, wc1, tw1, aw1, fw1);
+  else duo_commit<W1, false>(g1, n1, A1, m1, M1, wc1, tw1, aw1, fw1);
+  if (types0) duo_commit<W0, true>(g0, n0, A0, m0, M0, wc0, tw0, aw0, fw0);
+  else duo_commit<W0, false>(g0, n0, A0, m0, M0, wc0, tw0, aw0, fw0);
+  __syncthreads();
+  duo_stage<CSR_JACOBI, W1, U1>(n1, m1, M1, 0, M1, types1, tab, wc1, tw1, fw1, aw1, hbw1, omega, uw1, nullptr, 0, 0);
+  __syncthreads();
+  int own[6];
+  duo_owned(t0, T, own);
+  const int c_own = own[2], c_end = own[3];
+  duo_stage<CSR_JACOBI, W1, U1>(n1, m1, M1, hbw1, w[DW_U_S1], types1, tab, wc1, tw1, fw1, uw1, 0, omega, vw1,
+                                u1_out, c_own, c_end);
+  __syncthreads();
+  dict_put_table<CSR_JACOBI>(tab, g0.tv, g0.to, ntab0);
+  {
+    const int s1 = ce - w[DW_U_S1_LO], a_lo = m0 - hbw0;
+    for (int k = 2 * t; k < A0; k += 512) {
+      const int i = a_lo + k;
+      if (i < 0 || i >= n0) continue;
+      const int j = i >> 1;
+      double p0 = 0.0, p1 = 0.0;
+      const double b = (j < n1) ? vw1[j - s1] : 0.0;
+      if (j >= 1 && j - 1 < n1) p0 += 0.5 * vw1[j - 1 - s1];
+      if (j < n1) {
+        p0 += 0.5 * b;
+        p1 += 1.0 * b;
+      }
+      aw0[k] = aw0[k] + p0;
+      if (i + 1 < n0) aw0[k + 1] = aw0[k + 1] + p1;
+    }
+  }
+  __syncthreads();
+  duo_stage<CSR_JACOBI, W0, U0>(n0, m0, M0, 0, M0, types0, tab, wc0, tw0, fw0, aw0, hbw0, omega, uw0, nullptr, 0, 0);
+  __syncthreads();
+  duo_stage<CSR_JACOBI, W0, U0>(n0, m0, M0, hbw0, w[DW_U_S0], types0, tab, wc0, tw0, fw0, uw0, 0, omega, rs, u0_out,
+                                own[0], own[1]);
+  __syncthreads();
+  if (T == DUO_T) dict_prolong_tail<DUO_T>(tile, n0, rs, n_h, pre, pre1, uh_out);
+  else dict_prolong_tail<DUO_T_SMALL>(tile, n0, rs, n_h, pre, pre1, uh_out);
+}
+
 constexpr int PATCH_TW = 64;
 constexpr int PATCH_EH = 48;
 constexpr int patch_th(int rings) { return PATCH_EH - 2 * rings; }
@@ -2295,19 +2683,29 @@
          aligned16(a, b, c) && aligned16(D.rtype ? nullptr : D.codes, nullptr, nullptr) &&
          (!D.rtype || (reinterpret_cast<uintptr_t>(D.rtype) & 1) == 0);
 }
+template <int C> struct DictWU;
+template <> struct DictWU<0> { static constexpr int W = 1, U = 3; };
+template <> struct DictWU<1> { static constexpr int W = 1, U = 5; };
+template <> struct DictWU<2> { static constexpr int W = 1, U = 7; };
+template <> struct DictWU<3> { static constexpr int W = 1, U = 8; };
+template <> struct DictWU<4> { static constexpr int W = 2, U = 9; };
+template <> struct DictWU<5> { static constexpr int W = 2, U = 12; };
+template <> struct DictWU<6> { static constexpr int W = 2, U = 16; };
+constexpr int DICT_WU_CLASSES = 7;
+static int dict_wu_class(int words, int wmax) {
+  if (words == 1) return wmax <= 3 ? 0 : (wmax <= 5 ? 1 : (wmax <= 7 ? 2 : 3));
+  return wmax <= 9 ? 4 : (wmax <= 12 ? 5 : 6);
+}
+template <int C, class F>
+static void dict_dispatch_class(int c, F&& go) {
+  if constexpr (C < DICT_WU_CLASSES) {
+    if (c == C) go(std::integral_constant<int, DictWU<C>::W>{}, std::integral_constant<int, DictWU<C>::U>{});
+    else dict_dispatch_class<C + 1>(c, go);
+  }
+}
 template <class F>
 static hipError_t dict_dispatch_wu(int words, int wmax, F&& go) {
-  using std::integral_constant;
-  if (words == 1) {
-    if (wmax <= 3) go(integral_constant<int, 1>{}, integral_constant<int, 3>{});
-    else if (wmax <= 5) go(integral_constant<int, 1>{}, integral_constant<int, 5>{});
-    else if (wmax <= 7) go(integral_constant<int, 1>{}, integral_constant<int, 7>{});
-    else go(integral_constant<int, 1>{}, integral_constant<int, 8>{});
-  } else {
-    if (wmax <= 9) go(integral_constant<int, 2>{}, integral_constant<int, 9>{});
-    else if (wmax <= 12) go(integral_constant<int, 2>{}, integral_constant<int, 12>{});
-    else go(integral_constant<int, 2>{}, integral_constant<int, 16>{});
-  }
+  dict_dispatch_class<0>(dict_wu_class(words, wmax), go);
   return hipGetLastError();
 }
 hipError_t launch_dict_pair_down(int64_t n, const DictRef& D, int hb, const double* a,
@@ -2338,6 +2736,103 @@
                        dim3(256), 0, st, (int)n, D.codes, D.rtype, D.rwords, D.doff, D.dval, D.ntab,
                        a, f, u_out, omega, hbw, (int)n_h, uh_in, uh_out, dict_xcd_map(D));
   });
+}
+int duo_windows_host(int hb0, int hb1, int tile_rows, int32_t* out) {
+  if (hb0 < 0 || hb1 < 0 || hb0 > PAIR_HB - 1 || hb1 > PAIR_HB - 1 || tile_rows < 4 || (tile_rows & 1) ||
+      tile_rows > DUO_T || !out)
+    return 1;
+  int w[DW_COUNT];
+  duo_windows((hb0 + 1) & ~1, (hb1 + 1) & ~1, tile_rows, w);
+  for (int i = 0; i < DW_COUNT; ++i) out[i] = w[i];
+  return (w[DW_D_M1] <= DUO_D_M1 && w[DW_D_M0] <= DUO_D_M0 && w[DW_D_A0] <= DUO_D_A0 && w[DW_U_M1] <= DUO_U_M1 &&
+          w[DW_U_A1] <= DUO_U_A1 && w[DW_U_M0] <= DUO_U_M0 && w[DW_U_A0] <= DUO_U_A0)
+             ? 0
+             : 1;
+}
+int duo_owned_host(int tile, int tile_rows, int32_t* out) {
+  if (tile < 0 || tile_rows < 4 || (tile_rows & 1) || tile_rows > DUO_T || !out ||
+      (int64_t)tile * tile_rows > ((int64_t)1 << 30))
+    return 1;
+  int o[6];
+  duo_owned(tile * tile_rows, tile_rows, o);
+  for (int i = 0; i < 6; ++i) out[i] = o[i];
+  return 0;
+}
+constexpr int DUO_CLASS_SPAN = 3;
+static int duo_class(const DictRef& D) { return dict_wu_class(D.words, D.wmax); }
+template <int C0, int K, class F>
+static bool duo_dispatch_c1(int c1, F&& go) {
+  if constexpr (K > DUO_CLASS_SPAN) {
+    return false;
+  } else if constexpr (C0 - K < 0 || C0 - K >= DICT_WU_CLASSES) {
+    return duo_dispatch_c1<C0, K + 1>(c1, go);
+  } else {
+    if (c1 == C0 - K) {
+      go(std::integral_constant<int, C0>{}, std::integral_constant<int, C0 - K>{});
+      return true;
+    }
+    return duo_dispatch_c1<C0, K + 1>(c1, go);
+  }
+}
+template <int C0, class F>
+static bool duo_dispatch_c0(int c0, int c1, F&& go) {
+  if constexpr (C0 < DICT_WU_CLASSES) {
+    if (c0 == C0) return duo_dispatch_c1<C0, -1>(c1, go);
+    return duo_dispatch_c0<C0 + 1>(c0, c1, go);
+  } else {
+    return false;
+  }
+}
+constexpr int64_t DUO_MAX_ROWS = 100000;
+int duo_tile_rows(int hb0) { return ((hb0 + 1) & ~1) <= DUO_T_SMALL_HBW ? DUO_T_SMALL : DUO_T; }
+bool dict_duo_ok(int64_t n0, const DictRef& D0, int hb0, int64_t n1, const DictRef& D1, int hb1, int64_t n2) {
+  int32_t w[DW_COUNT];
+  const int c0 = duo_class(D0), c1 = duo_class(D1);
+  return n0 <= DUO_MAX_ROWS && n1 >= 1 && n2 >= 1 && n1 <= (n0 + 1) / 2 && n2 <= (n1 + 1) / 2 &&
+         dict_pair_ok(n0, D0, hb0, nullptr, nullptr, nullptr) && dict_pair_ok(n1, D1, hb1, nullptr, nullptr, nullptr) &&
+         c1 <= c0 + 1 && c0 - c1 <= DUO_CLASS_SPAN && duo_windows_host(hb0, hb1, duo_tile_rows(hb0), w) == 0;
+}
+hipError_t launch_dict_duo_down(int64_t n0, const DictRef& D0, int hb0, int64_t n1, const DictRef& D1, int hb1,
+                                const double* a0, const double* f0, double* u0_out, double* r0_out,
+                                double* f1_out, const double* diag1, double* u1_out, double* r1_out, int64_t n2,
+                                double* f2_out, const double* diag2, double* v2_out, double omega,
+                                hipStream_t st) {
+  if (!dict_duo_ok(n0, D0, hb0, n1, D1, hb1, n2) || !a0 || !f0 || !u0_out || !f1_out || !diag1 || !u1_out ||
+      !f2_out || !diag2 || !v2_out || !aligned16(a0, f0, diag1) || !aligned16(r0_out, nullptr, nullptr))
+    return hipErrorInvalidValue;
+  const int hbw0 = (hb0 + 1) & ~1, hbw1 = (hb1 + 1) & ~1;
+  const int T = duo_tile_rows(hb0);
+  const unsigned tiles = (unsigned)((n0 + T - 1) / T);
+  const bool found = duo_dispatch_c0<0>(duo_class(D0), duo_class(D1), [&](auto C0, auto C1) {
+    using K0 = DictWU<decltype(C0)::value>;
+    using K1 = DictWU<decltype(C1)::value>;
+    hipLaunchKernelGGL((dict_duo_down_kernel<K0::W, K0::U, K1::W, K1::U>), dim3(tiles), dim3(256), 0, st, (int)n0,
+                       D0.codes, D0.rtype, D0.rwords, D0.doff, D0.dval, D0.ntab, hbw0, (int)n1, D1.codes, D1.rtype,
+                       D1.rwords, D1.doff, D1.dval, D1.ntab, hbw1, a0, f0, u0_out, r0_out, f1_out, diag1, u1_out,
+                       r1_out, (int)n2, f2_out, diag2, v2_out, omega, T, dict_xcd_map(D0));
+  });
+  return found ? hipGetLastError() : hipErrorInvalidValue;
+}
+hipError_t launch_dict_duo_up(int64_t n0, const DictRef& D0, int hb0, int64_t n1, const DictRef& D1, int hb1,
+                              const double* a1, const double* f1, double* u1_out, const double* u0_in,
+                              const double* f0, double* u0_out, double omega, int64_t n_h, const double* uh_in,
+                              double* uh_out, hipStream_t st) {
+  if (!dict_duo_ok(n0, D0, hb0, n1, D1, hb1, 1) || !a1 || !f1 || !u1_out || !u0_in || !f0 || !u0_out ||
+      u0_out == u0_in || n0 > n_h || !uh_in || !uh_out || !aligned16(a1, f1, u0_in) || !aligned16(f0, u0_out, uh_in) ||
+      !aligned16(uh_out, nullptr, nullptr))
+    return hipErrorInvalidValue;
+  const int hbw0 = (hb0 + 1) & ~1, hbw1 = (hb1 + 1) & ~1;
+  const int T = duo_tile_rows(hb0);
+  const unsigned tiles = (unsigned)((n0 + T - 1) / T);
+  const bool found = duo_dispatch_c0<0>(duo_class(D0), duo_class(D1), [&](auto C0, auto C1) {
+    using K0 = DictWU<decltype(C0)::value>;
+    using K1 = DictWU<decltype(C1)::value>;
+    hipLaunchKernelGGL((dict_duo_up_kernel<K0::W, K0::U, K1::W, K1::U>), dim3(tiles), dim3(256), 0, st, (int)n0,
+                       D0.codes, D0.rtype, D0.rwords, D0.doff, D0.dval, D0.ntab, hbw0, (int)n1, D1.codes, D1.rtype,
+                       D1.rwords, D1.doff, D1.dval, D1.ntab, hbw1, a1, f1, u1_out, u0_in, f0, u0_out, omega,
+                       (int)n_h, uh_in, uh_out, T, dict_xcd_map(D0));
+  });
+  return found ? hipGetLastError() : hipErrorInvalidValue;
 }
 constexpr int MARCH_TL = 16, MARCH_TC = 64, MARCH_NT = 512;
 constexpr int MARCH_XL = MARCH_TL + 4, MARCH_XC = MARCH_TC + 4;
diff --git a/algebraic-multigrid_amd/csrc/kernels.hpp b/algebraic-multigrid_amd/csrc/kernels.hpp
--- a/algebraic-multigrid_amd/csrc/kernels.hpp
+++ b/algebraic-multigrid_amd/csrc/kernels.hpp
@@ -132,6 +132,20 @@
 hipError_t launch_dict_pair_up(int64_t n, const DictRef& D, int hb, const double* a,
                                const double* f, double* u_out, double omega, int64_t n_h,
                                const double* uh_in, double* uh_out, hipStream_t st);
+constexpr int AMG_DUO_WINDOWS_LEN = 31;
+int duo_windows_host(int hb0, int hb1, int tile_rows, int32_t* out);
+int duo_owned_host(int tile, int tile_rows, int32_t* out);
+int duo_tile_rows(int hb0);
+bool dict_duo_ok(int64_t n0, const DictRef& D0, int hb0, int64_t n1, const DictRef& D1, int hb1, int64_t n2);
+hipError_t launch_dict_duo_down(int64_t n0, const DictRef& D0, int hb0, int64_t n1, const DictRef& D1, int hb1,
+                                const double* a0, const double* f0, double* u0_out, double* r0_out,
+                                double* f1_out, const double* diag1, double* u1_out, double* r1_out, int64_t n2,
+                                double* f2_out, const double* diag2, double* v2_out, double omega,
+                                hipStream_t st);
+hipError_t launch_dict_duo_up(int64_t n0, const DictRef& D0, int hb0, int64_t n1, const DictRef& D1, int hb1,
+                              const double* a1, const double* f1, double* u1_out, const double* u0_in,
+                              const double* f0, double* u0_out, double omega, int64_t n_h, const double* uh_in,
+                              double* uh_out, hipStream_t st);
 constexpr int TAIL_LEVELS_MAX = 6;
 struct TailLevelRef {
   int n, hbw, words, ntab;
diff --git a/algebraic-multigrid_amd/csrc/solver.cpp b/algebraic-multigrid_amd/csrc/solver.cpp
--- a/algebraic-multigrid_amd/csrc/solver.cpp
+++ b/algebraic-multigrid_amd/csrc/solver.cpp
@@ -1446,6 +1446,10 @@
   const char* e = std::getenv("AMG_HIP_BLOCK_LINES");
   return (e && *e == '1') ? 1 : 0;
 }();
+int g_pair_duo = [] {
+  const char* e = std::getenv("AMG_HIP_PAIR_DUO");
+  return (e && *e == '0') ? 0 : 1;
+}();
 int64_t g_patch_min_rows = 1000000;
 
 struct amg_hip_solver {
@@ -1454,6 +1458,9 @@
   int patch_xf = g_patch_xf;
   int patch_tall = g_patch_tall;
   int patch_seam = g_patch_seam;
+  int pair_duo = g_pair_duo;
+  std::vector<int> duo_last;
+  bool duo_known = false;
   int device = 0;
   hipStream_t stream = nullptr;
   bool own_stream = true;
@@ -1678,6 +1685,40 @@
   }
   return -1;
 }
+
+static bool duo_can(const amg_hip_solver* s, int l, int tail_lt) {
+  const int nl = (int)s->lv.size();
+  if (!s->pair_duo || s->opt.no_fusion || s->opt.window || l < 1 || l + 2 >= nl) return false;
+  if (s->slab.levels > 0 && l < s->slab.levels) return false;
+  if (tail_lt >= 0 && l + 1 >= tail_lt) return false;
+  if (!(pair_level_ok(s, l) && pair_level_ok(s, l + 1) && pair_up_ok(s, l) && pair_up_ok(s, l + 1))) return false;
+  const Level& L0 = s->lv[l];
+  const Level& L1 = s->lv[l + 1];
+  const Level& L2 = s->lv[l + 2];
+  return L1.diag.p && L2.diag.p &&
+         dict_duo_ok(L0.n, L0.A_rows.dict_ref(), L0.A_rows.dict_hb, L1.n, L1.A_rows.dict_ref(), L1.A_rows.dict_hb, L2.n);
+}
+static std::vector<int> duo_pairing(const amg_hip_solver* s) {
+  const int nl = (int)s->lv.size();
+  std::vector<int> partner((size_t)nl, -1);
+  if (!s->pair_duo || s->opt.host_only) return partner;
+  const int tail_lt = tail_from(s);
+  for (int l = 1; l + 2 < nl;) {
+    if (duo_can(s, l, tail_lt)) {
+      partner[(size_t)l] = l + 1;
+      partner[(size_t)l + 1] = l;
+      l += 2;
+    } else {
+      ++l;
+    }
+  }
+  return partner;
+}
+int duo_partner(const amg_hip_solver* s, int l) {
+  if (l < 0 || l >= (int)s->lv.size()) return -1;
+  return s->duo_known ? s->duo_last[(size_t)l] : duo_pairing(s)[(size_t)l];
+}
+bool duo_first(const amg_hip_solver* s, int l) { return l >= 1 && duo_partner(s, l) == l + 1; }
 
 static bool march_fill(const amg_hip_solver* s, int l, MarchRef* R) {
   const Level& L = s->lv[l];
@@ -1977,6 +2018,11 @@
   bool first_sweep_done = false;
   const int tail_lt = (part == CYCLE_ALL || part == CYCLE_SLAB_TAIL) ? tail_from(s) : -1;
   bool tail_done = false;
+  const std::vector<int> duo = (part == CYCLE_ALL || part == CYCLE_SLAB_TAIL) ? duo_pairing(s) : std::vector<int>((size_t)nl, -1);
+  if (part == CYCLE_ALL || part == CYCLE_SLAB_TAIL) {
+    s->duo_last = duo;
+    s->duo_known = true;
+  }
   if (part == CYCLE_SLAB_TAIL) {
     Level& L = s->lv[k];
     if (!patch_xf_pair(s, k - 1)) {
@@ -2105,6 +2151,23 @@
       tail_done = true;
       break;
     }
+    if (first_sweep_done && duo[(size_t)l] == l + 1) {
+      Level& L = s->lv[l];
+      Level& C = s->lv[l + 1];
+      Level& CC = s->lv[l + 2];
+      const DevMat& A = L.A_rows;
+      const DevMat& AC = C.A_rows;
+      const bool keep = s->opt.keep_residual != 0;
+      HIP_TRY(launch_dict_duo_down(A.n_rows, A.dict_ref(), A.dict_hb, AC.n_rows, AC.dict_ref(), AC.dict_hb,
+                                   L.tmp.as<double>(), L.f.as<double>(), L.u.as<double>(),
+                                   keep ? L.r.as<double>() : nullptr, C.f.as<double>(), C.diag.as<double>(),
+                                   C.u.as<double>(), keep ? C.r.as<double>() : nullptr, CC.n, CC.f.as<double>(),
+                                   CC.diag.as<double>(), CC.tmp.as<double>(), s->opt.omega, st));
+      s->acct(mat_bytes(A) + 24.0 * L.n + 24.0 * C.n + (keep ? 8.0 * L.n : 0.0));
+      s->acct(mat_bytes(AC) + 24.0 * C.n + 24.0 * CC.n + (keep ? 8.0 * C.n : 0.0));
+      ++l;
+      continue;
+    }
     if (first_sweep_done && pair_level_ok(s, l)) {
       Level& L = s->lv[l];
       Level& C = s->lv[l + 1];
@@ -2261,6 +2324,20 @@
                          P.rowptr(), P.col(), P.v(), C.u.as<double>(), L.u.as<double>(),
                          L.u.as<double>(), 1.0, 0, st));
       s->acct(12.0 * P.nnz + 4.0 * L.n + 8.0 * C.n + 16.0 * L.n);
+    }
+    if (l >= 2 && duo[(size_t)l] == l - 1) {
+      Level& F = s->lv[l - 1];
+      Level& FF = s->lv[l - 2];
+      const DevMat& A = L.A_cols();
+      const DevMat& AF = F.A_cols();
+      HIP_TRY(launch_dict_duo_up(AF.n_rows, AF.dict_ref(), AF.dict_hb, A.n_rows, A.dict_ref(), A.dict_hb,
+                                 L.tmp.as<double>(), L.f.as<double>(), L.u.as<double>(), F.u.as<double>(),
+                                 F.f.as<double>(), F.tmp.as<double>(), s->opt.omega, FF.n, FF.u.as<double>(),
+                                 up_target(l - 2), st));
+      s->acct(mat_bytes(A) + 24.0 * L.n + 16.0 * F.n);
+      s->acct(mat_bytes(AF) + 24.0 * F.n + 16.0 * FF.n);
+      --l;
+      continue;
     }
     if (pair_up_ok(s, l)) {
       Level& F = s->lv[l - 1];
@@ -4153,6 +4230,16 @@
 void amg_hip_set_patch_seam(int32_t on) { g_patch_seam = on ? 1 : 0; }
 void amg_hip_set_band_chain(int32_t on) { g_no_band_chain = on ? 0 : 1; }
 void amg_hip_set_tail_fusion(int32_t on) { g_tail_fusion = on ? 1 : 0; }
+void amg_hip_set_pair_duo(int32_t on) { g_pair_duo = on ? 1 : 0; }
+int32_t amg_hip_pair_duo_partner(const amg_hip_solver* s, int32_t level) {
+  if (!s || level < 0 || level >= (int32_t)s->lv.size()) return -1;
+  return duo_partner(s, level);
+}
+int32_t amg_hip_duo_windows(int32_t hb_l, int32_t hb_l1, int32_t tile_rows, int32_t* out) {
+  return duo_windows_host(hb_l, hb_l1, tile_rows, out);
+}
+int32_t amg_hip_duo_owned(int32_t tile, int32_t tile_rows, int32_t* out) { return duo_owned_host(tile, tile_rows, out); }
+int32_t amg_hip_duo_tile_rows(int32_t hb_l) { return hb_l < 0 ? -1 : duo_tile_rows(hb_l); }
 void amg_hip_set_periodic_device_setup(int32_t on) { g_periodic_device_setup = on ? 1 : 0; }
 void amg_hip_set_f32_lines(int32_t on) { g_f32_lines = on ? 1 : 0; }
 void amg_hip_set_f32_dict(int32_t on) { g_f32_dict = on ? 1 : 0; }
@@ -4822,12 +4909,37 @@
   return AMG_HIP_OK;
 }
 
+static void* dev_vec(amg_hip_solver* s, int32_t level, int32_t which) {
+  Level& L = s->lv[level];
+  if (which == 0) return (duo_first(s, level) ? L.tmp : L.u).p;
+  return which == 1 ? L.f.p : L.r.p;
+}
+struct DuoView {
+  Level* lv[2] = {nullptr, nullptr};
+  DuoView(amg_hip_solver* s, int level) {
+    const int nl = (int)s->lv.size();
+    bool on[2];
+    for (int q = 0; q < 2; ++q) on[q] = level + q < nl && duo_first(s, level + q);
+    for (int q = 0; q < 2; ++q)
+      if (on[q]) {
+        lv[q] = &s->lv[level + q];
+        std::swap(lv[q]->u, lv[q]->tmp);
+      }
+  }
+  ~DuoView() {
+    for (Level* L : lv)
+      if (L) std::swap(L->u, L->tmp);
+  }
+  DuoView(const DuoView&) = delete;
+  DuoView& operator=(const DuoView&) = delete;
+};
+
 amg_hip_status amg_hip_vec_dev_ptr(amg_hip_solver* s, int32_t level, int32_t which, void** ptr, int64_t* n) {
   if (!s || !ptr || level < 0 || level >= (int32_t)s->lv.size() || which < 0 || which > 2)
     return fail(AMG_HIP_EINVAL, "bad argument");
   if (s->opt.host_only) return fail(AMG_HIP_EINVAL, "solver was created with host_only = 1: no device state");
   Level& L = s->lv[level];
-  *ptr = which == 0 ? L.u.p : (which == 1 ? L.f.p : L.r.p);
+  *ptr = dev_vec(s, level, which);
   if (n) *n = L.n;
   return AMG_HIP_OK;
 }
@@ -4847,7 +4959,7 @@
   amg_hip_status r = set_device(s);
   if (r != AMG_HIP_OK) return r;
   Level& L = s->lv[level];
-  void* v = which == 0 ? L.u.p : (which == 1 ? L.f.p : L.r.p);
+  void* v = dev_vec(s, level, which);
   if (to_solver)
     HIP_TRY(hipMemcpyAsync(v, dev_ptr, sizeof(double) * L.n, hipMemcpyDeviceToDevice, s->stream));
   else
@@ -4861,7 +4973,7 @@
   amg_hip_status r = set_device(s);
   if (r != AMG_HIP_OK) return r;
   Level& L = s->lv[level];
-  void* v = which == 0 ? L.u.p : (which == 1 ? L.f.p : L.r.p);
+  void* v = dev_vec(s, level, which);
   HIP_TRY(hipMemsetAsync(v, 0, sizeof(double) * L.n, s->stream));
   return AMG_HIP_OK;
 }
@@ -4874,6 +4986,7 @@
   if (r != AMG_HIP_OK) return r;
   hipStream_t st = s->stream;
   Level& L = s->lv[level];
+  const DuoView view(s, level);
   switch (op) {
     case 0: return enqueue_smooth(s, level, 0);
     case 1: return enqueue_residual(s, level);
@@ -5331,6 +5444,7 @@
   if (!s || level < 0 || level >= (int32_t)s->lv.size()) return nullptr;
   Level& L = s->lv[level];
   if (which == 0 && level >= 1 && !s->opt.host_only && patch_level_ok(s, level)) return &L.tmp;
+  if (which == 0 && level >= 1 && !s->opt.host_only && duo_first(s, level)) return &L.tmp;
   return which == 0 ? &L.u : (which == 1 ? &L.f : (which == 2 ? &L.r : nullptr));
 }
 amg_hip_status amg_hip_get_vec(amg_hip_solver* s, int32_t level, int32_t which, double* out) {
diff --git a/include/amg_hip.h b/include/amg_hip.h
--- a/include/amg_hip.h
+++ b/include/amg_hip.h
@@ -84,6 +84,12 @@
 void amg_hip_set_band_chain(int32_t on);
 
 void amg_hip_set_tail_fusion(int32_t on);
+
+void amg_hip_set_pair_duo(int32_t on);
+int32_t amg_hip_pair_duo_partner(const amg_hip_solver* s, int32_t level);
+int32_t amg_hip_duo_windows(int32_t hb_l, int32_t hb_l1, int32_t tile_rows, int32_t* out);
+int32_t amg_hip_duo_owned(int32_t tile, int32_t tile_rows, int32_t* out);
+int32_t amg_hip_duo_tile_rows(int32_t hb_l);
 
 void amg_hip_set_periodic_device_setup(int32_t on);
 
```

New measurement: 1570 V-cycles/s (median of 6 runs). 1.8% higher.
